# ml4ai/iqlpref

Measured on AMD Instinct MI355X. Metric: iql_grad_steps_per_sec, higher is better.
Workload: dtype bf16; 1 GPU; IQL antmaze-medium-diverse-v2 shapes (S=29 A=8 H=256), 1M-transition device replay, batch 256, one seed per GPU; batch=256, buffer_rows=1000000, graph_unroll=0, graph_launches_per_block=0, eager_steps_per_block=1390

## Files before the change

include/iqlhip.h:

```cpp
#ifndef IQLHIP_H
#define IQLHIP_H

#include <stddef.h>
#include <stdint.h>

#ifdef __cplusplus
extern "C" {
#endif

typedef enum {
  IQLHIP_OK = 0,
  IQLHIP_ERR_INVALID = -1,
  IQLHIP_ERR_HIP = -2,
  IQLHIP_ERR_UNSUPPORTED = -3,
  IQLHIP_ERR_NOMEM = -4
} iqlhip_status;

const char *iqlhip_last_error(void);
int iqlhip_abi_version(void);
const char *iqlhip_build_tag(void);


typedef struct {
  const float *rows;
  int64_t n_rows;
  int32_t row_stride;
  int32_t state_dim;
  int32_t action_dim;
  uint64_t generation;
} iqlhip_replay_view;

int32_t iqlhip_replay_next_offset(int32_t state_dim, int32_t action_dim);
int32_t iqlhip_replay_row_stride(int32_t state_dim, int32_t action_dim);

int iqlhip_replay_pack(float *rows, int32_t row_stride, int32_t state_dim,
                       int32_t action_dim, int64_t first_row, int64_t n,
                       const float *obs, const float *act, const float *rew,
                       const float *next_obs, const float *done, void *stream);

int iqlhip_replay_pack_normalized(float *rows, int32_t row_stride, int32_t state_dim,
                                  int32_t action_dim, int64_t first_row, int64_t n,
                                  const float *obs, const float *act, const float *rew,
                                  const float *next_obs, const float *done, const float *mean,
                                  const float *std, void *stream);

int iqlhip_prep_keep_mask(const uint8_t *terminals, const uint8_t *timeouts, int64_t n,
                          int32_t max_episode_steps, int32_t terminate_on_end, uint8_t *keep,
                          int64_t *ep_steps, void *stream);
int iqlhip_prep_reward_range(const float *rewards, const uint8_t *terminals, int64_t n,
                             int32_t max_episode_steps, double *trj_lens, double *min_ret,
                             double *max_ret, void *stream);
int iqlhip_prep_modify_reward(float *rewards, int64_t n, const double *trj_lens, int32_t sub_first,
                              int32_t scale, int32_t sub_one, double min_ret, double max_ret,
                              int32_t max_episode_steps, void *stream);
int iqlhip_prep_state_stats(const float *obs, int64_t n, int32_t state_dim, double eps, float *mean,
                            float *std, void *stream);

int iqlhip_replay_sample(const iqlhip_replay_view *view, int32_t batch,
                         const int64_t *idx, uint64_t seed, uint64_t step, float *s,
                         float *a, float *r, float *s2, float *d, int64_t *idx_out,
                         void *stream);

#define IQLHIP_PREC_FP32 0
#define IQLHIP_PREC_BF16 1

typedef struct {
  int32_t state_dim, action_dim;
  int32_t hidden_dim;
  int32_t batch_size;
  int32_t deterministic;
  int32_t precision;
  float dropout_p;
  float discount, tau, beta, iql_tau;
  double lr_q, lr_v, lr_actor;
  double adam_beta1, adam_beta2, adam_eps;
  int64_t cosine_t_max;
  uint64_t seed;
  int32_t n_critics;
  int32_t polyak_form;
  int32_t n_hidden;
} iqlhip_trainer_config;

#define IQLHIP_MAX_CRITICS 8
#define IQLHIP_MAX_HIDDEN 6
#define IQLHIP_N_TENSORS (2 * (IQLHIP_MAX_HIDDEN + 1) * (IQLHIP_MAX_CRITICS + 2) + 1)
int iqlhip_arena_layout(const iqlhip_trainer_config *cfg, int64_t offsets[IQLHIP_N_TENSORS],
                        int64_t *n_params, int64_t *n_target);

typedef struct {
  float *params;
  float *exp_avg;
  float *exp_avg_sq;
  float *target;
  float *grads;
} iqlhip_arenas;

typedef struct iqlhip_trainer iqlhip_trainer;

int iqlhip_trainer_create(iqlhip_trainer **out, const iqlhip_trainer_config *cfg,
                          const iqlhip_arenas *arenas);
int iqlhip_trainer_destroy(iqlhip_trainer *t);

int iqlhip_trainer_step_kind(iqlhip_trainer *t, int32_t *kind);

int iqlhip_trainer_sync_weights(iqlhip_trainer *t, void *stream);

int iqlhip_trainer_set_step(iqlhip_trainer *t, int64_t total_it);
int iqlhip_trainer_get_step(iqlhip_trainer *t, int64_t *total_it, double *actor_lr);
int iqlhip_trainer_set_lr(iqlhip_trainer *t, double lr_q, double lr_v, double lr_actor_base);

int iqlhip_train_steps(iqlhip_trainer *t, const iqlhip_replay_view *view, int64_t n_steps,
                       const int64_t *idx, const uint8_t *dropout_keep, float *losses_out,
                       int32_t graph_unroll, void *stream);

int iqlhip_train_steps_valid(iqlhip_trainer *t, const iqlhip_replay_view *view, int64_t n_steps,
                             const int64_t *idx, const int32_t *n_valid, const uint8_t *dropout_keep,
                             float *losses_out, int32_t graph_unroll, void *stream);

#define IQLHIP_MAX_GROUP 16
typedef struct iqlhip_group iqlhip_group;
int iqlhip_group_create(iqlhip_group **out, iqlhip_trainer *const *trainers, int32_t n);
int iqlhip_group_destroy(iqlhip_group *g);
int iqlhip_group_train_steps(iqlhip_group *g, const iqlhip_replay_view *views, int64_t n_steps,
                             const int64_t *const *idx, const uint8_t *const *dropout_keep,
                             float *const *losses_out, int32_t graph_unroll, void *stream);

int iqlhip_group_train_steps_valid(iqlhip_group *g, const iqlhip_replay_view *views, int64_t n_steps,
                                   const int64_t *const *idx, const int32_t *const *n_valid,
                                   const uint8_t *const *dropout_keep, float *const *losses_out,
                                   int32_t graph_unroll, void *stream);

int iqlhip_stream_create_cu_slice(void **stream, int32_t slice, int32_t n_slices);
int iqlhip_stream_destroy(void *stream);

int iqlhip_trainer_launch_counts(iqlhip_trainer *t, int64_t *eager_steps, int64_t *graph_launches);
int iqlhip_group_launch_counts(iqlhip_group *g, int64_t *eager_steps, int64_t *graph_launches);

int iqlhip_group_set_timing(iqlhip_group *g, int32_t enable);
int iqlhip_group_get_timing(iqlhip_group *g, double avg_ms[3], int64_t *n_launches);

int iqlhip_train_batch(iqlhip_trainer *t, const float *s, const float *a, const float *r,
                       const float *s2, const float *d, const uint8_t *dropout_keep,
                       float *losses_out, void *stream);

int iqlhip_forward(iqlhip_trainer *t, int32_t which, const float *s, const float *a,
                   int64_t n, float *out, void *stream);

#define IQLHIP_MLP_MAX_LAYERS 8
typedef struct {
  int32_t n_layers;
  int32_t dims[IQLHIP_MLP_MAX_LAYERS + 1];
  const float *weights[IQLHIP_MLP_MAX_LAYERS];
  const float *biases[IQLHIP_MLP_MAX_LAYERS];
  int32_t w_in_out;
  int32_t hidden_act;
  int32_t out_act;
  float dropout_p;
  uint32_t dropout_call;
  uint64_t dropout_seed;
} iqlhip_mlp_desc;

int iqlhip_mlp_forward(const iqlhip_mlp_desc *d, const float *x, int64_t n, int32_t x_stride,
                       float *out, int32_t out_stride, void *stream);

int iqlhip_cvar_tail_mean(const float *preds, int32_t S, int64_t N, int32_t n_tail, float *out,
                          void *stream);

typedef struct {
  int32_t state_dim, action_dim;
  int32_t embd_dim;
  int32_t num_heads;
  int32_t inter_dim;
  int32_t num_layers;
  int32_t n_temb;
  float eps;
  const float *state_wT, *state_b;
  const float *action_wT, *action_b;
  const float *temb;
  const float *sln_w, *sln_b;
  const float *ln0_w, *ln0_b;
  const float *qkv_w, *qkv_b;
  const float *attn_out_w, *attn_out_b;
  const float *ln1_w, *ln1_b;
  const float *mlp_in_w, *mlp_in_b;
  const float *mlp_out_w, *mlp_out_b;
  const float *lnf_w, *lnf_b;
  const float *pref_w_last;
  float pref_b_last;
} iqlhip_pt_weights;

int iqlhip_pt_relabel(const iqlhip_pt_weights *w, const float *obs, const float *act, int64_t n_rows,
                      const int64_t *win_start, const int32_t *win_len, const int32_t *win_t0,
                      int64_t n_win, int32_t query_length, float *out, void *stream);

typedef struct {
  const float *ln0_w, *ln0_b;
  const float *qkv_w, *qkv_b;
  const float *attn_out_w, *attn_out_b;
  const float *ln1_w, *ln1_b;
  const float *mlp_in_w, *mlp_in_b;
  const float *mlp_out_w, *mlp_out_b;
} iqlhip_pt_block;

typedef struct {
  int32_t state_dim, action_dim;
  int32_t embd_dim;
  int32_t num_heads;
  int32_t inter_dim;
  int32_t num_layers;
  int32_t n_temb;
  float eps;
  const float *state_wT, *state_b;
  const float *action_wT, *action_b;
  const float *temb;
  const float *sln_w, *sln_b;
  const float *lnf_w, *lnf_b;
  const float *pref_w_last;
  float pref_b_last;
  const iqlhip_pt_block *blocks;
} iqlhip_pt_model;

int iqlhip_pt_general_workspace_bytes(const iqlhip_pt_model *m, int32_t query_length, int64_t n_win,
                                      size_t *bytes);

int iqlhip_pt_relabel_general(const iqlhip_pt_model *m, const float *obs, const float *act, int64_t n_rows,
                              const int64_t *win_start, const int32_t *win_len, const int32_t *win_t0,
                              int64_t n_win, int32_t query_length, void *workspace, size_t workspace_bytes,
                              float *out, void *stream);

int iqlhip_np_randint(uint32_t *state, const int64_t *hi, int32_t K, int32_t batch,
                      int64_t n_batches, int64_t *const *out, void *stream);

int iqlhip_replay_append(float *rows, int32_t row_stride, int32_t state_dim, int32_t action_dim,
                         int64_t capacity, int64_t pointer, int64_t n, const float *obs, const float *act,
                         const float *rew, const float *next_obs, const float *done, void *stream);

int iqlhip_np_randint_growing(uint32_t *state, const int64_t *hi0, const int64_t *cap, int32_t growth,
                              int32_t K, int32_t batch, int64_t n_steps, int64_t *const *out, void *stream);

int iqlhip_explore_action(iqlhip_trainer *t, const float *s, int64_t rows, const float *eps,
                          float expl_noise, float noise_clip, float max_action, uint32_t call, float *out,
                          void *stream);

int iqlhip_block_epoch_indices(const int64_t *perm, int64_t n_rows, int32_t batch, int64_t t0,
                               int64_t n_steps, int64_t *idx, int32_t *n_valid, void *stream);

int iqlhip_block_epoch_indices_group(const int64_t *const *perm, int64_t n_rows, int32_t batch, int64_t t0,
                                     int64_t n_steps, int64_t *const *idx, int32_t *n_valid, int32_t K,
                                     void *stream);

typedef struct {
  int32_t n_obs;
  int32_t n_near;
  int32_t state_dim;
  int32_t action_dim;
  int32_t max_horizon;
// ... 41 lines not shown
```

iqlpref_amd/_lib.py:

```python
import ctypes as C
import os

HERE = os.path.dirname(os.path.abspath(__file__))
LIB_PATH = os.environ.get("IQLHIP_LIB") or os.path.join(HERE, "libiqlhip.so")

PREC_FP32 = 0
PREC_BF16 = 1
MAX_CRITICS = 8
MAX_HIDDEN = 6
N_TENSORS = 2 * (MAX_HIDDEN + 1) * (MAX_CRITICS + 2) + 1
MLP_MAX_LAYERS = 8
MAX_GROUP = 16
ACT_FLAX_BASE = 8
ABI_VERSION = 6
CHOICE_MEAN = 0
CHOICE_MEDIAN = 1

ERR_INVALID = -1
ERR_HIP = -2
ERR_UNSUPPORTED = -3
ERR_NOMEM = -4


class ReplayView(C.Structure):
    _fields_ = [("rows", C.c_void_p), ("n_rows", C.c_int64), ("row_stride", C.c_int32),
                ("state_dim", C.c_int32), ("action_dim", C.c_int32), ("generation", C.c_uint64)]


class TrainerConfig(C.Structure):
    _fields_ = [("state_dim", C.c_int32), ("action_dim", C.c_int32),
                ("hidden_dim", C.c_int32), ("batch_size", C.c_int32),
                ("deterministic", C.c_int32), ("precision", C.c_int32),
                ("dropout_p", C.c_float),
                ("discount", C.c_float), ("tau", C.c_float), ("beta", C.c_float),
                ("iql_tau", C.c_float),
                ("lr_q", C.c_double), ("lr_v", C.c_double), ("lr_actor", C.c_double),
                ("adam_beta1", C.c_double), ("adam_beta2", C.c_double),
                ("adam_eps", C.c_double),
                ("cosine_t_max", C.c_int64), ("seed", C.c_uint64),
                ("n_critics", C.c_int32), ("polyak_form", C.c_int32), ("n_hidden", C.c_int32)]


class Arenas(C.Structure):
    _fields_ = [("params", C.c_void_p), ("exp_avg", C.c_void_p), ("exp_avg_sq", C.c_void_p),
                ("target", C.c_void_p), ("grads", C.c_void_p)]


class MlpDesc(C.Structure):
    _fields_ = [("n_layers", C.c_int32), ("dims", C.c_int32 * (MLP_MAX_LAYERS + 1)),
                ("weights", C.c_void_p * MLP_MAX_LAYERS),
                ("biases", C.c_void_p * MLP_MAX_LAYERS),
                ("w_in_out", C.c_int32), ("hidden_act", C.c_int32), ("out_act", C.c_int32),
                ("dropout_p", C.c_float), ("dropout_call", C.c_uint32), ("dropout_seed", C.c_uint64)]


class PtWeights(C.Structure):
    _fields_ = ([("state_dim", C.c_int32), ("action_dim", C.c_int32), ("embd_dim", C.c_int32),
                 ("num_heads", C.c_int32), ("inter_dim", C.c_int32), ("num_layers", C.c_int32),
                 ("n_temb", C.c_int32), ("eps", C.c_float)] +
                [(n, C.c_void_p) for n in (
                    "state_wT", "state_b", "action_wT", "action_b", "temb", "sln_w", "sln_b",
                    "ln0_w", "ln0_b", "qkv_w", "qkv_b", "attn_out_w", "attn_out_b",
                    "ln1_w", "ln1_b", "mlp_in_w", "mlp_in_b", "mlp_out_w", "mlp_out_b",
                    "lnf_w", "lnf_b", "pref_w_last")] +
                [("pref_b_last", C.c_float)])


PT_MAX_LAYERS = 8


class PtBlock(C.Structure):
    _fields_ = [(n, C.c_void_p) for n in (
        "ln0_w", "ln0_b", "qkv_w", "qkv_b", "attn_out_w", "attn_out_b",
        "ln1_w", "ln1_b", "mlp_in_w", "mlp_in_b", "mlp_out_w", "mlp_out_b")]


class PtModel(C.Structure):
    _fields_ = ([("state_dim", C.c_int32), ("action_dim", C.c_int32), ("embd_dim", C.c_int32),
                 ("num_heads", C.c_int32), ("inter_dim", C.c_int32), ("num_layers", C.c_int32),
                 ("n_temb", C.c_int32), ("eps", C.c_float)] +
                [(n, C.c_void_p) for n in (
                    "state_wT", "state_b", "action_wT", "action_b", "temb", "sln_w", "sln_b",
                    "lnf_w", "lnf_b", "pref_w_last")] +
                [("pref_b_last", C.c_float), ("blocks", C.POINTER(PtBlock))])


class BbSim(C.Structure):
    _fields_ = ([(n, C.c_int32) for n in ("n_obs", "n_near", "state_dim", "action_dim", "max_horizon",
                                          "actor_out_stride")] +
                [(n, C.c_void_p) for n in ("state", "drift", "ctl", "obs_hist", "act_hist", "record", "actor_in",
                                           "actor_out", "state_mean", "state_std", "min_actions", "max_actions")])


P = C.c_void_p
SYMBOLS = {
    "iqlhip_last_error": (C.c_char_p, []),
    "iqlhip_abi_version": (C.c_int, []),
    "iqlhip_build_tag": (C.c_char_p, []),
    "iqlhip_replay_row_stride": (C.c_int32, [C.c_int32, C.c_int32]),
    "iqlhip_replay_next_offset": (C.c_int32, [C.c_int32, C.c_int32]),
    "iqlhip_replay_pack": (C.c_int, [P, C.c_int32, C.c_int32, C.c_int32, C.c_int64, C.c_int64,
                                     P, P, P, P, P, P]),
    "iqlhip_replay_pack_normalized": (C.c_int, [P, C.c_int32, C.c_int32, C.c_int32, C.c_int64, C.c_int64,
                                                P, P, P, P, P, P, P, P]),
    "iqlhip_prep_keep_mask": (C.c_int, [P, P, C.c_int64, C.c_int32, C.c_int32, P, P, P]),
    "iqlhip_prep_reward_range": (C.c_int, [P, P, C.c_int64, C.c_int32, P, C.POINTER(C.c_double),
                                           C.POINTER(C.c_double), P]),
    "iqlhip_prep_modify_reward": (C.c_int, [P, C.c_int64, P, C.c_int32, C.c_int32, C.c_int32, C.c_double,
                                            C.c_double, C.c_int32, P]),
    "iqlhip_prep_state_stats": (C.c_int, [P, C.c_int64, C.c_int32, C.c_double, P, P, P]),
    "iqlhip_replay_sample": (C.c_int, [C.POINTER(ReplayView), C.c_int32, P, C.c_uint64,
                                       C.c_uint64, P, P, P, P, P, P, P]),
    "iqlhip_arena_layout": (C.c_int, [C.POINTER(TrainerConfig), C.POINTER(C.c_int64 * N_TENSORS),
                                      C.POINTER(C.c_int64), C.POINTER(C.c_int64)]),
    "iqlhip_trainer_create": (C.c_int, [C.POINTER(P), C.POINTER(TrainerConfig), C.POINTER(Arenas)]),
    "iqlhip_trainer_destroy": (C.c_int, [P]),
    "iqlhip_trainer_step_kind": (C.c_int, [P, C.POINTER(C.c_int32)]),
    "iqlhip_trainer_sync_weights": (C.c_int, [P, P]),
    "iqlhip_trainer_set_step": (C.c_int, [P, C.c_int64]),
    "iqlhip_trainer_get_step": (C.c_int, [P, C.POINTER(C.c_int64), C.POINTER(C.c_double)]),
    "iqlhip_trainer_set_lr": (C.c_int, [P, C.c_double, C.c_double, C.c_double]),
    "iqlhip_train_steps": (C.c_int, [P, C.POINTER(ReplayView), C.c_int64, P, P, P, C.c_int32, P]),
    "iqlhip_train_steps_valid": (C.c_int, [P, C.POINTER(ReplayView), C.c_int64, P, P, P, P, C.c_int32, P]),
    "iqlhip_group_create": (C.c_int, [C.POINTER(P), C.POINTER(P), C.c_int32]),
    "iqlhip_group_destroy": (C.c_int, [P]),
    "iqlhip_group_train_steps": (C.c_int, [P, C.POINTER(ReplayView), C.c_int64, C.POINTER(P), C.POINTER(P),
                                           C.POINTER(P), C.c_int32, P]),
    "iqlhip_group_train_steps_valid": (C.c_int, [P, C.POINTER(ReplayView), C.c_int64, C.POINTER(P), C.POINTER(P),
                                                 C.POINTER(P), C.POINTER(P), C.c_int32, P]),
    "iqlhip_group_set_timing": (C.c_int, [P, C.c_int32]),
    "iqlhip_group_get_timing": (C.c_int, [P, C.POINTER(C.c_double * 3), C.POINTER(C.c_int64)]),
    "iqlhip_trainer_launch_counts": (C.c_int, [P, C.POINTER(C.c_int64), C.POINTER(C.c_int64)]),
    "iqlhip_group_launch_counts": (C.c_int, [P, C.POINTER(C.c_int64), C.POINTER(C.c_int64)]),
    "iqlhip_stream_create_cu_slice": (C.c_int, [C.POINTER(P), C.c_int32, C.c_int32]),
    "iqlhip_stream_destroy": (C.c_int, [P]),
    "iqlhip_train_batch": (C.c_int, [P, P, P, P, P, P, P, P, P]),
    "iqlhip_forward": (C.c_int, [P, C.c_int32, P, P, C.c_int64, P, P]),
    "iqlhip_mlp_forward": (C.c_int, [C.POINTER(MlpDesc), P, C.c_int64, C.c_int32, P, C.c_int32, P]),
    "iqlhip_cvar_tail_mean": (C.c_int, [P, C.c_int32, C.c_int64, C.c_int32, P, P]),
    "iqlhip_pt_relabel": (C.c_int, [C.POINTER(PtWeights), P, P, C.c_int64, P, P, P, C.c_int64, C.c_int32,
                                    P, P]),
    "iqlhip_pt_general_workspace_bytes": (C.c_int, [C.POINTER(PtModel), C.c_int32, C.c_int64,
                                                    C.POINTER(C.c_size_t)]),
    "iqlhip_pt_relabel_general": (C.c_int, [C.POINTER(PtModel), P, P, C.c_int64, P, P, P, C.c_int64, C.c_int32,
                                            P, C.c_size_t, P, P]),
    "iqlhip_np_randint": (C.c_int, [P, P, C.c_int32, C.c_int32, C.c_int64, P, P]),
    "iqlhip_replay_append": (C.c_int, [P, C.c_int32, C.c_int32, C.c_int32, C.c_int64, C.c_int64, C.c_int64,
                                       P, P, P, P, P, P]),
    "iqlhip_np_randint_growing": (C.c_int, [P, P, P, C.c_int32, C.c_int32, C.c_int32, C.c_int64, P, P]),
    "iqlhip_explore_action": (C.c_int, [P, P, C.c_int64, P, C.c_float, C.c_float, C.c_float, C.c_uint32, P, P]),
    "iqlhip_block_epoch_indices": (C.c_int, [P, C.c_int64, C.c_int32, C.c_int64, C.c_int64, P, P, P]),
    "iqlhip_block_epoch_indices_group": (C.c_int, [C.POINTER(P), C.c_int64, C.c_int32, C.c_int64, C.c_int64,
                                                   C.POINTER(P), P, C.c_int32, P]),
    "iqlhip_bb_sim_reset": (C.c_int, [C.POINTER(BbSim), P]),
    "iqlhip_bb_sim_step": (C.c_int, [C.POINTER(BbSim), P]),
    "iqlhip_bb_sim_rollout": (C.c_int, [C.POINTER(BbSim), C.POINTER(MlpDesc), C.c_int32, P]),
    "iqlhip_bb_sim_episodes_scratch_bytes": (C.c_int, [C.POINTER(C.POINTER(MlpDesc)), C.c_int32,
                                                       C.POINTER(C.c_size_t)]),
    "iqlhip_bb_sim_episodes": (C.c_int, [C.POINTER(BbSim), C.POINTER(C.POINTER(MlpDesc)), C.c_int32, P, C.c_size_t,
                                         P]),
    "iqlhip_posterior_choice_workspace_bytes": (C.c_int, [C.c_int32, C.c_int64, C.c_int32, C.POINTER(C.c_size_t)]),
    "iqlhip_posterior_choice": (C.c_int, [P, P, C.c_int32, C.c_int64, C.c_int32, C.c_int32, P, P, P, C.c_size_t, P]),
    "iqlhip_step_cost": (C.c_int, [C.POINTER(TrainerConfig), C.POINTER(C.c_double),
                                   C.POINTER(C.c_double)]),
    "iqlhip_trainer_set_timing": (C.c_int, [P, C.c_int32]),
    "iqlhip_trainer_get_timing": (C.c_int, [P, C.POINTER(C.c_double * 3), C.POINTER(C.c_int64)]),
}

_lib = None


def load():
    global _lib
    if _lib is not None:
        return _lib
    if not os.path.exists(LIB_PATH):
        raise ImportError(
            f"{LIB_PATH} is missing: build it with `python -m iqlpref_amd.build` "
            "(hipcc --offload-arch=gfx950). iqlpref_amd has no CPU fallback.")
    lib = C.CDLL(LIB_PATH)
    for name, (res, args) in SYMBOLS.items():
        fn = getattr(lib, name)
        fn.restype = res
        fn.argtypes = args
    if lib.iqlhip_abi_version() != ABI_VERSION:
        raise ImportError("libiqlhip.so ABI version mismatch; rebuild it")
    if not os.environ.get("IQLHIP_LIB"):
        from . import build as _build
        want, have = _build.source_tag(), lib.iqlhip_build_tag().decode()
        if want != have:
            raise ImportError(
                f"{LIB_PATH} was built from other sources (library tag {have}, sources {want}): "
                "rebuild it with `python -m iqlpref_amd.build`")
    _lib = lib
    return lib


def build_tag():
    return load().iqlhip_build_tag().decode()


def check(rc):
    if rc == 0:
        return
    msg = load().iqlhip_last_error().decode("utf-8", "replace")
    if rc == ERR_INVALID:
        raise ValueError(msg)
    if rc == ERR_UNSUPPORTED:
        raise NotImplementedError(msg)
    if rc == ERR_NOMEM:
        raise MemoryError(msg)
    raise RuntimeError(msg)


def require_gpu(device):
    import torch
    dev = torch.device(device)
    if dev.type != "cuda" or not torch.cuda.is_available():
        raise RuntimeError(
            f"iqlpref_amd runs on a ROCm GPU only (got device={device!r}, "
            f"torch.cuda.is_available()={torch.cuda.is_available()}); there is no CPU path")
    return dev


def stream_ptr():
    import torch
    raw = getattr(torch._C, "_cuda_getCurrentRawStream", None)
    if raw is not None:
        return C.c_void_p(raw(torch.cuda.current_device()))
    return C.c_void_p(torch.cuda.current_stream().cuda_stream)


def ptr(t):
    return C.c_void_p(t.data_ptr()) if t is not None else C.c_void_p(0)
```

iqlpref_amd/csrc/api.hip:

```cpp
#include <hip/hip_runtime.h>

#include <algorithm>
#include <cmath>
#include <cstdarg>
#include <cstdio>
#include <cstdlib>
#include <cstring>
#include <new>
#include <vector>

#include "../../include/iqlhip.h"
#include "common.h"
#include "iql_deep.h"
#include "iql_step.h"
#include "step_math.h"

namespace iqlhip {
struct DeepTrainer;
bool deep_shape_ok(const iqlhip_trainer_config &, int n_hidden, const char **why);
hipError_t deep_create(DeepTrainer **, const iqlhip_trainer_config &, int n_hidden, const iqlhip_arenas &,
                       const int64_t *offsets);
void deep_destroy(DeepTrainer *);
hipError_t deep_sync_weights(DeepTrainer *, hipStream_t);
const DeepDesc &deep_desc(const DeepTrainer *);
const DeepDesc *deep_desc_dev(const DeepTrainer *);
hipError_t deep_step(const DeepTrainer *, const DeepDesc *, const DeepArgs *, DeepCtr *, const AdamCoef *coefs, int K,
                     hipStream_t, hipEvent_t *ev);
hipError_t deep_infer(DeepTrainer *, int which, const float *s, const float *a, int64_t n, float *out, hipStream_t);
int layer2_parts(int H);
hipError_t launch_forward(bool, const TrainerDesc &, const TrainerDesc *, const DevArgs *, const DevCtr *,
                          int n_seeds, hipStream_t);
hipError_t launch_backward(bool, const TrainerDesc &, const TrainerDesc *, const DevArgs *, DevCtr *,
                           int n_seeds, hipStream_t, bool counts = false);
hipError_t launch_stage(bool, const TrainerDesc &, const TrainerDesc *, const DevArgs *, const DevCtr *,
                        int n_seeds, hipStream_t);
int strip_rows();
int update_lds_floats();
hipError_t launch_update(bool, const TrainerDesc *, const DevArgs *, DevCtr *, const UpdItem *, int,
                         int n_seeds, hipStream_t);
hipError_t launch_sync_weights(bool, const TrainerDesc *, hipStream_t);
hipError_t prepare_step_kernels();

hipError_t launch_infer(bool, const TrainerDesc &, const TrainerDesc *, const FwdNet &, const float *,
                        const float *, int64_t, float *, int, hipStream_t);

hipError_t launch_pack(float *rows, int stride, int S, int A, int64_t first, int64_t n, const float *obs,
                       const float *act, const float *rew, const float *nxt, const float *done,
                       hipStream_t st);
hipError_t launch_sample(const iqlhip_replay_view &v, int batch, const int64_t *idx, uint64_t seed,
                         uint64_t step, float *s, float *a, float *r, float *s2, float *d,
                         int64_t *idx_out, hipStream_t st);
hipError_t launch_mlp_f32(const iqlhip_mlp_desc &d, const float *x, int64_t n, int x_stride, float *out,
                          int out_stride, hipStream_t st);
hipError_t launch_cvar(const float *preds, int S, int64_t N, int n_tail, float *out, hipStream_t st);
hipError_t launch_keep_steps(const uint8_t *term, const uint8_t *tmo, int64_t n, int64_t M, int toe,
                             uint8_t *keep, int64_t *ep_steps, hipStream_t st);
hipError_t launch_reward_range(const float *rew, const uint8_t *term, int64_t n, int64_t M, double *trj_lens,
                               double *out3, hipStream_t st);
hipError_t launch_modify_reward(float *rew, int64_t n, const double *trj_lens, int sub_first, int scale,
                                int sub_one, double min_ret, double range, float steps, hipStream_t st);
hipError_t launch_state_stats(const float *x, int64_t n, int S, double eps, float *mean_f, float *std_f,
                              hipStream_t st);
hipError_t launch_pack_norm(float *rows, int stride, int S, int A, int64_t first, int64_t n, const float *obs,
                            const float *act, const float *rew, const float *nxt, const float *done,
                            const float *mean, const float *sd, hipStream_t st);
size_t pt_smem_bytes(const iqlhip_pt_weights &W, int ql);
hipError_t launch_pt(const iqlhip_pt_weights &W, const float *obs, const float *act, int64_t n_rows,
                     const int64_t *win_start, const int32_t *win_len, const int32_t *win_t0, int64_t n_win,
                     int ql, float *out, hipStream_t st);
size_t pt_general_bytes(const iqlhip_pt_model &m, int ql, int64_t nw);
int64_t pt_general_fit(const iqlhip_pt_model &m, int ql, size_t bytes);
int pt_general_tp(int ql);
hipError_t launch_pt_general(const iqlhip_pt_model &m, const float *obs, const float *act, int64_t n_rows,
                             const int64_t *win_start, const int32_t *win_len, const int32_t *win_t0,
                             int64_t n_win, int ql, float *ws, int64_t chunk, float *out, hipStream_t st);
hipError_t launch_block_epoch(const int64_t *perm, int64_t n_rows, int batch, int64_t t0, int64_t n_steps, int64_t *idx,
                              int32_t *n_valid, hipStream_t st);
hipError_t launch_block_epoch_group(const int64_t *const *perm, int64_t n_rows, int batch, int64_t t0, int64_t n_steps,
                                    int64_t *const *idx, int32_t *n_valid, int K, hipStream_t st);
hipError_t launch_replay_append(float *rows, int stride, int S, int A, int64_t pointer, int64_t capacity, int64_t n,
                                const float *obs, const float *act, const float *rew, const float *nxt,
                                const float *done, hipStream_t st);
hipError_t launch_np_randint_growing(uint32_t *state, const int64_t *hi0, const int64_t *cap, int growth, int K,
                                     int batch, int64_t n_steps, int64_t *const *out, hipStream_t st);
hipError_t launch_explore_epilogue(float *act, int64_t rows, int A, const float *log_std, const float *eps,
                                   float expl_noise, float noise_clip, float max_action, uint64_t seed, uint32_t call,
                                   hipStream_t st);
hipError_t launch_np_randint(uint32_t *state, const int64_t *hi, int K, int64_t total, int64_t *const *out,
                             hipStream_t st);
hipError_t launch_bb_step(const iqlhip_bb_sim &sim, int reset, hipStream_t st);
size_t bb_episodes_scratch_bytes(const iqlhip_mlp_desc *const *actors, int n);
hipError_t launch_bb_episodes(const iqlhip_bb_sim *sims, const iqlhip_mlp_desc *const *actors, int n, void *scratch,
                              hipStream_t st);
size_t choice_workspace_bytes(int64_t N, int n);
int64_t choice_fit_rows(int64_t N, int n, size_t bytes);
hipError_t launch_posterior_choice(uint32_t *state, const float *preds, int S, int64_t N, int n, int mode,
                                   float *out, uint16_t *idx_out, uint16_t *ws, int64_t slot_rows,
                                   hipStream_t st);
}

using namespace iqlhip;

static thread_local char g_err[512] = "";
static int fail(int code, const char *fmt, ...) {
  va_list ap;
  va_start(ap, fmt);
  vsnprintf(g_err, sizeof(g_err), fmt, ap);
  va_end(ap);
  return code;
}
#define HIP_TRY(expr)                                                                         \
  do {                                                                                        \
    hipError_t e_ = (expr);                                                                   \
    if (e_ != hipSuccess)                                                                     \
      return fail(IQLHIP_ERR_HIP, "%s failed: %s (%s:%d)", #expr, hipGetErrorString(e_), __FILE__, \
                  __LINE__);                                                                  \
  } while (0)

extern "C" const char *iqlhip_last_error(void) { return g_err; }
static hipError_t capture_stream(hipStream_t *out) {
  static thread_local hipStream_t pool[64] = {};
  int dev = 0;
  hipError_t e = hipGetDevice(&dev);
  if (e != hipSuccess) return e;
  if (dev < 0 || dev >= 64) return hipErrorInvalidDevice;
  if (!pool[dev]) {
    e = hipStreamCreateWithFlags(&pool[dev], hipStreamNonBlocking);
    if (e != hipSuccess) return e;
  }
  *out = pool[dev];
  return hipSuccess;
}

extern "C" int iqlhip_abi_version(void) { return 6; }
#ifndef IQLHIP_BUILD_TAG
#define IQLHIP_BUILD_TAG "untagged"
#endif
static const char g_build_tag[] = "IQLHIP_BUILD_TAG=" IQLHIP_BUILD_TAG;
extern "C" const char *iqlhip_build_tag(void) { return g_build_tag + sizeof("IQLHIP_BUILD_TAG=") - 1; }

extern "C" int32_t iqlhip_replay_next_offset(int32_t S, int32_t A) { return round_up(S + A + 2, 4); }
extern "C" int32_t iqlhip_replay_row_stride(int32_t S, int32_t A) {
  return round_up(iqlhip_replay_next_offset(S, A) + S, 4);
}

extern "C" int iqlhip_replay_pack(float *rows, int32_t row_stride, int32_t S, int32_t A, int64_t first_row,
                                  int64_t n, const float *obs, const float *act, const float *rew,
                                  const float *next_obs, const float *done, void *stream) {
  if (!rows || !obs || !act || !rew || !next_obs || !done) return fail(IQLHIP_ERR_INVALID, "null pointer");
  if (S <= 0 || A <= 0 || n < 0 || first_row < 0 || row_stride < iqlhip_replay_row_stride(S, A) || (row_stride & 3))
    return fail(IQLHIP_ERR_INVALID, "bad replay geometry S=%d A=%d stride=%d", S, A, row_stride);
  if (n == 0) return 0;
  HIP_TRY(launch_pack(rows, row_stride, S, A, first_row, n, obs, act, rew, next_obs, done,
                      (hipStream_t)stream));
  return 0;
}

extern "C" int iqlhip_replay_pack_normalized(float *rows, int32_t row_stride, int32_t S, int32_t A,
                                             int64_t first_row, int64_t n, const float *obs, const float *act,
                                             const float *rew, const float *next_obs, const float *done,
                                             const float *mean, const float *std, void *stream) {
  if (!rows || !obs || !act || !rew || !next_obs || !done || !mean || !std)
    return fail(IQLHIP_ERR_INVALID, "null pointer");
  if (S <= 0 || A <= 0 || n < 0 || first_row < 0 || row_stride < iqlhip_replay_row_stride(S, A) || (row_stride & 3))
    return fail(IQLHIP_ERR_INVALID, "bad replay geometry S=%d A=%d stride=%d", S, A, row_stride);
  if (n == 0) return 0;
  HIP_TRY(launch_pack_norm(rows, row_stride, S, A, first_row, n, obs, act, rew, next_obs, done, mean, std,
                           (hipStream_t)stream));
  return 0;
}

extern "C" int iqlhip_prep_keep_mask(const uint8_t *terminals, const uint8_t *timeouts, int64_t n,
                                     int32_t max_episode_steps, int32_t terminate_on_end, uint8_t *keep,
                                     int64_t *ep_steps, void *stream) {
  if (!terminals || !keep || !ep_steps) return fail(IQLHIP_ERR_INVALID, "null pointer");
  if (n < 1) return fail(IQLHIP_ERR_INVALID, "n must be >= 1");
  if (!timeouts && max_episode_steps < 1) return fail(IQLHIP_ERR_INVALID, "max_episode_steps must be >= 1");
  HIP_TRY(launch_keep_steps(terminals, timeouts, n, max_episode_steps, terminate_on_end != 0, keep, ep_steps,
                            (hipStream_t)stream));
  return 0;
}

extern "C" int iqlhip_prep_reward_range(const float *rewards, const uint8_t *terminals, int64_t n,
                                        int32_t max_episode_steps, double *trj_lens, double *min_ret,
                                        double *max_ret, void *stream) {
  if (!rewards || !terminals || !trj_lens || !min_ret || !max_ret) return fail(IQLHIP_ERR_INVALID, "null pointer");
  if (n < 1 || max_episode_steps < 1) return fail(IQLHIP_ERR_INVALID, "n and max_episode_steps must be >= 1");
  double out3[3];
  HIP_TRY(launch_reward_range(rewards, terminals, n, max_episode_steps, trj_lens, out3, (hipStream_t)stream));
  if (out3[2] == 0.0) return fail(IQLHIP_ERR_INVALID, "dataset holds no complete episode");
  *min_ret = out3[0], *max_ret = out3[1];
  return 0;
}

extern "C" int iqlhip_prep_modify_reward(float *rewards, int64_t n, const double *trj_lens, int32_t sub_first,
                                         int32_t scale, int32_t sub_one, double min_ret, double max_ret,
                                         int32_t max_episode_steps, void *stream) {
  if (!rewards) return fail(IQLHIP_ERR_INVALID, "null pointer");
  if (sub_first < 0 || sub_first > 2) return fail(IQLHIP_ERR_INVALID, "sub_first must be 0, 1 or 2");
  if (sub_first == 2 && !trj_lens) return fail(IQLHIP_ERR_INVALID, "sub_first = 2 needs trj_lens");
  if (n <= 0) return 0;
  HIP_TRY(launch_modify_reward(rewards, n, trj_lens, sub_first, scale != 0, sub_one != 0, min_ret,
                               max_ret - min_ret, (float)max_episode_steps, (hipStream_t)stream));
  return 0;
}

extern "C" int iqlhip_prep_state_stats(const float *obs, int64_t n, int32_t state_dim, double eps, float *mean,
                                       float *std, void *stream) {
  if (!obs || !mean || !std) return fail(IQLHIP_ERR_INVALID, "null pointer");
  if (n < 1 || state_dim < 1 || state_dim > 256) return fail(IQLHIP_ERR_UNSUPPORTED, "n >= 1, 1 <= state_dim <= 256");
  HIP_TRY(launch_state_stats(obs, n, state_dim, eps, mean, std, (hipStream_t)stream));
  return 0;
}

extern "C" int iqlhip_replay_sample(const iqlhip_replay_view *view, int32_t batch, const int64_t *idx,
                                    uint64_t seed, uint64_t step, float *s, float *a, float *r, float *s2,
                                    float *d, int64_t *idx_out, void *stream) {
  if (!view || !view->rows || !s || !a || !r || !s2 || !d) return fail(IQLHIP_ERR_INVALID, "null pointer");
  if (batch <= 0) return fail(IQLHIP_ERR_INVALID, "batch must be positive");
  if (view->n_rows <= 0) return fail(IQLHIP_ERR_INVALID, "cannot sample from an empty replay buffer");
  HIP_TRY(launch_sample(*view, batch, idx, seed, step, s, a, r, s2, d, idx_out, (hipStream_t)stream));
  return 0;
}

static void group_invalidate(struct iqlhip_group *g);

struct Throttle {
  static constexpr int NEV = 2;
  hipEvent_t ev[NEV] = {};
  bool used[NEV] = {};
  int head = 0;
  int64_t since = 0;
  static int64_t window() {
    static const int64_t w = [] {
      const char *e = getenv("IQLHIP_MAX_INFLIGHT");
      const int64_t total = e ? atoll(e) : 6144;
      return total <= 0 ? (int64_t)0 : (total / 3 > 0 ? total / 3 : (int64_t)1);
    }();
    return w;
  }
  hipError_t queued(int64_t n, hipStream_t st) {
    const int64_t w = window();
    if (w == 0) return hipSuccess;
    since += n;
    if (since < w) return hipSuccess;
    since = 0;
    hipError_t e;
    if (!ev[head] && (e = hipEventCreateWithFlags(&ev[head], hipEventDisableTiming)) != hipSuccess) return e;
    if (used[head] && (e = hipEventSynchronize(ev[head])) != hipSuccess) return e;
    if ((e = hipEventRecord(ev[head], st)) != hipSuccess) return e;
    used[head] = true;
    head = (head + 1) % NEV;
    return hipSuccess;
  }
  void destroy() {
    for (auto &e : ev)
      if (e) (void)hipEventDestroy(e), e = nullptr;
  }
};

struct StepQueue {
  static constexpr int ARG_RING = 8;
  DevArgs *harg[ARG_RING] = {};
  hipEvent_t harg_ev[ARG_RING] = {};
  bool harg_used[ARG_RING] = {};
  int harg_head = 0;
  DevArgs dev_args[IQLHIP_MAX_GROUP];
  bool dev_args_valid = false;
  hipGraphExec_t gexec = nullptr;
  int graph_unroll = 0;
  bool graph_counts = false;
  hipStream_t cap_stream = nullptr;
  Throttle throttle;
  bool timing = false;
  hipEvent_t ev[5] = {};
  double t_acc[3] = {0, 0, 0};
  double t_empty = 0;
  int64_t t_n = 0;
  int64_t n_eager = 0, n_graph = 0;

  int push(const DevArgs *want, int K, DevArgs *dst, hipStream_t st) {
    const int slot = harg_head;
    harg_head = (slot + 1) % ARG_RING;
    if (!harg[slot]) {
      HIP_TRY(hipHostMalloc((void **)&harg[slot], sizeof(DevArgs) * K, hipHostMallocDefault));
      HIP_TRY(hipEventCreateWithFlags(&harg_ev[slot], hipEventDisableTiming));
    }
    if (harg_used[slot]) HIP_TRY(hipEventSynchronize(harg_ev[slot]));
    for (int k = 0; k < K; ++k) harg[slot][k] = dev_args[k] = want[k];
    HIP_TRY(hipMemcpyAsync(dst, harg[slot], sizeof(DevArgs) * K, hipMemcpyHostToDevice, st));
    HIP_TRY(hipEventRecord(harg_ev[slot], st));
    harg_used[slot] = true;
    return 0;
  }
  void drop_graph() {
    if (gexec) (void)hipGraphExecDestroy(gexec);
    gexec = nullptr;
  }
  template <typename Step>
  int ensure_graph(int U, bool counts, Step step) {
    if (gexec && graph_unroll == U && graph_counts == counts) return 0;
    drop_graph();
    hipGraph_t g = nullptr;
    if (!cap_stream) HIP_TRY(capture_stream(&cap_stream));
    HIP_TRY(hipStreamBeginCapture(cap_stream, hipStreamCaptureModeThreadLocal));
    int rc = 0;
    for (int u = 0; u < U && !rc; ++u) rc = step(cap_stream);
    const hipError_t ce = hipStreamEndCapture(cap_stream, &g);
    if ((rc || ce != hipSuccess) && g) (void)hipGraphDestroy(g);
    if (rc) return rc;
    HIP_TRY(ce);
    const hipError_t ie = hipGraphInstantiate(&gexec, g, nullptr, nullptr, 0);
    (void)hipGraphDestroy(g);
    HIP_TRY(ie);
    graph_unroll = U, graph_counts = counts;
    return 0;
  }
  int replay(int64_t &done, int64_t n, hipStream_t st) {
    for (; done + graph_unroll <= n; done += graph_unroll) {
      HIP_TRY(hipGraphLaunch(gexec, st));
      ++n_graph;
      HIP_TRY(throttle.queued(3 * (int64_t)graph_unroll, st));
    }
    return 0;
  }
  int eager_issued(hipStream_t st) {
    ++n_eager;
    if (!timing) {
      HIP_TRY(throttle.queued(3, st));
      return 0;
    }
    HIP_TRY(hipEventRecord(ev[4], st));
    HIP_TRY(hipEventSynchronize(ev[4]));
    for (int k = 0; k < 3; ++k) {
      float ms = 0.f;
      HIP_TRY(hipEventElapsedTime(&ms, ev[k], ev[k + 1]));
      t_acc[k] += ms;
    }
    float ems = 0.f;
    HIP_TRY(hipEventElapsedTime(&ems, ev[3], ev[4]));
    t_empty += ems;
    ++t_n;
    return 0;
  }
  int set_timing(bool enable) {
    timing = enable;
    t_acc[0] = t_acc[1] = t_acc[2] = 0, t_empty = 0, t_n = 0;
    if (timing)
      for (auto &e : ev)
        if (!e) HIP_TRY(hipEventCreate(&e));
    return 0;
  }
  void get_timing(double avg_ms[3], int64_t *n) const {
    for (int k = 0; k < 3; ++k) {
      const double v = t_n ? (t_acc[k] - t_empty) / (double)t_n : 0.0;
      avg_ms[k] = v > 0 ? v : 0.0;
    }
    if (n) *n = t_n;
  }
  void launch_counts(int64_t *eager_steps, int64_t *graph_launches) const {
    if (eager_steps) *eager_steps = n_eager;
    if (graph_launches) *graph_launches = n_graph;
  }
  void destroy() {
    drop_graph();
    for (int k = 0; k < ARG_RING; ++k) {
      if (harg_ev[k]) (void)hipEventDestroy(harg_ev[k]);
      if (harg[k]) (void)hipHostFree(harg[k]);
    }
    for (auto &e : ev)
      if (e) (void)hipEventDestroy(e);
    throttle.destroy();
  }
};

struct DeepRing {
  static constexpr int RING = 4;
  static constexpr int64_t CAP = 1024;
  int K = 0;
  char *dev = nullptr;
  char *host[RING] = {};
  hipEvent_t ev[RING] = {};
  bool used[RING] = {};
  int head = 0;
  size_t head_bytes() const { return (size_t)K * (sizeof(DeepArgs) + sizeof(DeepCtr)); }
  size_t bytes(int64_t n) const { return head_bytes() + (size_t)n * K * sizeof(AdamCoef); }
  DeepArgs *dargs() const { return reinterpret_cast<DeepArgs *>(dev); }
  DeepCtr *dctr() const { return reinterpret_cast<DeepCtr *>(dev + (size_t)K * sizeof(DeepArgs)); }
  AdamCoef *dcoef() const { return reinterpret_cast<AdamCoef *>(dev + head_bytes()); }
  hipError_t init(int k) {
    K = k;
    hipError_t e = hipMalloc((void **)&dev, bytes(CAP));
    return e != hipSuccess ? e : hipMemset(dev, 0, bytes(CAP));
  }
  void destroy() {
    for (int k = 0; k < RING; ++k) {
      if (ev[k]) (void)hipEventDestroy(ev[k]);
      if (host[k]) (void)hipHostFree(host[k]);
      ev[k] = nullptr, host[k] = nullptr;
    }
    if (dev) (void)hipFree(dev);
    dev = nullptr;
  }
};

struct iqlhip_trainer {
  iqlhip_trainer_config cfg;
  iqlhip_arenas arenas;
  DeepTrainer *deep = nullptr;
  DeepRing deep_ring;
  TrainerDesc D;
  bool bf16;
  void *ws = nullptr;
  size_t ws_bytes = 0;
  TrainerDesc *ddesc = nullptr;
  DevArgs *dargs = nullptr;
  DevCtr *dctr = nullptr;
  UpdItem *ditems = nullptr;
  int n_items = 0;
  int own_n_items = 0;
  std::vector<UpdItem> net_items[MAX_TRAIN];
  int n_half0[MAX_TRAIN] = {};
  TrainerDesc *own_ddesc = nullptr;
  DevArgs *own_dargs = nullptr;
  DevCtr *own_dctr = nullptr;
  UpdItem *own_ditems = nullptr;
  struct iqlhip_group *group = nullptr;

  float *batch_rows = nullptr;
  int64_t total_it = 0;
  double lr_q, lr_v, lr_a_base;
  StepQueue queue;
};

static_assert(MAX_CRITICS == IQLHIP_MAX_CRITICS, "iql_step.h and iqlhip.h disagree");
static_assert(IQLHIP_N_TENSORS == 2 * DEEP_MAX_LIN * MAX_TRAIN + 1, "offset table size");
static_assert(IQLHIP_MAX_HIDDEN + 1 == DEEP_MAX_LIN, "iql_deep.h and iqlhip.h disagree");
static int n_critics(const iqlhip_trainer_config &c) { return c.n_critics > 0 ? c.n_critics : 2; }
static int n_hidden(const iqlhip_trainer_config &c) { return c.n_hidden > 0 ? c.n_hidden : 2; }
static bool is_deep(const iqlhip_trainer_config &c) {
  static const bool force_general = getenv("IQLHIP_FORCE_GENERAL") != nullptr;
  return n_hidden(c) != 2 || (c.hidden_dim != 64 && c.hidden_dim != 128 && c.hidden_dim != 256) || force_general;
}

static int check_cfg(const iqlhip_trainer_config *c) {
  if (!c) return fail(IQLHIP_ERR_INVALID, "null config");
  if (c->n_critics < 0 || c->n_critics == 1 || c->n_critics > MAX_CRITICS)
    return fail(IQLHIP_ERR_UNSUPPORTED, "n_critics %d: 0 (= 2) or 2..%d", c->n_critics, MAX_CRITICS);
  if (c->state_dim <= 0 || c->action_dim <= 0) return fail(IQLHIP_ERR_INVALID, "bad dims");
  if (c->n_hidden < 0) return fail(IQLHIP_ERR_INVALID, "n_hidden must be >= 0");
  if (const char *why = nullptr; !deep_shape_ok(*c, n_hidden(*c), &why))
    return fail(IQLHIP_ERR_UNSUPPORTED, "n_hidden %d, hidden_dim %d: %s", n_hidden(*c), c->hidden_dim, why);
  if (c->batch_size < 16 || c->batch_size % 16)
    return fail(IQLHIP_ERR_UNSUPPORTED, "batch_size %d: must be a positive multiple of 16", c->batch_size);
  if (c->action_dim > 32) return fail(IQLHIP_ERR_UNSUPPORTED, "action_dim %d > 32", c->action_dim);
  if (c->state_dim + c->action_dim > 128) return fail(IQLHIP_ERR_UNSUPPORTED, "state_dim+action_dim > 128");
  if (!is_deep(*c) && (c->batch_size / 16) * (n_critics(*c) + 2 + (c->deterministic ? 0 : c->action_dim)) + n_critics(*c) + 2 >
      update_lds_floats())
    return fail(IQLHIP_ERR_UNSUPPORTED, "batch_size %d too large for action_dim %d", c->batch_size,
                c->action_dim);
  if (c->precision != IQLHIP_PREC_FP32 && c->precision != IQLHIP_PREC_BF16)
    return fail(IQLHIP_ERR_INVALID, "precision must be IQLHIP_PREC_FP32 or IQLHIP_PREC_BF16");
  if (c->dropout_p >= 1.0f) return fail(IQLHIP_ERR_INVALID, "dropout_p must be < 1");
  if (c->cosine_t_max <= 0) return fail(IQLHIP_ERR_INVALID, "cosine_t_max must be positive");
  if (c->polyak_form != 0 && c->polyak_form != 1) return fail(IQLHIP_ERR_INVALID, "polyak_form must be 0 or 1");
  return 0;
}

struct Layout {
  int64_t off[IQLHIP_N_TENSORS];
  int64_t n_params, n_target;
  int64_t true_params, true_target;
};
static void net_dims(const iqlhip_trainer_config &c, int net, int *in, int *out) {
  const int E = n_critics(c);
  *in = net < E ? c.state_dim + c.action_dim : c.state_dim;
  *out = (net == E + 1) ? c.action_dim : 1;
}
static Layout make_layout(const iqlhip_trainer_config &c) {
  constexpr int64_t ALIGN = 32;
  Layout L;
  int64_t o = 0, cnt = 0;
  const int H = c.hidden_dim, NL = n_hidden(c) + 1;
  const int E = n_critics(c), ntrain = E + 2;
  for (int k = 0; k < IQLHIP_N_TENSORS; ++k) L.off[k] = -1;
  for (int n = 0; n < ntrain; ++n) {
    int in, out;
    net_dims(c, n, &in, &out);
    for (int l = 0; l < NL; ++l) {
      const int64_t rows = l == NL - 1 ? out : H, cols = l == 0 ? in : H;
      const int64_t sz[2] = {rows * cols, rows};
      for (int k = 0; k < 2; ++k) {
        o = (o + ALIGN - 1) / ALIGN * ALIGN;
        L.off[(n * NL + l) * 2 + k] = o;
        o += sz[k];
        cnt += sz[k];
      }
    }
    if (n == E - 1) L.n_target = o, L.true_target = cnt;
  }
  if (c.deterministic) {
    L.off[ntrain * NL * 2] = -1;
  } else {
    o = (o + ALIGN - 1) / ALIGN * ALIGN;
    L.off[ntrain * NL * 2] = o;
    o += c.action_dim;
    cnt += c.action_dim;
  }
  L.n_params = o;
  L.true_params = cnt;
  return L;
}

extern "C" int iqlhip_arena_layout(const iqlhip_trainer_config *cfg, int64_t offsets[IQLHIP_N_TENSORS],
                                   int64_t *n_params, int64_t *n_target) {
  if (int e = check_cfg(cfg)) return e;
  const Layout L = make_layout(*cfg);
  if (offsets) memcpy(offsets, L.off, sizeof(L.off));
  if (n_params) *n_params = L.n_params;
  if (n_target) *n_target = L.n_target;
  return 0;
}

extern "C" int iqlhip_step_cost(const iqlhip_trainer_config *cfg, double *bytes, double *flops) {
  if (int e = check_cfg(cfg)) return e;
  const Layout L = make_layout(*cfg);
  const double B = cfg->batch_size, S = cfg->state_dim, A = cfg->action_dim, H = cfg->hidden_dim;
  if (bytes) *bytes = 4.0 * B * (2 * S + A + 2) + 32.0 * (double)L.true_params + 8.0 * (double)L.true_target;
  if (flops) {
    const double E = n_critics(*cfg), HH = (n_hidden(*cfg) - 1) * H * H;
    const double wv = S * H + HH + H, wq = (S + A) * H + HH + H, wa = S * H + HH + H * A;
    const double fwd = 2 * wv + 2 * E * wq + wa;
    const double dw = wv + E * wq + wa;
    const double dx = (HH + H) * (E + 1) + (HH + H * A);
    *flops = 2.0 * B * (fwd + dw + dx);
  }
  return 0;
}

template <typename T>
static T *carve(char *&p, size_t n) {
  T *r = reinterpret_cast<T *>(p);
  p += (n * sizeof(T) + 255) / 256 * 256;
  return r;
}

static std::vector<UpdItem> flatten_table(const std::vector<UpdItem> (&per_xcd)[8], size_t min_depth, size_t *depth_out,
                                          size_t min_idle) {
  size_t depth = 0, n_real = 0;
  for (auto &v : per_xcd) depth = v.size() > depth ? v.size() : depth, n_real += v.size();
  while (8 * depth - n_real < min_idle) ++depth;
  if (depth < min_depth) depth = min_depth;
  std::vector<UpdItem> items;
  for (size_t d = 0; d < depth; ++d)
    for (int x = 0; x < 8; ++x) {
      UpdItem pad;
      memset(&pad, 0, sizeof(pad));
      pad.net = -1;
      items.push_back(d < per_xcd[x].size() ? per_xcd[x][d] : pad);
    }
  int n_pad = 0;
  for (auto &it : items)
    if (it.net < 0) it.o0 = n_pad++;
  for (auto &it : items)
    if (it.net < 0) it.i0 = n_pad;
  if (depth_out) *depth_out = depth;
  return items;
}

static void deal_items(const iqlhip_trainer *t, int member, int group_size, std::vector<UpdItem> (&per_xcd)[8]) {
  const int NT = t->D.ntrain;
  const bool group = group_size > 1;
  const bool whole = group && group_size % 8 == 0;
  if (whole && NT == 4) {
    for (int n = 0; n < NT; ++n)
      for (auto &it : t->net_items[n]) per_xcd[(2 * n + member) & 7].push_back(it);
    return;
  }
  if (NT == 4) {
    for (int n = 0; n < NT; ++n)
      for (size_t i = 0; i < t->net_items[n].size(); ++i)
        per_xcd[(2 * n + ((int)i < t->n_half0[n] ? 0 : 1)) & 7].push_back(t->net_items[n][i]);
    return;
  }
  size_t total = 0, g = 0;
  for (int n = 0; n < NT; ++n) total += t->net_items[n].size();
  for (int n = 0; n < NT; ++n)
    for (auto &it : t->net_items[n]) {
      const int x = (int)(g * 8 / total);
      per_xcd[(x + (group ? member : 0)) & 7].push_back(it);
      ++g;
    }
  if (!group) {
    constexpr size_t CUS_PER_XCD = 32;
    auto weight = [](const UpdItem &it) { return it.layer == 1 ? 3 : (it.layer == 0 ? 2 : 1); };
    for (auto &col : per_xcd) {
      if (col.size() <= CUS_PER_XCD || col.size() >= 2 * CUS_PER_XCD) continue;
      const size_t d = col.size() - CUS_PER_XCD;
      std::vector<UpdItem> sorted(col);
      std::stable_sort(sorted.begin(), sorted.end(), [&](const UpdItem &a, const UpdItem &b) { return weight(a) < weight(b); });
      std::vector<UpdItem> out(sorted.begin(), sorted.begin() + d);
      out.insert(out.end(), sorted.begin() + 2 * d, sorted.end());
      out.insert(out.end(), sorted.begin() + d, sorted.begin() + 2 * d);
      col.swap(out);
    }
  }
}

extern "C" int iqlhip_trainer_create(iqlhip_trainer **out, const iqlhip_trainer_config *cfg,
                                     const iqlhip_arenas *ar) {
  if (!out) return fail(IQLHIP_ERR_INVALID, "null out");
  if (int e = check_cfg(cfg)) return e;
  if (!ar || !ar->params || !ar->exp_avg || !ar->exp_avg_sq || !ar->target)
    return fail(IQLHIP_ERR_INVALID, "null arena pointer");
  HIP_TRY(prepare_step_kernels());
  iqlhip_trainer *t = new (std::nothrow) iqlhip_trainer();
  if (!t) return fail(IQLHIP_ERR_NOMEM, "host allocation failed");
  t->cfg = *cfg;
  t->arenas = *ar;
  t->bf16 = cfg->precision == IQLHIP_PREC_BF16;
  t->lr_q = cfg->lr_q, t->lr_v = cfg->lr_v, t->lr_a_base = cfg->lr_actor;
  const Layout L = make_layout(*cfg);
  if (is_deep(*cfg)) {
    memset(&t->D, 0, sizeof(t->D));
    t->D.E = n_critics(*cfg);
    const size_t rows_bytes = (size_t)cfg->batch_size * iqlhip_replay_row_stride(cfg->state_dim, cfg->action_dim) * 4;
    hipError_t e = deep_create(&t->deep, *cfg, n_hidden(*cfg), *ar, L.off);
    if (e == hipSuccess && (e = hipMalloc((void **)&t->batch_rows, rows_bytes)) != hipSuccess) deep_destroy(t->deep);
    if (e == hipSuccess && (e = t->deep_ring.init(1)) != hipSuccess) {
      deep_destroy(t->deep);
      (void)hipFree(t->batch_rows);
      t->deep_ring.destroy();
    }
    if (e != hipSuccess) {
      delete t;
      return fail(e == hipErrorOutOfMemory ? IQLHIP_ERR_NOMEM : IQLHIP_ERR_HIP, "general step: %s", hipGetErrorString(e));
    }
    *out = t;
    return 0;
  }
  const int S = cfg->state_dim, A = cfg->action_dim, H = cfg->hidden_dim, B = cfg->batch_size;
  const int es = t->bf16 ? 2 : 4, KM = t->bf16 ? 32 : 16;
  TrainerDesc &D = t->D;
  memset(&D, 0, sizeof(D));
  D.S = S, D.A = A, D.H = H, D.B = B, D.BP = round_up(B, 32);
  const int E = n_critics(*cfg), NT = E + 2, NF = 2 * E + 3;
  D.E = E, D.ntrain = NT, D.nfwd = NF, D.net_v = E, D.net_a = E + 1;
  D.out_v = E, D.out_qt = E + 1, D.out_nv = 2 * E + 1, D.out_mean = 2 * E + 2;
  D.two_over_B = 2.0f / (float)B, D.inv_E = 1.0f / (float)E;
  D.OUTW = round_up(D.out_mean + A, 4);
  D.deterministic = cfg->deterministic;
  D.has_dropout = cfg->dropout_p > 0.f;
  D.discount = cfg->discount, D.tau = cfg->tau, D.beta = cfg->beta, D.iql_tau = cfg->iql_tau;
  D.one_m_tau = (float)(1.0 - (double)cfg->tau);
  D.polyak_convex = cfg->polyak_form == 1;
  if (D.has_dropout) {
    const float scale = 1.0f / (float)(1.0 - (double)cfg->dropout_p);
    if (t->bf16) {
      uint32_t u;
      memcpy(&u, &scale, 4);
      u = (u + 0x7fffu + ((u >> 16) & 1u)) & 0xffff0000u;
      memcpy(&D.drop_scale, &u, 4);
    } else {
      D.drop_scale = scale;
    }
    const double thr = (double)cfg->dropout_p * 4294967296.0;
    D.drop_thr = thr >= 4294967295.0 ? 0xffffffffu : (uint32_t)thr;
  }
  D.beta1 = cfg->adam_beta1, D.beta2 = cfg->adam_beta2, D.eps = cfg->adam_eps;
  D.t_max = cfg->cosine_t_max;
  D.seed = cfg->seed;
  D.params = ar->params, D.exp_avg = ar->exp_avg, D.exp_avg_sq = ar->exp_avg_sq;
  D.target = ar->target, D.grads = ar->grads;
  D.off_log_std = L.off[NT * 6];
  D.opmax = round_up(A, 16);
  D.xrows = round_up(S + A, 64);
  D.k1max = round_up(S + A, KM);
  size_t total = 0;
  auto add = [&](size_t bytes) { total += (bytes + 255) / 256 * 256; };
  int k1pad[MAX_TRAIN], outpad[MAX_TRAIN], indim[MAX_TRAIN], outdim[MAX_TRAIN];
  for (int n = 0; n < NT; ++n) {
    net_dims(*cfg, n, &indim[n], &outdim[n]);
    k1pad[n] = round_up(indim[n], KM);
    outpad[n] = round_up(outdim[n], 16);
    const int copies = (n < E) ? 2 : 1;
    for (int c = 0; c < copies; ++c) {
      add((size_t)H * k1pad[n] * es);
      add((size_t)H * H * es);
      add((size_t)outpad[n] * H * es);
    }
    add((size_t)H * H * es);
    add((size_t)H * outpad[n] * es);
  }
  add((size_t)2 * D.xrows * D.BP * es);
  add((size_t)B * 2 * 4);
  add((size_t)B * A * 4);
  add((size_t)NT * 2 * H * D.BP * es);
  add((size_t)NT * H * D.BP * es);
  add((size_t)NT * H * D.BP * es);
  add((size_t)NT * D.opmax * D.BP * es);
  add((size_t)layer2_parts(H) * B * D.OUTW * 4);
  add((size_t)NT * (B / 16) * 4);
  add((size_t)(B / 16) * A * 4);
  add((size_t)A * 4);
  const int stride = iqlhip_replay_row_stride(S, A);
  add((size_t)B * stride * 4);
  add((size_t)B * stride * 4);
  add(sizeof(DevArgs));
  add(sizeof(DevCtr));
  add(sizeof(TrainerDesc));
  for (int n = 0; n < NT; ++n) {
    std::vector<UpdItem> half[2];
    auto put = [&](int layer, int o0, int i0) {
      UpdItem it;
      memset(&it, 0, sizeof(it));
      it.net = n, it.layer = layer, it.o0 = o0, it.i0 = i0;
      const int rows = layer == 2 ? outpad[n] : H;
      half[(layer == 2 && rows <= 64) ? ((i0 / 32) & 1) : (o0 >= rows / 2 ? 1 : 0)].push_back(it);
    };
    for (int o0 = 0; o0 < H; o0 += 64)
      for (int i0 = 0; i0 < H; i0 += 32) put(1, o0, i0);
    for (int o0 = 0; o0 < H; o0 += strip_rows()) put(0, o0, 0);
    for (int o0 = 0; o0 < outpad[n]; o0 += 64)
      for (int i0 = 0; i0 < H; i0 += 32) put(2, o0, i0);
    t->n_half0[n] = (int)half[0].size();
    t->net_items[n] = half[0];
    t->net_items[n].insert(t->net_items[n].end(), half[1].begin(), half[1].end());
  }
  size_t n_slots;
  {
    std::vector<UpdItem> per_xcd[8];
    deal_items(t, 0, 1, per_xcd);
    size_t depth = 0;
    n_slots = flatten_table(per_xcd, 0, &depth, (size_t)(B + 15) / 16).size();
  }
  t->n_items = t->own_n_items = (int)n_slots;
  add(n_slots * sizeof(UpdItem));

  if (hipMalloc(&t->ws, total) != hipSuccess) {
    delete t;
    return fail(IQLHIP_ERR_NOMEM, "hipMalloc of %zu workspace bytes failed", total);
  }
  t->ws_bytes = total;
  if (hipMemset(t->ws, 0, total) != hipSuccess) {
    (void)hipFree(t->ws);
    delete t;
    return fail(IQLHIP_ERR_HIP, "hipMemset failed");
  }
  char *p = reinterpret_cast<char *>(t->ws);
  for (int n = 0; n < NT; ++n) {
    TrainNet &N = D.net[n];
    N.in_dim = indim[n], N.k1pad = k1pad[n], N.out_dim = outdim[n], N.out_pad = outpad[n];
    N.has_target = n < E;
    for (int k = 0; k < 3; ++k) {
      N.off_w[k] = L.off[n * 6 + 2 * k];
      N.off_b[k] = L.off[n * 6 + 2 * k + 1];
      N.toff_w[k] = N.has_target ? N.off_w[k] : -1;
      N.toff_b[k] = N.has_target ? N.off_b[k] : -1;
    }
    N.wc[0] = carve<char>(p, (size_t)H * k1pad[n] * es);
    N.wc[1] = carve<char>(p, (size_t)H * H * es);
    N.wc[2] = carve<char>(p, (size_t)outpad[n] * H * es);
    if (N.has_target) {
      N.tc[0] = carve<char>(p, (size_t)H * k1pad[n] * es);
      N.tc[1] = carve<char>(p, (size_t)H * H * es);
      N.tc[2] = carve<char>(p, (size_t)outpad[n] * H * es);
    }
    N.w2ct = carve<char>(p, (size_t)H * H * es);
    N.w3t = carve<char>(p, (size_t)H * outpad[n] * es);
  }
  D.xT = carve<char>(p, (size_t)2 * D.xrows * D.BP * es);
  D.rd = carve<float>(p, (size_t)B * 2);
  D.actf = carve<float>(p, (size_t)B * A);
  D.hT = carve<char>(p, (size_t)NT * 2 * H * D.BP * es);
  D.dz1T = carve<char>(p, (size_t)NT * H * D.BP * es);
  D.dz2T = carve<char>(p, (size_t)NT * H * D.BP * es);
  D.dz3T = carve<char>(p, (size_t)NT * D.opmax * D.BP * es);
  D.outs = carve<float>(p, (size_t)layer2_parts(H) * B * D.OUTW);
  D.lossp = carve<float>(p, (size_t)NT * (B / 16));
  D.lsp = carve<float>(p, (size_t)(B / 16) * A);
  D.ls_snap = carve<float>(p, (size_t)A);
  t->batch_rows = carve<float>(p, (size_t)B * stride);
  D.stage_rows = carve<float>(p, (size_t)B * stride);
  D.stage_stride = stride;
  D.next_off = iqlhip_replay_next_offset(S, A);
  D.prefetch = !getenv("IQLHIP_NO_PREFETCH") ? 1 : 0;
  t->own_dargs = t->dargs = carve<DevArgs>(p, 1);
  t->own_dctr = t->dctr = carve<DevCtr>(p, 1);
  t->own_ddesc = t->ddesc = carve<TrainerDesc>(p, 1);
  t->own_ditems = t->ditems = carve<UpdItem>(p, n_slots);

  for (int n_ = 0; n_ < NT; ++n_)
  for (auto &it : t->net_items[n_]) {
    const TrainNet &N = D.net[it.net];
    const int L = it.layer;
    it.Odim = (L == 2) ? N.out_dim : H;
    it.Idim = (L == 0) ? N.in_dim : H;
    it.Opad = (L == 2) ? N.out_pad : H;
    it.Kw = (L == 0) ? N.k1pad : H;
    it.has_target = N.has_target;
    it.group = it.net == D.net_v ? 1 : (it.net == D.net_a ? 2 : 0);
    it.off_w = N.off_w[L], it.off_b = N.off_b[L], it.toff_w = N.toff_w[L], it.toff_b = N.toff_b[L];

    it.wc = N.wc[L], it.tc = N.has_target ? N.tc[L] : nullptr, it.w2ct = (L == 1) ? N.w2ct : nullptr;
    it.w3t = (L == 2) ? N.w3t : nullptr;
    const size_t plane = (size_t)H * D.BP * es;
    it.Xsrc = (L == 0) ? D.xT : reinterpret_cast<char *>(D.hT) + (size_t)(it.net * 2 + (L - 1)) * plane;
    it.Zsrc = (L == 0)   ? reinterpret_cast<char *>(D.dz1T) + (size_t)it.net * plane
              : (L == 1) ? reinterpret_cast<char *>(D.dz2T) + (size_t)it.net * plane
                         : reinterpret_cast<char *>(D.dz3T) + (size_t)it.net * D.opmax * D.BP * es;
  }
  std::vector<UpdItem> items;
  {
    std::vector<UpdItem> per_xcd[8];
    deal_items(t, 0, 1, per_xcd);
    items = flatten_table(per_xcd, 0, nullptr, (size_t)(B + 15) / 16);
  }
  if (items.size() != n_slots || hipMemcpy(t->ditems, items.data(), items.size() * sizeof(UpdItem), hipMemcpyHostToDevice) !=
      hipSuccess) {
    (void)hipFree(t->ws);
    delete t;
    return fail(IQLHIP_ERR_HIP, "hipMemcpy of the work items failed");
  }

  auto mk = [&](int f, int net, bool target, int in_off, int out_col, int slot) {
    FwdNet &F = D.fwd[f];
    const TrainNet &N = D.net[net];
    F.w1c = target ? N.tc[0] : N.wc[0];
    F.w2c = target ? N.tc[1] : N.wc[1];
    F.w3c = target ? N.tc[2] : N.wc[2];
    const float *base = target ? ar->target : ar->params;
    F.b1 = base + N.off_b[0], F.b2 = base + N.off_b[1], F.b3 = base + N.off_b[2];
    F.in_off = in_off, F.in_dim = N.in_dim, F.k1pad = N.k1pad;
    F.out_dim = N.out_dim, F.out_pad = N.out_pad, F.out_col = out_col;
    F.train_slot = slot;
    F.tanh_out = net == D.net_a;
    F.dropout = (net == D.net_a) && D.has_dropout;
    F.stage = f == 0;
  };
  for (int e = 0; e < E; ++e) mk(e, e, false, 0, e, e);
  mk(E, D.net_v, false, 0, D.out_v, D.net_v);
  mk(E + 1, D.net_a, false, 0, D.out_mean, D.net_a);
  for (int e = 0; e < E; ++e) mk(E + 2 + e, e, true, 0, D.out_qt + e, -1);
  mk(2 * E + 2, D.net_v, false, D.next_off, D.out_nv, -1);

  if (hipMemcpy(t->ddesc, &t->D, sizeof(TrainerDesc), hipMemcpyHostToDevice) != hipSuccess) {
    (void)hipFree(t->ws);
    delete t;
    return fail(IQLHIP_ERR_HIP, "hipMemcpy of the descriptor failed");
  }
  *out = t;
  return 0;
}

extern "C" int iqlhip_trainer_destroy(iqlhip_trainer *t) {
  if (!t) return 0;
  if (t->group) return fail(IQLHIP_ERR_INVALID, "trainer is a member of a group: destroy the group first");
  t->queue.destroy();
  if (t->deep) {
    deep_destroy(t->deep);
    (void)hipFree(t->batch_rows);
    t->deep_ring.destroy();
  }
  if (t->ws) (void)hipFree(t->ws);
  delete t;
  return 0;
}

extern "C" int iqlhip_trainer_step_kind(iqlhip_trainer *t, int32_t *kind) {
  if (!t || !kind) return fail(IQLHIP_ERR_INVALID, "null argument");
  *kind = t->deep ? 1 : 0;
  return 0;
}

extern "C" int iqlhip_trainer_sync_weights(iqlhip_trainer *t, void *stream) {
  if (!t) return fail(IQLHIP_ERR_INVALID, "null trainer");
  if (t->deep) {
    HIP_TRY(deep_sync_weights(t->deep, (hipStream_t)stream));
    return 0;
  }
  HIP_TRY(launch_sync_weights(t->bf16, t->ddesc, (hipStream_t)stream));
  return 0;
}

extern "C" int iqlhip_trainer_set_step(iqlhip_trainer *t, int64_t total_it) {
  if (!t || total_it < 0) return fail(IQLHIP_ERR_INVALID, "bad argument");
  HIP_TRY(hipDeviceSynchronize());
  t->total_it = total_it;
  if (t->deep) return 0;
  DevCtr c;
  memset(&c, 0, sizeof(c));
  c.ctr[0] = total_it, c.ctr[1] = total_it;
  HIP_TRY(hipMemcpy(t->dctr, &c, sizeof(c), hipMemcpyHostToDevice));
  t->queue.dev_args_valid = false;
  if (t->group) group_invalidate(t->group);
  return 0;
}

static double cosine_lr(double base, int64_t t, int64_t t_max) {
  return base * (1.0 + cos(M_PI * (double)t / (double)t_max)) * 0.5;
}

extern "C" int iqlhip_trainer_get_step(iqlhip_trainer *t, int64_t *total_it, double *actor_lr) {
  if (!t) return fail(IQLHIP_ERR_INVALID, "null trainer");
  if (total_it) *total_it = t->total_it;
  if (actor_lr) *actor_lr = cosine_lr(t->lr_a_base, t->total_it, t->cfg.cosine_t_max);
  return 0;
}

extern "C" int iqlhip_trainer_set_lr(iqlhip_trainer *t, double lr_q, double lr_v, double lr_a_base) {
  if (!t) return fail(IQLHIP_ERR_INVALID, "null trainer");
  t->lr_q = lr_q, t->lr_v = lr_v, t->lr_a_base = lr_a_base;
  return 0;
}

extern "C" int iqlhip_trainer_set_timing(iqlhip_trainer *t, int32_t enable) {
  return t ? t->queue.set_timing(enable != 0) : fail(IQLHIP_ERR_INVALID, "null trainer");
}

extern "C" int iqlhip_trainer_get_timing(iqlhip_trainer *t, double avg_ms[3], int64_t *n) {
  if (!t) return fail(IQLHIP_ERR_INVALID, "null trainer");
  t->queue.get_timing(avg_ms, n);
  return 0;
}

extern "C" int iqlhip_trainer_launch_counts(iqlhip_trainer *t, int64_t *eager_steps, int64_t *graph_launches) {
  if (!t) return fail(IQLHIP_ERR_INVALID, "null trainer");
  t->queue.launch_counts(eager_steps, graph_launches);
  return 0;
}

static bool continues(const DevArgs &a, const DevArgs &b) {
  return a.rows == b.rows && a.n_rows == b.n_rows && a.row_stride == b.row_stride &&
         a.generation == b.generation && a.idx_mode == 0 && b.idx_mode == 0 && !a.drop_keep && !b.drop_keep &&
         !a.losses_out && !b.losses_out && !a.n_valid && !b.n_valid && a.lr_q == b.lr_q && a.lr_v == b.lr_v && a.lr_a_base == b.lr_a_base;
}

struct StepTarget {
  bool bf16;
  const TrainerDesc &D;
  const TrainerDesc *desc;
  DevArgs *args;
  DevCtr *ctr;
  const UpdItem *items;
  int n_items, K;
};

static int enqueue_step(const StepTarget &x, bool counts, hipStream_t st, hipEvent_t *ev) {
  if (!x.D.prefetch) HIP_TRY(launch_stage(x.bf16, x.D, x.desc, x.args, x.ctr, x.K, st));
  if (ev) HIP_TRY(hipEventRecord(ev[0], st));
  HIP_TRY(launch_forward(x.bf16, x.D, x.desc, x.args, x.ctr, x.K, st));
  if (ev) HIP_TRY(hipEventRecord(ev[1], st));
  HIP_TRY(launch_backward(x.bf16, x.D, x.desc, x.args, x.ctr, x.K, st, counts));
  if (ev) HIP_TRY(hipEventRecord(ev[2], st));
  HIP_TRY(launch_update(x.bf16, x.desc, x.args, x.ctr, x.items, x.n_items, x.K, st));
  if (ev) HIP_TRY(hipEventRecord(ev[3], st));
  return 0;
}

static int run_tuned(StepQueue &q, const StepTarget &x, const DevArgs *want, int64_t n_steps, int graph_unroll,
                     bool counts, hipStream_t st) {
  bool same = x.D.prefetch && q.dev_args_valid && !q.timing, all_philox = true;
  for (int k = 0; k < x.K; ++k) {
    same = same && continues(q.dev_args[k], want[k]);
    all_philox = all_philox && want[k].idx_mode == 0;
  }
  if (!same) {
    if (int rc = q.push(want, x.K, x.args, st)) return rc;
    if (x.D.prefetch) HIP_TRY(launch_stage(x.bf16, x.D, x.desc, x.args, x.ctr, x.K, st));
  }
  q.dev_args_valid = all_philox;
  int64_t done = 0;
  if (!q.timing && graph_unroll > 0 && n_steps >= graph_unroll) {
    if (int rc = q.ensure_graph(graph_unroll, counts, [&](hipStream_t cs) { return enqueue_step(x, counts, cs, nullptr); }))
      return rc;
    if (int rc = q.replay(done, n_steps, st)) return rc;
  }
  for (; done < n_steps; ++done) {
    if (int rc = enqueue_step(x, counts, st, q.timing ? q.ev : nullptr)) return rc;
    if (int rc = q.eager_issued(st)) return rc;
  }
  return 0;
}

struct DeepRun {
  iqlhip_trainer *const *tr;
  int K;
  DeepRing *ring;
  const DeepDesc *ddesc;
  StepQueue &q;
};

static int deep_push(const DeepRun &r, const DevArgs *a, int64_t done, int64_t n, hipStream_t st) {
  DeepRing &R = *r.ring;
  const int K = r.K, slot = R.head;
  R.head = (slot + 1) % DeepRing::RING;
  if (!R.host[slot]) {
    HIP_TRY(hipHostMalloc((void **)&R.host[slot], R.bytes(DeepRing::CAP), hipHostMallocDefault));
    HIP_TRY(hipEventCreateWithFlags(&R.ev[slot], hipEventDisableTiming));
  }
  if (R.used[slot]) HIP_TRY(hipEventSynchronize(R.ev[slot]));
  DeepArgs *ha = reinterpret_cast<DeepArgs *>(R.host[slot]);
  DeepCtr *hc = reinterpret_cast<DeepCtr *>(R.host[slot] + (size_t)K * sizeof(DeepArgs));
  AdamCoef *hk = reinterpret_cast<AdamCoef *>(R.host[slot] + R.head_bytes());
  for (int k = 0; k < K; ++k) {
    const iqlhip_trainer_config &c = r.tr[k]->cfg;
    const int64_t B = c.batch_size, H = c.hidden_dim, NH = n_hidden(c);
    DeepArgs &x = ha[k];
    memset(&x, 0, sizeof(x));
    x.rows = a[k].rows, x.n_rows = a[k].n_rows, x.row_stride = a[k].row_stride, x.idx_mode = a[k].idx_mode;
    x.idx = a[k].idx ? a[k].idx + done * B : nullptr;
    x.drop_keep = a[k].drop_keep ? a[k].drop_keep + done * NH * B * H : nullptr;
    x.losses_out = a[k].losses_out ? a[k].losses_out + done * 3 : nullptr;
    x.base_step = a[k].base_step + done, x.n_steps = n;
    hc[k].ctr[0] = hc[k].ctr[1] = x.base_step;
    for (int64_t i = 0; i < n; ++i)
      hk[i * K + k] = make_adam_coef(c.adam_beta1, c.adam_beta2, c.adam_eps, a[k].lr_q, a[k].lr_v, a[k].lr_a_base,
                                     c.cosine_t_max, x.base_step + i + 1);
  }
  HIP_TRY(hipMemcpyAsync(R.dev, R.host[slot], R.bytes(n), hipMemcpyHostToDevice, st));
  HIP_TRY(hipEventRecord(R.ev[slot], st));
  R.used[slot] = true;
  return 0;
}

static int deep_run(const DeepRun &r, const DevArgs *a, int64_t n_steps, int graph_unroll, hipStream_t st) {
  StepQueue &q = r.q;
  auto step = [&](hipStream_t s, hipEvent_t *ev) {
    HIP_TRY(deep_step(r.tr[0]->deep, r.ddesc, r.ring->dargs(), r.ring->dctr(), r.ring->dcoef(), r.K, s, ev));
    return 0;
  };
  const int U = q.timing ? 0 : (int)std::min<int64_t>(std::max(graph_unroll, 0), DeepRing::CAP);
  const int64_t cap = U > 0 ? DeepRing::CAP / U * U : DeepRing::CAP;
  for (int64_t done = 0; done < n_steps;) {
    const int64_t n = std::min(cap, n_steps - done);
    if (int rc = deep_push(r, a, done, n, st)) return rc;
    int64_t i = 0;
    if (U > 0 && n >= U) {
      if (int rc = q.ensure_graph(U, false, [&](hipStream_t cs) { return step(cs, nullptr); })) return rc;
      if (int rc = q.replay(i, n, st)) return rc;
    }
    for (; i < n; ++i) {
      if (int rc = step(st, q.timing ? q.ev : nullptr)) return rc;
      if (int rc = q.eager_issued(st)) return rc;
    }
    done += n;
  }
  return 0;
}

static int check_counts(const iqlhip_trainer *t0, bool counts, const char *who) {
  if (counts && t0->deep)
    return fail(IQLHIP_ERR_UNSUPPORTED,
                "per-step valid-row counts (a short batch) run on the tuned step only (n_hidden 2, hidden_dim 64 / "
                "128 / 256); this %s (n_hidden %d, hidden_dim %d) runs the general layer-wise step",
                who, n_hidden(t0->cfg), t0->cfg.hidden_dim);
  if (counts && t0->bf16)
    return fail(IQLHIP_ERR_UNSUPPORTED, "per-step valid-row counts (a short batch) are built for precision fp32 only");
  return 0;
}

static int check_view(const iqlhip_replay_view &v, const iqlhip_trainer_config &c) {
  if (v.state_dim != c.state_dim || v.action_dim != c.action_dim)
    return fail(IQLHIP_ERR_INVALID, "replay dims (%d,%d) do not match the trainer (%d,%d)", v.state_dim,
                v.action_dim, c.state_dim, c.action_dim);
  if (v.n_rows <= 0) return fail(IQLHIP_ERR_INVALID, "cannot sample from an empty replay buffer");
  if (v.row_stride != iqlhip_replay_row_stride(v.state_dim, v.action_dim))
    return fail(IQLHIP_ERR_INVALID, "row_stride %d is not the packed layout's (%d)", v.row_stride,
                iqlhip_replay_row_stride(v.state_dim, v.action_dim));
  return 0;
}

static DevArgs make_args(const iqlhip_trainer *t, const iqlhip_replay_view &v, int64_t n_steps, const int64_t *idx,
                         const int32_t *n_valid, const uint8_t *dropout_keep, float *losses_out) {
  DevArgs a;
  memset(&a, 0, sizeof(a));
  a.rows = v.rows, a.n_rows = v.n_rows, a.row_stride = v.row_stride;
  a.generation = v.generation;
  a.idx_mode = idx ? 1 : 0, a.idx = idx;
  a.drop_keep = dropout_keep, a.losses_out = losses_out;
  a.n_valid = n_valid;
  a.base_step = t->total_it, a.n_steps = n_steps;
  a.lr_q = t->lr_q, a.lr_v = t->lr_v, a.lr_a_base = t->lr_a_base;
  return a;
}

static int run_solo(iqlhip_trainer *t, const DevArgs &a, int graph_unroll, hipStream_t st) {
  const bool counts = a.n_valid != nullptr;
  if (int rc = check_counts(t, counts, "trainer")) return rc;
  if (t->deep) {
    iqlhip_trainer *tr[1] = {t};
    return deep_run({tr, 1, &t->deep_ring, deep_desc_dev(t->deep), t->queue}, &a, a.n_steps, graph_unroll, st);
  }
  if (t->group) group_invalidate(t->group);
  const StepTarget x = {t->bf16, t->D, t->ddesc, t->dargs, t->dctr, t->ditems, t->n_items, 1};
  return run_tuned(t->queue, x, &a, a.n_steps, graph_unroll, counts, st);
}

extern "C" int iqlhip_train_steps(iqlhip_trainer *t, const iqlhip_replay_view *view, int64_t n_steps,
                                  const int64_t *idx, const uint8_t *dropout_keep, float *losses_out,
                                  int32_t graph_unroll, void *stream) {
  return iqlhip_train_steps_valid(t, view, n_steps, idx, nullptr, dropout_keep, losses_out, graph_unroll, stream);
}

extern "C" int iqlhip_train_steps_valid(iqlhip_trainer *t, const iqlhip_replay_view *view, int64_t n_steps,
                                        const int64_t *idx, const int32_t *n_valid, const uint8_t *dropout_keep,
                                        float *losses_out, int32_t graph_unroll, void *stream) {
  if (!t || !view || !view->rows) return fail(IQLHIP_ERR_INVALID, "null argument");
  if (n_steps < 0) return fail(IQLHIP_ERR_INVALID, "n_steps must be >= 0");
  if (int rc = check_view(*view, t->cfg)) return rc;
  if (n_steps == 0) return 0;
  const DevArgs a = make_args(t, *view, n_steps, idx, n_valid, dropout_keep, losses_out);
  if (int rc = run_solo(t, a, graph_unroll, (hipStream_t)stream)) return rc;
  t->total_it += n_steps;
  return 0;
}

extern "C" int iqlhip_train_batch(iqlhip_trainer *t, const float *s, const float *a, const float *r,
                                  const float *s2, const float *d, const uint8_t *dropout_keep,
                                  float *losses_out, void *stream) {
  if (!t || !s || !a || !r || !s2 || !d) return fail(IQLHIP_ERR_INVALID, "null argument");
  const int S = t->cfg.state_dim, A = t->cfg.action_dim, B = t->cfg.batch_size;
  const int stride = iqlhip_replay_row_stride(S, A);
  HIP_TRY(launch_pack(t->batch_rows, stride, S, A, 0, B, s, a, r, s2, d, (hipStream_t)stream));
  const iqlhip_replay_view rows = {t->batch_rows, B, stride, S, A, 0};
  DevArgs args = make_args(t, rows, 1, nullptr, nullptr, dropout_keep, losses_out);
  args.idx_mode = 2;
  if (int rc = run_solo(t, args, 0, (hipStream_t)stream)) return rc;
  t->total_it += 1;
  return 0;
}

struct iqlhip_group {
  int K = 0;
  int n_items = 0;
  iqlhip_trainer *tr[IQLHIP_MAX_GROUP] = {};
  void *mem = nullptr;
  TrainerDesc *gdesc = nullptr;
  DevArgs *gargs = nullptr;
  DevCtr *gctr = nullptr;
  UpdItem *gitems = nullptr;
  StepQueue queue;
  bool deep = false;
  DeepRing deep_ring;
  DeepDesc *gdeep = nullptr;
};

static void group_invalidate(iqlhip_group *g) { g->queue.dev_args_valid = false; }

static bool same_shape(const iqlhip_trainer_config &a, const iqlhip_trainer_config &b) {
  return a.state_dim == b.state_dim && a.action_dim == b.action_dim && a.hidden_dim == b.hidden_dim &&
         a.batch_size == b.batch_size && a.deterministic == b.deterministic && a.precision == b.precision &&
         n_critics(a) == n_critics(b) && (a.dropout_p > 0.f) == (b.dropout_p > 0.f) &&
         n_hidden(a) == n_hidden(b);
}

static int deep_group_create(iqlhip_group **out, iqlhip_trainer *const *trainers, int32_t n) {
  iqlhip_group *g = new (std::nothrow) iqlhip_group();
  if (!g) return fail(IQLHIP_ERR_NOMEM, "host allocation failed");
  g->K = n, g->deep = true;
  hipError_t e = hipDeviceSynchronize();
  if (e == hipSuccess) e = hipMalloc(&g->mem, sizeof(DeepDesc) * n);
  if (e == hipSuccess) {
    g->gdeep = reinterpret_cast<DeepDesc *>(g->mem);
    e = g->deep_ring.init(n);
  }
  for (int k = 0; k < n && e == hipSuccess; ++k)
    e = hipMemcpy(g->gdeep + k, &deep_desc(trainers[k]->deep), sizeof(DeepDesc), hipMemcpyHostToDevice);
  if (e != hipSuccess) {
    g->deep_ring.destroy();
    if (g->mem) (void)hipFree(g->mem);
    delete g;
    return fail(e == hipErrorOutOfMemory ? IQLHIP_ERR_NOMEM : IQLHIP_ERR_HIP, "general-step group: %s",
                hipGetErrorString(e));
  }
  for (int k = 0; k < n; ++k) g->tr[k] = trainers[k], trainers[k]->group = g;
  *out = g;
  return 0;
}

extern "C" int iqlhip_group_create(iqlhip_group **out, iqlhip_trainer *const *trainers, int32_t n) {
  if (!out || !trainers) return fail(IQLHIP_ERR_INVALID, "null argument");
  if (n < 1 || n > IQLHIP_MAX_GROUP) return fail(IQLHIP_ERR_INVALID, "group size %d: 1..%d", n, IQLHIP_MAX_GROUP);
  for (int k = 0; k < n; ++k) {
    if (!trainers[k]) return fail(IQLHIP_ERR_INVALID, "null trainer");
    if ((trainers[k]->deep != nullptr) != (trainers[0]->deep != nullptr))
      return fail(IQLHIP_ERR_INVALID, "trainer %d: a group holds trainers of the tuned step (n_hidden = 2, hidden_dim "
                  "64 / 128 / 256) or of the general step, not both", k);
    if (trainers[k]->group) return fail(IQLHIP_ERR_INVALID, "trainer %d already belongs to a group", k);
    for (int j = 0; j < k; ++j)
      if (trainers[j] == trainers[k]) return fail(IQLHIP_ERR_INVALID, "trainer %d listed twice", k);
    if (!same_shape(trainers[0]->cfg, trainers[k]->cfg) || trainers[k]->n_items != trainers[0]->n_items)
      return fail(IQLHIP_ERR_INVALID, "trainer %d differs in shape from trainer 0 (dims, batch, precision, "
                  "critics, hidden layers, policy kind and dropout on/off must match)", k);
  }
  if (trainers[0]->deep) return deep_group_create(out, trainers, n);
  iqlhip_group *g = new (std::nothrow) iqlhip_group();
  if (!g) return fail(IQLHIP_ERR_NOMEM, "host allocation failed");
  g->K = n;
  std::vector<std::vector<UpdItem>> tables(n);
  {
    size_t depth = 0;
    for (int pass = 0; pass < 2; ++pass)
      for (int k = 0; k < n; ++k) {
        std::vector<UpdItem> per_xcd[8];
        deal_items(trainers[k], k, n, per_xcd);
        size_t d = 0;
        tables[k] = flatten_table(per_xcd, depth, &d, (size_t)(trainers[k]->D.B + 15) / 16);
        depth = d > depth ? d : depth;
      }
  }
  const int ni = (int)tables[0].size();
  for (int k = 0; k < n; ++k)
    if ((int)tables[k].size() != ni) {
      delete g;
      return fail(IQLHIP_ERR_INVALID, "item tables of the members differ in size");
    }
  g->n_items = ni;
  auto up = [](size_t b) { return (b + 255) / 256 * 256; };
  const size_t b_desc = up(sizeof(TrainerDesc) * n), b_args = up(sizeof(DevArgs) * n),
               b_ctr = up(sizeof(DevCtr) * n), b_items = up(sizeof(UpdItem) * (size_t)ni * n);
  HIP_TRY(hipDeviceSynchronize());
  if (hipMalloc(&g->mem, b_desc + b_args + b_ctr + b_items) != hipSuccess) {
    delete g;
    return fail(IQLHIP_ERR_NOMEM, "hipMalloc of the group descriptors failed");
  }
  char *p = reinterpret_cast<char *>(g->mem);
  g->gdesc = reinterpret_cast<TrainerDesc *>(p), p += b_desc;
  g->gargs = reinterpret_cast<DevArgs *>(p), p += b_args;
  g->gctr = reinterpret_cast<DevCtr *>(p), p += b_ctr;
  g->gitems = reinterpret_cast<UpdItem *>(p);
  hipError_t e = hipSuccess;
  for (int k = 0; k < n && e == hipSuccess; ++k) {
    iqlhip_trainer *t = trainers[k];
    e = hipMemcpy(g->gdesc + k, t->ddesc, sizeof(TrainerDesc), hipMemcpyDeviceToDevice);
    if (e == hipSuccess) e = hipMemcpy(g->gargs + k, t->dargs, sizeof(DevArgs), hipMemcpyDeviceToDevice);
    if (e == hipSuccess) e = hipMemcpy(g->gctr + k, t->dctr, sizeof(DevCtr), hipMemcpyDeviceToDevice);
    if (e == hipSuccess)
      e = hipMemcpy(g->gitems + (size_t)k * ni, tables[k].data(), sizeof(UpdItem) * ni, hipMemcpyHostToDevice);
  }
  if (e != hipSuccess) {
    (void)hipFree(g->mem);
    delete g;
    return fail(IQLHIP_ERR_HIP, "copying the member descriptors failed: %s", hipGetErrorString(e));
  }
  for (int k = 0; k < n; ++k) {
    iqlhip_trainer *t = trainers[k];
    g->tr[k] = t;
    t->group = g;
// ... 552 lines not shown
```

iqlpref_amd/csrc/iql_step.h:

```cpp
#pragma once
#include <stdint.h>

namespace iqlhip {

constexpr int MAX_CRITICS = 8;
constexpr int MAX_TRAIN = MAX_CRITICS + 2;
constexpr int MAX_FWD = 2 * MAX_CRITICS + 3;

struct FwdNet {
  const void *w1c, *w2c, *w3c;
  const float *b1, *b2, *b3;
  int32_t in_off;
  int32_t in_dim, k1pad;
  int32_t out_dim, out_pad;
  int32_t out_col;
  int32_t train_slot;
  int32_t tanh_out;
  int32_t dropout;
  int32_t stage;
};

struct TrainNet {
  int64_t off_w[3], off_b[3];
  int64_t toff_w[3], toff_b[3];
  void *wc[3];
  void *w2ct;
  void *w3t;
  void *tc[3];
  int32_t in_dim, k1pad, out_dim, out_pad;
  int32_t has_target;
};

struct TrainerDesc {
  int32_t S, A, H, B, BP, OUTW, k1max;
  int32_t E, ntrain, nfwd, net_v, net_a;
  int32_t out_v, out_qt, out_nv, out_mean;
  int32_t stage_stride, next_off;
  int32_t opmax, xrows;
  int32_t deterministic, has_dropout;
  int32_t prefetch;
  int32_t polyak_convex;
  float two_over_B, inv_E;
  float discount, tau, beta, iql_tau;
  float one_m_tau;
  float drop_scale;
  uint32_t drop_thr;
  int32_t pad0_;
  uint64_t seed;
  float *stage_rows;
  void *xT;
  float *rd;
  float *actf;
  void *hT;
  void *dz1T;
  void *dz2T;
  void *dz3T;
  float *outs;
  float *lossp;
  float *lsp;
  float *ls_snap;
  float *params, *exp_avg, *exp_avg_sq, *target, *grads;
  int64_t off_log_std;
  unsigned long long *dbg;
  double beta1, beta2, eps;
  int64_t t_max;
  FwdNet fwd[MAX_FWD];
  TrainNet net[MAX_TRAIN];
};

struct DevArgs {
  const float *rows;
  int64_t n_rows;
  int32_t row_stride;
  int32_t idx_mode;
  const int64_t *idx;
  const uint8_t *drop_keep;
  float *losses_out;
  int64_t base_step;
  double lr_q, lr_v, lr_a_base;
  int64_t n_steps;
  uint64_t generation;
  const int32_t *n_valid;
};

struct AdamCoef {
  float one_m_b1, b2, one_m_b2, neg_step[3], bc2_sqrt, eps;
  float inv_bc2_sqrt, pad_;
};

struct DevCtr {
  int64_t ctr[2];
  int64_t coef_step;
  AdamCoef coef;
  float last_losses[4];
  double loss_sum[4];
};

struct UpdItem {
  int32_t net, layer;
  int32_t o0, i0;
  int32_t Odim, Idim;
  int32_t Opad, Kw;
  int32_t has_target, group;
  int64_t off_w, off_b, toff_w, toff_b;
  void *wc, *tc, *w2ct;
  void *w3t;
  const void *Xsrc, *Zsrc;
};

}
```

iqlpref_amd/csrc/iql_step.hip:

```cpp
#include "common.h"
#include "iql_step.h"
#include "step_math.h"

namespace iqlhip {

constexpr int SLAB = 16;

#ifdef IQL_STAMPS
#define STAMP(kern, slot)                                                                   \
  do {                                                                                      \
    if (D.dbg && threadIdx.x == 0 && blockIdx.x < 512) {                                                      \
      unsigned long long *d_ = D.dbg + (((size_t)(kern) * 512 + blockIdx.x) * 8 + (slot)) * 2; \
      d_[0] = wall_clock64();                                                               \
      d_[1] = clock64();                                                                    \
    }                                                                                       \
  } while (0)
#else
#define STAMP(kern, slot) \
  do {                    \
  } while (0)
#endif

template <class T>
__device__ __forceinline__ void pin_s(T v) {
// ... 129 lines not shown
template <bool BF16, int H, class Issue, class Fill>
__device__ __forceinline__ void mlp_slab(const FwdNet &N, const TrainerDesc &D, const DevArgs *Ap,
                                         int64_t step, int slab, char *smem, float *out, int out_stride,
                                         int64_t row0, int64_t n_valid, Issue issue, Fill fill) {
  using K = KCfg<BF16, H>;
  using P = Prec<BF16>;
  using T = typename P::T;
  const int tid = threadIdx.x, lane = tid & 63;
  const int wave = __builtin_amdgcn_readfirstlane(tid >> 6);
  const int r = lane & 15, q = lane >> 4;
  constexpr int HP = K::HP, TPW = K::TPW;
  const int K1P = D.k1max + P::EPV;
  T *xs = reinterpret_cast<T *>(smem);
  T *h1 = xs + SLAB * K1P;
  T *h2 = h1 + SLAB * HP;
  float *red = reinterpret_cast<float *>(h2 + SLAB * HP);

  STAMP(0, 0);
  pin_s(D.hT), pin_s(D.BP), pin_s(N.train_slot), pin_s(N.dropout), pin_s(N.b3), pin_s(N.out_dim);
  pin_s(N.out_col), pin_s(N.tanh_out), pin_s(N.out_pad), pin_s(out), pin_s(out_stride), pin_s(n_valid);
  issue();
  const int nk1 = N.k1pad / P::KM;
  const int nt3 = N.out_pad / 16;
  float bias1[TPW], bias2[TPW];
#pragma unroll
  for (int jj = 0; jj < TPW; ++jj) {
    bias1[jj] = ldg(N.b1 + 16 * (wave * TPW + jj) + r);
    bias2[jj] = ldg(N.b2 + 16 * (wave * TPW + jj) + r);
  }
  float bias3[2];
#pragma unroll
  for (int jt = 0; jt < 2; ++jt) bias3[jt] = ldg(N.b3 + (16 * jt + r < N.out_dim ? 16 * jt + r : N.out_dim - 1));
  uint4 w1[K::NK1][TPW], w2[K::NKC][TPW], w3[K::NK3][2];
  const T *W1 = reinterpret_cast<const T *>(N.w1c);
  const T *W2 = reinterpret_cast<const T *>(N.w2c);
  const T *W3 = reinterpret_cast<const T *>(N.w3c);
  load_w<P, K::NK1, TPW>(w1, W1, nk1, 0, nk1, wave * TPW, lane);
  load_w<P, K::NKC, TPW>(w2, W2, K::NK2, 0, K::NKC, wave * TPW, lane);
#pragma unroll
  for (int i = 0; i < K::NK3; ++i) {
    const int ks = wave + 4 * i;
#pragma unroll
    for (int jt = 0; jt < 2; ++jt)
      w3[i][jt] = ldg16(W3 + frag_off<P>(jt < nt3 ? jt : 0, ks < K::NK2 ? ks : 0, K::NK2, lane));
  }

  STAMP(0, 1);
  fill(xs, K1P);
  __syncthreads();
  STAMP(0, 2);

  {
    f32x4 acc[TPW];
#pragma unroll
    for (int jj = 0; jj < TPW; ++jj) acc[jj] = f32x4{0.f, 0.f, 0.f, 0.f};
    mma_w<P, K::NK1, TPW>(xs, K1P, 0, nk1, w1, acc, lane);
#pragma unroll
    for (int jj = 0; jj < TPW; ++jj) {
      const int col = 16 * (wave * TPW + jj) + r;
      const float bias = P::round(bias1[jj]);
      float v[4];
#pragma unroll
      for (int i = 0; i < 4; ++i) v[i] = fmaxf(P::round(acc[jj][i] + bias), 0.f);
      if (N.dropout) {
        bool keep[4];
        dropout_keep4(D, *Ap, step, 0, slab * 4 + q, col, keep);
#pragma unroll
        for (int i = 0; i < 4; ++i) v[i] = keep[i] ? P::round(v[i] * D.drop_scale) : 0.f;
      }
#pragma unroll
      for (int i = 0; i < 4; ++i) h1[(4 * q + i) * HP + col] = P::from_f32(v[i]);
      if (N.train_slot >= 0)
        store4T<BF16>(reinterpret_cast<T *>(D.hT) + (size_t)(N.train_slot * 2 + 0) * H * D.BP +
                          fidx<P>(col, slab * SLAB + 4 * q, D.BP / P::KM), v);
    }
  }
  __syncthreads();
  STAMP(0, 3);

  {
    f32x4 acc[TPW];
#pragma unroll
    for (int jj = 0; jj < TPW; ++jj) acc[jj] = f32x4{0.f, 0.f, 0.f, 0.f};
    mma_w<P, K::NKC, TPW>(h1, HP, 0, K::NKC, w2, acc, lane);
#pragma unroll 1
    for (int ch = 1; ch < K::NCH; ++ch) {
      load_w<P, K::NKC, TPW>(w2, W2, K::NK2, ch * K::NKC, K::NKC, wave * TPW, lane);
      mma_w<P, K::NKC, TPW>(h1, HP, ch * K::NKC * P::KM, K::NKC, w2, acc, lane);
    }
#pragma unroll
    for (int jj = 0; jj < TPW; ++jj) {
      const int col = 16 * (wave * TPW + jj) + r;
      const float bias = P::round(bias2[jj]);
      float v[4];
#pragma unroll
      for (int i = 0; i < 4; ++i) v[i] = fmaxf(P::round(acc[jj][i] + bias), 0.f);
      if (N.dropout) {
        bool keep[4];
        dropout_keep4(D, *Ap, step, 1, slab * 4 + q, col, keep);
#pragma unroll
        for (int i = 0; i < 4; ++i) v[i] = keep[i] ? P::round(v[i] * D.drop_scale) : 0.f;
      }
#pragma unroll
      for (int i = 0; i < 4; ++i) h2[(4 * q + i) * HP + col] = P::from_f32(v[i]);
      if (N.train_slot >= 0)
        store4T<BF16>(reinterpret_cast<T *>(D.hT) + (size_t)(N.train_slot * 2 + 1) * H * D.BP +
                          fidx<P>(col, slab * SLAB + 4 * q, D.BP / P::KM), v);
    }
  }
  __syncthreads();
  STAMP(0, 4);

  {
    f32x4 acc3[2] = {f32x4{0.f, 0.f, 0.f, 0.f}, f32x4{0.f, 0.f, 0.f, 0.f}};
#pragma unroll
    for (int i = 0; i < K::NK3; ++i) {
      const int ks = wave + 4 * i;
      if (ks < K::NK2) {
        const uint4 a = *reinterpret_cast<const uint4 *>(h2 + r * HP + ks * P::KM + P::EPV * q);
#pragma unroll
        for (int jt = 0; jt < 2; ++jt)
          if (jt < nt3) P::mma(a, w3[i][jt], acc3[jt]);
      }
    }
#pragma unroll
    for (int jt = 0; jt < 2; ++jt)
      *reinterpret_cast<f32x4 *>(red + ((wave * 2 + jt) * 64 + lane) * 4) = acc3[jt];
  }
  __syncthreads();
  if (wave == 0) {
#pragma unroll
    for (int jt = 0; jt < 2; ++jt) {
      if (jt < nt3) {
        f32x4 s = *reinterpret_cast<f32x4 *>(red + ((0 * 2 + jt) * 64 + lane) * 4);
#pragma unroll
        for (int w = 1; w < 4; ++w) s += *reinterpret_cast<f32x4 *>(red + ((w * 2 + jt) * 64 + lane) * 4);
        const int col = 16 * jt + r;
        if (col < N.out_dim) {
          const float bias = P::round(bias3[jt]);
#pragma unroll
          for (int i = 0; i < 4; ++i) {
            float v = P::round(s[i] + bias);
            if (N.tanh_out) v = P::round(tanhf(v));
            if (row0 + 4 * q + i < n_valid)
              stg(out + (size_t)(row0 + 4 * q + i) * out_stride + N.out_col + col, v);
          }
        }
      }
    }
  }
  STAMP(0, 5);
}

template <bool BF16>
__device__ __forceinline__ void stage_rows16(const TrainerDesc &D, const DevArgs &A, int64_t step, int row0,
                                             int row_step, int tid) {
  using P = Prec<BF16>;
  using T = typename P::T;
  const int rr = tid >> 4, l16 = tid & 15;
  const int B = D.B, nq = D.stage_stride >> 2, S = D.S, SA = D.S + D.A, nkb = D.BP / P::KM;
  T *const xT = reinterpret_cast<T *>(D.xT) + (size_t)(step & 1) * D.xrows * D.BP;
  for (int row = row0 + rr; row < B; row += row_step) {
    int64_t ix;
    if (A.idx_mode == 1)
      ix = ldg(A.idx + (size_t)(step - A.base_step) * B + row);
    else if (A.idx_mode == 2)
      ix = row;
    else
      ix = philox_index(D.seed, (uint64_t)step, (uint32_t)row, (uint64_t)A.n_rows);
    ix = ix < 0 ? 0 : (ix >= A.n_rows ? A.n_rows - 1 : ix);
    const float *src = A.rows + (size_t)ix * A.row_stride;
    float *dst = D.stage_rows + (size_t)row * D.stage_stride;
    for (int c = l16; c < nq; c += 16) {
      const float4 v4 = __builtin_bit_cast(float4, ldg16(src + 4 * c));
      stg16(dst + 4 * c, v4);
      const float v[4] = {v4.x, v4.y, v4.z, v4.w};
#pragma unroll
      for (int e = 0; e < 4; ++e) {
        const int col = 4 * c + e;
        if (col < SA) stg(xT + fidx<P>(col, row, nkb), P::from_f32(v[e]));
        if (col >= S && col < SA) stg(D.actf + (size_t)row * D.A + (col - S), v[e]);
        if (col >= SA && col < SA + 2) stg(D.rd + (size_t)row * 2 + (col - SA), v[e]);
      }
    }
  }
}

template <bool BF16>
__global__ __launch_bounds__(256) void k_stage(const TrainerDesc *__restrict__ Dp,
                                               const DevArgs *__restrict__ Ap,
                                               const DevCtr *__restrict__ Cp) {
  Dp += blockIdx.y, Ap += blockIdx.y, Cp += blockIdx.y;
  stage_rows16<BF16>(*Dp, *Ap, Cp->ctr[0], blockIdx.x * 16, gridDim.x * 16, threadIdx.x);
}

__device__ __forceinline__ void write_adam_coef(const TrainerDesc &D, const DevArgs &A, int64_t t1,
                                                AdamCoef *out);

template <bool BF16, int H>
struct FCfg {
  using P = Prec<BF16>;
  static constexpr int TPW = H / 64;
  static constexpr int SPL = TPW >= 4 ? 4 : TPW;
  static constexpr int HQ = H / SPL;
  static constexpr int NK2 = H / P::KM;
  static constexpr int NK3 = HQ / P::KM;
  static constexpr int NK1 = BF16 ? 4 : 8;
  static constexpr int HP = H + P::EPV;
  static constexpr int HQP = HQ + P::EPV;
  static_assert(HQ == 64, "one 16-column tile per wave and part");
};

template <bool BF16, int H, int MT, int PW>
__global__ __launch_bounds__(256, 3) void k_forward(const TrainerDesc *__restrict__ Dp,
                                                 const DevArgs *__restrict__ Ap,
                                                 const DevCtr *__restrict__ Cp, const int nsl_,
                                                 const int nfwd_) {
  using C = FCfg<BF16, H>;
  using P = Prec<BF16>;
  using T = typename P::T;
  constexpr int ROWS = 16 * MT, TPW = C::TPW, SPL = C::SPL, HP = C::HP, HQP = C::HQP;
  constexpr int NPG = SPL / PW;
  static_assert(SPL % PW == 0 && PW <= 2, "parts per work-group: 1 or 2, dividing the parts");
  Dp += blockIdx.y, Ap += blockIdx.y, Cp += blockIdx.y;
  const TrainerDesc &D = *Dp;
  const int idx_ = blockIdx.x >> 3;
  const int per_job = nsl_ * NPG;
  const int fnet = (idx_ / per_job) * 8 + (blockIdx.x & 7);
  const int rest = idx_ % per_job;
  const int slab = rest / NPG;
  const int part0 = __builtin_amdgcn_readfirstlane((rest % NPG) * PW);
  if (fnet > nfwd_) return;
  if (fnet == nfwd_) {
    if (rest == 0 && threadIdx.x == 0) {
      STAMP(0, 0);
      write_adam_coef(D, *Ap, Cp->ctr[0] + 1, const_cast<AdamCoef *>(&Cp->coef));
      const_cast<DevCtr *>(Cp)->coef_step = Cp->ctr[0] + 1;
      STAMP(0, 5);
    }
    if (rest == 0 && !D.deterministic && (int)threadIdx.x < D.A)
      stg(D.ls_snap + threadIdx.x, ldg(D.params + D.off_log_std + threadIdx.x));
    return;
  }
  const FwdNet N = D.fwd[fnet];
  const int B = D.B, BP = D.BP, OUTW = D.OUTW, k1max = D.k1max;
  const float *const stage = D.stage_rows;
  const unsigned sstride = (unsigned)D.stage_stride;
  float *const g_outs = D.outs;
  void *const g_hT = D.hT;
  const int64_t step = Cp->ctr[0];
  extern __shared__ __attribute__((aligned(16))) char smem[];
  const int tid = threadIdx.x, lane = tid & 63;
  const int wave = __builtin_amdgcn_readfirstlane(tid >> 6);
  const int r = lane & 15, q = lane >> 4;
  const int K1P = k1max + P::EPV;
  T *xs = reinterpret_cast<T *>(smem);
  T *h1 = xs + ROWS * K1P;
  T *h2 = h1 + ROWS * HP;
  STAMP(0, 0);

  const int rr = tid >> 4, l16 = tid & 15;
  const int lim4 = round_up(N.in_dim, 4) - 4;
  float4 xq[MT][2];
#pragma unroll
  for (int m = 0; m < MT; ++m) {
    const int row_ = slab * ROWS + 16 * m + rr;
    const unsigned row = (unsigned)(row_ < B ? row_ : B - 1);
    const float *src = stage + N.in_off;
#pragma unroll
    for (int j = 0; j < 2; ++j) {
      const int c = 4 * l16 + 64 * j;
      xq[m][j] = __builtin_bit_cast(float4, ldg16(src + (row * sstride + (unsigned)(c < lim4 ? c : lim4))));
    }
  }
  const int nk1 = N.k1pad / P::KM;
  const int nt3 = N.out_pad / 16;
  const int tile2 = part0 * 4 + wave;
  float bias1[TPW], bias3[2];
  {
    const float *b1w = N.b1 + 16 * (wave * TPW);
#pragma unroll
    for (int jj = 0; jj < TPW; ++jj) bias1[jj] = ldg(b1w + 16 * jj + r);
  }
  float bias2[PW];
#pragma unroll
  for (int j = 0; j < PW; ++j) bias2[j] = ldg(N.b2 + 16 * (tile2 + 4 * j) + r);
#pragma unroll
  for (int jt = 0; jt < 2; ++jt)
    bias3[jt] = ldg(N.b3 + (16 * jt + r < N.out_dim ? 16 * jt + r : N.out_dim - 1));
  uint4 w1[C::NK1][TPW], w2[PW][C::NK2], w3[PW][C::NK3][2];
  auto load_w2 = [&]() {
#pragma unroll
    for (int j = 0; j < PW; ++j) {
      const T *W2w = reinterpret_cast<const T *>(N.w2c) + (size_t)(tile2 + 4 * j) * C::NK2 * 64 * P::EPV;
#pragma unroll
      for (int ks = 0; ks < C::NK2; ++ks) w2[j][ks] = ldg16(W2w + ks * 64 * P::EPV + lane * P::EPV);
    }
  };
  auto load_w3 = [&]() {
#pragma unroll
    for (int j = 0; j < PW; ++j) {
      const T *W3w = reinterpret_cast<const T *>(N.w3c) + (size_t)((part0 + j) * C::NK3) * 64 * P::EPV;
#pragma unroll
      for (int ks = 0; ks < C::NK3; ++ks)
#pragma unroll
        for (int jt = 0; jt < 2; ++jt)
          if (jt < nt3) w3[j][ks][jt] = ldg16(W3w + (size_t)(jt * C::NK2 + ks) * 64 * P::EPV + lane * P::EPV);
    }
  };
  {
    const T *W1w = reinterpret_cast<const T *>(N.w1c) + (size_t)(wave * TPW) * nk1 * 64 * P::EPV;
#pragma unroll
    for (int ks = 0; ks < C::NK1; ++ks) {
      if (ks < nk1) {
#pragma unroll
        for (int jj = 0; jj < TPW; ++jj)
          w1[ks][jj] = ldg16(W1w + (size_t)(jj * nk1 + ks) * 64 * P::EPV + lane * P::EPV);
      }
    }
  }
  STAMP(0, 1);

#pragma unroll
  for (int m = 0; m < MT; ++m) {
#pragma unroll
    for (int j = 0; j < 2; ++j) {
      const int c = 4 * l16 + 64 * j;
      const float v[4] = {xq[m][j].x, xq[m][j].y, xq[m][j].z, xq[m][j].w};
      if (c < N.k1pad) {
        T tv[4];
#pragma unroll
        for (int e = 0; e < 4; ++e) tv[e] = P::from_f32(c + e < N.in_dim ? v[e] : 0.f);
        if constexpr (BF16) {
          uint2 u;
          u.x = (uint32_t)tv[0] | ((uint32_t)tv[1] << 16), u.y = (uint32_t)tv[2] | ((uint32_t)tv[3] << 16);
          *reinterpret_cast<uint2 *>(xs + (16 * m + rr) * K1P + c) = u;
        } else {
          *reinterpret_cast<float4 *>(xs + (16 * m + rr) * K1P + c) = make_float4(tv[0], tv[1], tv[2], tv[3]);
        }
      }
    }
  }
  __syncthreads();
  STAMP(0, 2);

  {
    f32x4 acc[MT][TPW];
#pragma unroll
    for (int m = 0; m < MT; ++m)
#pragma unroll
      for (int jj = 0; jj < TPW; ++jj) acc[m][jj] = f32x4{0.f, 0.f, 0.f, 0.f};
#pragma unroll
    for (int ks = 0; ks < C::NK1; ++ks) {
      if (ks < nk1) {
#pragma unroll
        for (int m = 0; m < MT; ++m) {
          const uint4 a = *reinterpret_cast<const uint4 *>(xs + (16 * m + r) * K1P + ks * P::KM + P::EPV * q);
#pragma unroll
          for (int jj = 0; jj < TPW; ++jj) P::mma(a, w1[ks][jj], acc[m][jj]);
        }
      }
    }
    __builtin_amdgcn_sched_barrier(0);
    load_w2();
    __builtin_amdgcn_sched_barrier(0);
    bool lean = false;
    if constexpr (BF16) lean = !N.dropout;
#pragma unroll
    for (int jj = 0; jj < TPW; ++jj) {
      const int tile = wave * TPW + jj;
      const int col = 16 * tile + r;
      const float bias = P::round(bias1[jj]);
      const bool mine = N.train_slot >= 0 && ((tile * SPL) / (4 * TPW)) / PW * PW == part0;
      if (lean) {
        if constexpr (BF16) {
          uint2 u[MT];
#pragma unroll
          for (int m = 0; m < MT; ++m) {
            u[m] = relu_bias_bf16x4(acc[m][jj], bias);
            T *hrow = h1 + (16 * m + 4 * q) * HP + col;
            hrow[0] = (T)(u[m].x & 0xffff), hrow[HP] = (T)(u[m].x >> 16);
            hrow[2 * HP] = (T)(u[m].y & 0xffff), hrow[3 * HP] = (T)(u[m].y >> 16);
          }
          T *plane = reinterpret_cast<T *>(g_hT) + (size_t)(N.train_slot * 2 + 0) * H * BP;
          if constexpr (MT == 2) {
            if (mine && slab * ROWS + ROWS <= B) {
#pragma unroll
              for (int m = 0; m < MT; m += 2) act_store16_pair(plane, col, slab * ROWS + 16 * m, q, BP / P::KM, u[m], u[m + 1]);
            }
          } else {
#pragma unroll
            for (int m = 0; m < MT; ++m)
              if (mine && slab * ROWS + 16 * m < B) act_store8_fwd(plane, fidx<P>(col, slab * ROWS + 16 * m + 4 * q, BP / P::KM), u[m]);
          }
        }
        continue;
      }
#pragma unroll
      for (int m = 0; m < MT; ++m) {
        const int row0 = slab * ROWS + 16 * m;
        float v[4];
#pragma unroll
        for (int i = 0; i < 4; ++i) v[i] = fmaxf(P::round(acc[m][jj][i] + bias), 0.f);
        if (N.dropout) {
          bool keep[4];
          dropout_keep4(D, *Ap, step, 0, (row0 >> 2) + q, col, keep);
#pragma unroll
          for (int i = 0; i < 4; ++i) v[i] = keep[i] ? P::round(v[i] * D.drop_scale) : 0.f;
        }
#pragma unroll
        for (int i = 0; i < 4; ++i) h1[(16 * m + 4 * q + i) * HP + col] = P::from_f32(v[i]);
        if (mine && row0 < B)
          store4T<BF16>(reinterpret_cast<T *>(g_hT) + (size_t)(N.train_slot * 2 + 0) * H * BP +
                            fidx<P>(col, row0 + 4 * q, BP / P::KM), v);
      }
    }
  }
  __syncthreads();
  STAMP(0, 3);

  {
    f32x4 acc[PW][MT];
#pragma unroll
    for (int j = 0; j < PW; ++j)
#pragma unroll
      for (int m = 0; m < MT; ++m) acc[j][m] = f32x4{0.f, 0.f, 0.f, 0.f};
#pragma unroll
    for (int ks = 0; ks < C::NK2; ++ks) {
#pragma unroll
      for (int m = 0; m < MT; ++m) {
        const uint4 a = *reinterpret_cast<const uint4 *>(h1 + (16 * m + r) * HP + ks * P::KM + P::EPV * q);
#pragma unroll
        for (int j = 0; j < PW; ++j) P::mma(a, w2[j][ks], acc[j][m]);
      }
    }
    __builtin_amdgcn_sched_barrier(0);
    load_w3();
    __builtin_amdgcn_sched_barrier(0);
    bool lean = false;
    if constexpr (BF16) lean = !N.dropout;
#pragma unroll
    for (int j = 0; j < PW; ++j) {
      const int col = 16 * (tile2 + 4 * j) + r;
      const float bias = P::round(bias2[j]);
      T *h2j = h2 + j * ROWS * HQP;
      if (lean) {
        if constexpr (BF16) {
          uint2 u[MT];
#pragma unroll
          for (int m = 0; m < MT; ++m) {
            u[m] = relu_bias_bf16x4(acc[j][m], bias);
            T *hrow = h2j + (16 * m + 4 * q) * HQP + 16 * wave + r;
            hrow[0] = (T)(u[m].x & 0xffff), hrow[HQP] = (T)(u[m].x >> 16);
            hrow[2 * HQP] = (T)(u[m].y & 0xffff), hrow[3 * HQP] = (T)(u[m].y >> 16);
          }
          T *plane = reinterpret_cast<T *>(g_hT) + (size_t)(N.train_slot * 2 + 1) * H * BP;
          if constexpr (MT == 2) {
            if (N.train_slot >= 0 && slab * ROWS + ROWS <= B) {
#pragma unroll
              for (int m = 0; m < MT; m += 2) act_store16_pair(plane, col, slab * ROWS + 16 * m, q, BP / P::KM, u[m], u[m + 1]);
            }
          } else {
#pragma unroll
            for (int m = 0; m < MT; ++m)
              if (N.train_slot >= 0 && slab * ROWS + 16 * m < B)
                act_store8_fwd(plane, fidx<P>(col, slab * ROWS + 16 * m + 4 * q, BP / P::KM), u[m]);
          }
        }
        continue;
      }
#pragma unroll
      for (int m = 0; m < MT; ++m) {
        const int row0 = slab * ROWS + 16 * m;
        float v[4];
#pragma unroll
        for (int i = 0; i < 4; ++i) v[i] = fmaxf(P::round(acc[j][m][i] + bias), 0.f);
        if (N.dropout) {
          bool keep[4];
          dropout_keep4(D, *Ap, step, 1, (row0 >> 2) + q, col, keep);
#pragma unroll
          for (int i = 0; i < 4; ++i) v[i] = keep[i] ? P::round(v[i] * D.drop_scale) : 0.f;
        }
#pragma unroll
        for (int i = 0; i < 4; ++i) h2j[(16 * m + 4 * q + i) * HQP + 16 * wave + r] = P::from_f32(v[i]);
        if (N.train_slot >= 0 && row0 < B)
          store4T<BF16>(reinterpret_cast<T *>(g_hT) + (size_t)(N.train_slot * 2 + 1) * H * BP +
                            fidx<P>(col, row0 + 4 * q, BP / P::KM), v);
      }
    }
  }
  __syncthreads();
  STAMP(0, 4);

  for (int pr = wave; pr < MT * PW; pr += 4) {
    const int m = pr % MT, j = pr / MT;
    const T *h2j = h2 + j * ROWS * HQP;
    f32x4 acc3[2] = {f32x4{0.f, 0.f, 0.f, 0.f}, f32x4{0.f, 0.f, 0.f, 0.f}};
#pragma unroll
    for (int ks = 0; ks < C::NK3; ++ks) {
      const uint4 a = *reinterpret_cast<const uint4 *>(h2j + (16 * m + r) * HQP + ks * P::KM + P::EPV * q);
#pragma unroll
      for (int jt = 0; jt < 2; ++jt) {
        if (jt < nt3) {
          if constexpr (PW == 1) {
            P::mma(a, w3[0][ks][jt], acc3[jt]);
          } else {
            if (j == 0) P::mma(a, w3[0][ks][jt], acc3[jt]);
            else P::mma(a, w3[PW - 1][ks][jt], acc3[jt]);
          }
        }
      }
    }
    float *outp = g_outs + (size_t)(part0 + j) * B * OUTW;
    const int row0 = slab * ROWS + 16 * m + 4 * q;
#pragma unroll
    for (int jt = 0; jt < 2; ++jt) {
      const int col = 16 * jt + r;
      if (jt < nt3 && col < N.out_dim && row0 < B) {
        const float bias = part0 + j == 0 ? P::round(bias3[jt]) : 0.f;
        outs_store4<false>(outp, (size_t)(N.out_col + col) * B + row0,
                           make_float4(acc3[jt][0] + bias, acc3[jt][1] + bias, acc3[jt][2] + bias, acc3[jt][3] + bias));
      }
    }
  }
  STAMP(0, 5);
}

template <int H, bool DROP>
__global__ __launch_bounds__(512, 1) void k_forward_tp(const TrainerDesc *__restrict__ Dp,
                                                        const DevArgs *__restrict__ Ap,
                                                        const DevCtr *__restrict__ Cp, const int nsl_,
                                                        const int nfwd_) {
  using C = FCfg<true, H>;
  using P = Prec<true>;
  using T = typename P::T;
  constexpr int ROWS = 64, MT = ROWS / 16, NW = 8;
  constexpr int TPW = H / (16 * NW);
  constexpr int SPL = C::SPL, HP = C::HP, NK2 = C::NK2, NK3 = C::NK3;
  static_assert(H == 256 && TPW == 2 && SPL == 4, "k_forward_tp is built for H = 256");
  Dp += blockIdx.y, Ap += blockIdx.y, Cp += blockIdx.y;
  const TrainerDesc &D = *Dp;
  const int idx_ = blockIdx.x >> 3;
  const int fnet = (idx_ / nsl_) * 8 + (blockIdx.x & 7);
  const int slab = idx_ % nsl_;
  if (fnet > nfwd_) return;
  if (fnet == nfwd_) {
    if (slab == 0 && threadIdx.x == 0) {
      STAMP(0, 0);
      write_adam_coef(D, *Ap, Cp->ctr[0] + 1, const_cast<AdamCoef *>(&Cp->coef));
      const_cast<DevCtr *>(Cp)->coef_step = Cp->ctr[0] + 1;
      STAMP(0, 5);
    }
    if (slab == 0 && !D.deterministic && (int)threadIdx.x < D.A)
      stg(D.ls_snap + threadIdx.x, ldg(D.params + D.off_log_std + threadIdx.x));
    return;
  }
  const FwdNet N = D.fwd[fnet];
  const int B = D.B, BP = D.BP, OUTW = D.OUTW, k1max = D.k1max;
  const float *const stage = D.stage_rows;
  const unsigned sstride = (unsigned)D.stage_stride;
  float *const g_outs = D.outs;
  void *const g_hT = D.hT;
  const int64_t step = Cp->ctr[0];
  extern __shared__ __attribute__((aligned(16))) char smem[];
  const int tid = threadIdx.x, lane = tid & 63;
  const int wave = __builtin_amdgcn_readfirstlane(tid >> 6);
  const int r = lane & 15, q = lane >> 4;
  const int K1P = k1max + P::EPV;
  T *xs = reinterpret_cast<T *>(smem);
  T *h1 = xs + ROWS * K1P;
  T *h2 = h1 + ROWS * HP;
  STAMP(0, 0);

  const int rr = tid >> 3, l8 = tid & 7;
  const int lim4 = round_up(N.in_dim, 4) - 4;
  float4 xq[4];
  {
    const int row_ = slab * ROWS + rr;
    const unsigned row = (unsigned)(row_ < B ? row_ : B - 1);
    const float *src = stage + N.in_off;
#pragma unroll
    for (int j = 0; j < 4; ++j) {
      const int c = 4 * l8 + 32 * j;
      xq[j] = __builtin_bit_cast(float4, ldg16(src + (row * sstride + (unsigned)(c < lim4 ? c : lim4))));
    }
  }
  const int nk1 = N.k1pad / P::KM;
  const int nt3 = N.out_pad / 16;
  const int tile0 = wave * TPW;
  const int part = tile0 / 4;
  float bias1[TPW], bias2[TPW], bias3[2];
#pragma unroll
  for (int jj = 0; jj < TPW; ++jj) {
    bias1[jj] = ldg(N.b1 + 16 * (tile0 + jj) + r);
    bias2[jj] = ldg(N.b2 + 16 * (tile0 + jj) + r);
  }
#pragma unroll
  for (int jt = 0; jt < 2; ++jt)
    bias3[jt] = ldg(N.b3 + (16 * jt + r < N.out_dim ? 16 * jt + r : N.out_dim - 1));
  uint4 w1[C::NK1][TPW], w2[TPW][NK2], w3[NK3][2];
  {
    const T *W1w = reinterpret_cast<const T *>(N.w1c) + (size_t)tile0 * nk1 * 64 * P::EPV;
#pragma unroll
    for (int ks = 0; ks < C::NK1; ++ks) {
      if (ks < nk1) {
#pragma unroll
        for (int jj = 0; jj < TPW; ++jj)
          w1[ks][jj] = ldg16(W1w + (size_t)(jj * nk1 + ks) * 64 * P::EPV + lane * P::EPV);
      }
    }
  }
  auto load_w23 = [&]() {
#pragma unroll
    for (int jj = 0; jj < TPW; ++jj) {
      const T *W2w = reinterpret_cast<const T *>(N.w2c) + (size_t)(tile0 + jj) * NK2 * 64 * P::EPV;
#pragma unroll
      for (int ks = 0; ks < NK2; ++ks) w2[jj][ks] = ldg16(W2w + ks * 64 * P::EPV + lane * P::EPV);
    }
    const T *W3w = reinterpret_cast<const T *>(N.w3c) + (size_t)(part * NK3) * 64 * P::EPV;
// ... 1240 lines not shown
      }
      uint4 xf[UKC][GNI], zf[UKC][GNB];
      auto issue = [&](const int k0, const int ks) {
        const int kk = k0 + ks < kend ? k0 + ks : kend - 1;
#pragma unroll
        for (int c = 0; c < GNI; ++c) xf[ks][c] = ldg16(xb[c] + (size_t)kk * 1024 + lane16);
#pragma unroll
        for (int b = 0; b < GNB; ++b) zf[ks][b] = ldg16(zb[b] + (size_t)kk * 1024 + lane16);
      };
      auto chunk = [&](const int k0, const bool first) {
#pragma unroll
        for (int ks = 0; ks < GIF; ++ks) issue(k0, ks);
        if (first) STAMP(2, 1);
#pragma unroll
        for (int ks = 0; ks < UKC; ++ks) {
          __builtin_amdgcn_sched_barrier(0);
          if (k0 + ks < kend) {
#pragma unroll
            for (int b = 0; b < GNB; ++b) {
              if (wave_bias) frag_acc<BF16>(bsum[b], zf[ks][b]);
#pragma unroll
              for (int c = 0; c < GNI; ++c) P::mma(xf[ks][c], zf[ks][b], acc[b][c]);
            }
          }
          __builtin_amdgcn_sched_barrier(0);
          if (ks + GIF < UKC) issue(k0, ks + GIF);
        }
      };
      chunk(kbeg, true);
#pragma unroll 1
      for (int k0 = kbeg + UKC; k0 < kend; k0 += UKC) chunk(k0, false);
      __builtin_amdgcn_sched_barrier(0);
      load_state();
      float *const tdst = half ? tile2 : tile;
#pragma unroll
      for (int b = 0; b < GNB; ++b)
#pragma unroll
        for (int c = 0; c < GNI; ++c)
          *reinterpret_cast<f32x4 *>(&tdst[(16 * GNB * gw + 16 * b + r) * ULD + 16 * c + 4 * q]) = acc[b][c];
      if (wave_bias) {
#pragma unroll
        for (int b = 0; b < GNB; ++b) {
          float bs = bsum[b];
          bs = xor32_sum(xor16_sum(bs));
          if (q == 0) (half ? bgrad2 : bgrad)[16 * GNB * gw + 16 * b + r] = bs;
        }
      }
    }
  }
  __syncthreads();
  STAMP(2, 3);

  T *wc = reinterpret_cast<T *>(it.wc);
  T *tc = reinterpret_cast<T *>(it.tc);
  const int nkw = Kw / P::KM;
#pragma unroll
  for (int ps = 0; ps < UNP; ++ps) {
    const int ol = tr + URPP * ps, o = o0 + ol, i = i0 + tc4;
    const float4 g4 = *reinterpret_cast<const float4 *>(&tile[ol * ULD + tc4]);
    float g[4] = {g4.x, g4.y, g4.z, g4.w};
    if constexpr (!LAT) {
      if (ksplit) {
        const float4 h4 = *reinterpret_cast<const float4 *>(&tile2[ol * ULD + tc4]);
        g[0] += h4.x, g[1] += h4.y, g[2] += h4.z, g[3] += h4.w;
      }
    }
    float p[4] = {pw[ps][0], pw[ps][1], pw[ps][2], pw[ps][3]};
    float m[4] = {mw[ps][0], mw[ps][1], mw[ps][2], mw[ps][3]};
    float v[4] = {vw[ps][0], vw[ps][1], vw[ps][2], vw[ps][3]};
    float tv[4] = {tw[ps][0], tw[ps][1], tw[ps][2], tw[ps][3]};
#pragma unroll
    for (int k = 0; k < 4; ++k) {
      g[k] = P::round(g[k]);
      adam_apply<BF16>(p[k], m[k], v[k], g[k], coef, neg_step);
      if (has_target) tv[k] = polyak(D, tv[k], p[k]);
    }
    if (L == 1) *reinterpret_cast<float4 *>(&tile[ol * ULD + tc4]) = make_float4(p[0], p[1], p[2], p[3]);
    const bool copies_from_lds = !LAT && L == 1;
    if (copies_from_lds && has_target)
      *reinterpret_cast<float4 *>(&tile2[ol * ULD + tc4]) = make_float4(tv[0], tv[1], tv[2], tv[3]);
    if (o < Odim && i < Idim) {
      const int64_t e = it.off_w + (int64_t)o * Idim + i;
      const int64_t te = it.toff_w + (int64_t)o * Idim + i;
      state_store(g_params, e, make_float4(p[0], p[1], p[2], p[3]));
      state_store(g_m, e, make_float4(m[0], m[1], m[2], m[3]));
      state_store(g_v, e, make_float4(v[0], v[1], v[2], v[3]));
      if (g_grads) stg16(g_grads + e, make_float4(g[0], g[1], g[2], g[3]));
      if (has_target) state_store(g_target, te, make_float4(tv[0], tv[1], tv[2], tv[3]));
      if (!copies_from_lds) {
        store4T<BF16>(wc + fidx<P>(o, i, nkw), p);
        if (has_target) store4T<BF16>(tc + fidx<P>(o, i, nkw), tv);
      }
      if (L == 2) {
        T *w3t = reinterpret_cast<T *>(it.w3t);
#pragma unroll
        for (int k = 0; k < 4; ++k) stg(w3t + (size_t)(i + k) * Opad + o, P::from_f32(p[k]));
      }
    }
  }
  STAMP(2, 5);
  if (do_bias && tid < UTO && o0 + tid < Odim) {
    const int64_t e = it.off_b + o0 + tid;
    float gb = bgrad[tid];
    if constexpr (!LAT) {
      if (ksplit) gb += bgrad2[tid];
    }
    const float g = P::round(gb);
    adam_apply<BF16>(pb, mb, vb, g, coef, neg_step);
    stg(g_params + e, pb), stg(g_m + e, mb), stg(g_v + e, vb);
    if (g_grads) stg(g_grads + e, g);
    if (has_target) stg(g_target + it.toff_b + o0 + tid, polyak(D, tb, pb));
  }
  STAMP(2, 6);
  if (L == 1) {
    __syncthreads();
    if constexpr (!LAT) {
      static_assert(LAT || (UT == 256 && UTO == 64 && UTI == 32), "one pass of 8-element stores covers the tile");
      {
        const int ol = tid >> 2, c8 = (tid & 3) * 8;
        const float4 a0 = *reinterpret_cast<const float4 *>(&tile[ol * ULD + c8]);
        const float4 a1 = *reinterpret_cast<const float4 *>(&tile[ol * ULD + c8 + 4]);
        const float pv8[8] = {a0.x, a0.y, a0.z, a0.w, a1.x, a1.y, a1.z, a1.w};
        copy_store8<BF16>(wc, fidx<P>(o0 + ol, i0 + c8, nkw), fidx<P>(o0 + ol, i0 + c8 + 4, nkw), pv8);
        if (has_target) {
          const float4 t0 = *reinterpret_cast<const float4 *>(&tile2[ol * ULD + c8]);
          const float4 t1 = *reinterpret_cast<const float4 *>(&tile2[ol * ULD + c8 + 4]);
          const float tv8[8] = {t0.x, t0.y, t0.z, t0.w, t1.x, t1.y, t1.z, t1.w};
          copy_store8<BF16>(tc, fidx<P>(o0 + ol, i0 + c8, nkw), fidx<P>(o0 + ol, i0 + c8 + 4, nkw), tv8);
        }
      }
      {
        const int il = tid & (UTI - 1), o8 = (tid >> 5) * 8;
        float pv8[8];
#pragma unroll
        for (int k = 0; k < 8; ++k) pv8[k] = tile[(o8 + k) * ULD + il];
        copy_store8<BF16>(reinterpret_cast<T *>(it.w2ct), fidx<P>(i0 + il, o0 + o8, H / P::KM),
                          fidx<P>(i0 + il, o0 + o8 + 4, H / P::KM), pv8);
      }
      STAMP(2, 4);
      return;
    }
#pragma unroll
    for (int ps = 0; ps < (UTO / 4) / (UT / UTI); ++ps) {
      const int il = tid & (UTI - 1), o4 = ((tid >> 5) + (UT / UTI) * ps) * 4;
      float pv4[4];
#pragma unroll
      for (int k = 0; k < 4; ++k) pv4[k] = tile[(o4 + k) * ULD + il];
      store4T<BF16>(reinterpret_cast<T *>(it.w2ct) + fidx<P>(i0 + il, o0 + o4, H / P::KM), pv4);
    }
  }
  STAMP(2, 4);
}

template <bool BF16, int H, bool PRE, int PW, bool NV = false>
__global__ __launch_bounds__(256, PRE ? 1 : (PW > 1 ? (BF16 ? 4 : 2) : (BF16 ? 6 : 3)))
void k_backward(const TrainerDesc *__restrict__ Dp, const DevArgs *__restrict__ Ap, DevCtr *__restrict__ Cp,
                const int nslab, const int ntrain) {
  extern __shared__ __attribute__((aligned(16))) char smem[];
  backward_body<BF16, H, PRE, PW, NV>(Dp + blockIdx.y, Ap + blockIdx.y, Cp + blockIdx.y, (int)blockIdx.x, smem, nslab,
                                      ntrain);
}

template <bool BF16, bool LAT>
__global__ __launch_bounds__(LAT ? 512 : 256, LAT ? 2 : (BF16 ? 4 : 3)) void k_update(const TrainerDesc *__restrict__ Dp,
                                                             const DevArgs *__restrict__ Ap,
                                                             DevCtr *__restrict__ Cp,
                                                             const UpdItem *__restrict__ items, int n_items) {
  if ((int)blockIdx.x > n_items) return;
  update_body<BF16, LAT, (LAT ? 512 : 256)>(Dp + blockIdx.y, Ap + blockIdx.y, Cp + blockIdx.y,
                         items + (size_t)blockIdx.y * n_items, n_items, (int)blockIdx.x);
}

template <bool BF16>
__global__ void k_sync_weights(const TrainerDesc *__restrict__ Dp) {
  const TrainerDesc &D = *Dp;
  using P = Prec<BF16>;
  using T = typename P::T;
  const int net = blockIdx.y;
  if (net >= D.ntrain) return;
  const TrainNet &N = D.net[net];
  const int H = D.H;
  for (int L = 0; L < 3; ++L) {
    const int Odim = (L == 2) ? N.out_dim : H;
    const int Idim = (L == 0) ? N.in_dim : H;
    const int Kw = (L == 0) ? N.k1pad : H;
    const int total = Odim * Idim;
    for (int e = blockIdx.x * blockDim.x + threadIdx.x; e < total; e += gridDim.x * blockDim.x) {
      const int o = e / Idim, i = e - o * Idim;
      const float p = ldg(D.params + N.off_w[L] + e);
      stg(reinterpret_cast<T *>(N.wc[L]) + fidx<P>(o, i, Kw / P::KM), P::from_f32(p));
      if (L == 1) stg(reinterpret_cast<T *>(N.w2ct) + fidx<P>(i, o, H / P::KM), P::from_f32(p));
      if (L == 2) stg(reinterpret_cast<T *>(N.w3t) + (size_t)i * N.out_pad + o, P::from_f32(p));
      if (N.has_target)
        stg(reinterpret_cast<T *>(N.tc[L]) + fidx<P>(o, i, Kw / P::KM),
            P::from_f32(ldg(D.target + N.toff_w[L] + e)));
    }
  }
}

size_t infer_smem_bytes(bool bf16, int H, int k1max) {
  const int es = bf16 ? 2 : 4, epv = bf16 ? 8 : 4;
  return (size_t)SLAB * (k1max + epv) * es + 2 * (size_t)SLAB * (H + epv) * es + 4 * 2 * 64 * 4 * 4;
}
size_t fwd_smem_bytes(bool bf16, int H, int k1max, int mt, int pw) {
  const int es = bf16 ? 2 : 4, epv = bf16 ? 8 : 4;
  return (size_t)16 * mt * ((k1max + epv) + (H + epv) + pw * (64 + epv)) * es;
}
size_t bwd_smem_bytes(bool bf16, int H) {
  const int es = bf16 ? 2 : 4, epv = bf16 ? 8 : 4;
  return (size_t)SLAB * (H + epv) * es + 3 * SLAB * 32 * 4 + SLAB * 4 + SLAB * FIN_LD * 4;
}
int fwd_row_tiles(int B, int n_seeds) {
  const int64_t rows = (int64_t)B * n_seeds;
  if (rows >= 512 && B % 32 == 0) return 2;
  return 1;
}
int layer2_parts(int H) { return H >= 256 ? 4 : H / 64; }
int fwd_parts_per_wg(int B, int H, int n_seeds) {
  return ((int64_t)B * n_seeds >= 1024 && layer2_parts(H) % 2 == 0) ? 2 : 1;
}

#define DISPATCH_H(BF, HH, CALL)                 \
  do {                                           \
    if (BF) {                                    \
      if (HH == 256) { CALL(true, 256); }        \
      else if (HH == 128) { CALL(true, 128); }   \
      else { CALL(true, 64); }                   \
    } else {                                     \
      if (HH == 256) { CALL(false, 256); }       \
      else if (HH == 128) { CALL(false, 128); }  \
      else { CALL(false, 64); }                  \
    }                                            \
  } while (0)

bool use_tp(bool bf16, const TrainerDesc &D, int n_seeds, bool backward) {
  if (!bf16 || D.H != 256 || D.B % 64 != 0) return false;
  const int64_t fwd_wgs = (int64_t)D.nfwd * (D.B / 64) * n_seeds, bwd_wgs = (int64_t)D.ntrain * (D.B / 32) * n_seeds;
  const bool fwd_tp = fwd_wgs >= 72 && fwd_wgs <= 256;
  return backward ? (fwd_tp && bwd_wgs >= 144 && bwd_wgs <= 256) : fwd_tp;
}
hipError_t prepare_step_kernels() {
  hipError_t e = hipFuncSetAttribute(reinterpret_cast<const void *>(k_forward_tp<256, false>),
                                     hipFuncAttributeMaxDynamicSharedMemorySize, 160 * 1024);
  if (e != hipSuccess) return e;
  return hipFuncSetAttribute(reinterpret_cast<const void *>(k_forward_tp<256, true>),
                             hipFuncAttributeMaxDynamicSharedMemorySize, 160 * 1024);
}
size_t fwd_tp_smem_bytes(int H, int k1max) { return (size_t)64 * ((k1max + 8) + 2 * (H + 8)) * 2; }
size_t bwd_smem_bytes(bool bf16, int H);

hipError_t launch_forward(bool bf16, const TrainerDesc &D, const TrainerDesc *dD, const DevArgs *a,
                          const DevCtr *c, int n_seeds, hipStream_t st) {
  if (use_tp(bf16, D, n_seeds, false)) {
    const int nsl64 = D.B / 64;
    const int grid = 8 * ((D.nfwd + 1 + 7) / 8) * nsl64;
    if (D.has_dropout)
      hipLaunchKernelGGL((k_forward_tp<256, true>), dim3(grid, n_seeds), dim3(512), fwd_tp_smem_bytes(256, D.k1max), st,
                         dD, a, c, nsl64, D.nfwd);
    else
      hipLaunchKernelGGL((k_forward_tp<256, false>), dim3(grid, n_seeds), dim3(512), fwd_tp_smem_bytes(256, D.k1max), st,
                         dD, a, c, nsl64, D.nfwd);
    return hipGetLastError();
  }
  const int mt = fwd_row_tiles(D.B, n_seeds), nsl = (D.B + 16 * mt - 1) / (16 * mt);
  const int pw = fwd_parts_per_wg(D.B, D.H, n_seeds);
  const int grid = 8 * ((D.nfwd + 1 + 7) / 8) * nsl * (layer2_parts(D.H) / pw);
  const size_t sm = fwd_smem_bytes(bf16, D.H, D.k1max, mt, pw);
#define LAUNCH_F(BF, HH, MTV, PWV)                                                                            \
  hipLaunchKernelGGL((k_forward<BF, HH, MTV, PWV>), dim3(grid, n_seeds), dim3(256), sm, st, dD, a, c, nsl, D.nfwd)
#define CALL(BF, HH)                                                   \
  do {                                                                 \
    if constexpr (HH >= 128) {                                         \
      if (pw == 2) {                                                   \
        if (mt == 2) LAUNCH_F(BF, HH, 2, 2);                           \
        else LAUNCH_F(BF, HH, 1, 2);                                   \
        break;                                                         \
      }                                                                \
    }                                                                  \
    if (mt == 2) LAUNCH_F(BF, HH, 2, 1);                               \
    else LAUNCH_F(BF, HH, 1, 1);                                       \
  } while (0)
  DISPATCH_H(bf16, D.H, CALL);
#undef CALL
#undef LAUNCH_F
  return hipGetLastError();
}
int bwd_parts_per_wg(int B, int H, int n_seeds) {
  return ((int64_t)B * n_seeds >= 512 && layer2_parts(H) % 2 == 0) ? 2 : 1;
}
hipError_t launch_backward(bool bf16, const TrainerDesc &D, const TrainerDesc *dD, const DevArgs *a,
                           DevCtr *c, int n_seeds, hipStream_t st, bool counts) {
  if (use_tp(bf16, D, n_seeds, true)) {
    const int nslab32 = D.B / 32;
    const int nxn = (D.ntrain <= 4 && nslab32 % 2 == 0) ? 2 : 1;
    const int grid = 8 * ((D.ntrain * nxn + 7) / 8) * (nslab32 / nxn);
    hipLaunchKernelGGL((k_backward_tp<256>), dim3(grid, n_seeds), dim3(512), 2 * bwd_smem_bytes(true, 256), st, dD, a, c,
                       nslab32, D.ntrain, nxn);
    return hipGetLastError();
  }
  const int pw = bwd_parts_per_wg(D.B, D.H, n_seeds);
  const int grid = 8 * ((layer2_parts(D.H) / pw * D.ntrain + 7) / 8) * (D.B / SLAB);
  const size_t sm = bwd_smem_bytes(bf16, D.H);
  const bool pre = (int64_t)D.B * n_seeds < 1024;
#define LAUNCH_B(BF, HH, PRE_, PW_)                                                                          \
  hipLaunchKernelGGL((k_backward<BF, HH, PRE_, PW_>), dim3(grid, n_seeds), dim3(256), sm, st, dD, a, c, D.B / SLAB, \
                     D.ntrain)
#define CALL(BF, HH)                                                  \
  do {                                                                \
    if constexpr (HH >= 128) {                                        \
      if (pw == 2) { LAUNCH_B(BF, HH, false, 2); break; }             \
    }                                                                 \
    if (pre) LAUNCH_B(BF, HH, true, 1);                               \
    else LAUNCH_B(BF, HH, false, 1);                                  \
  } while (0)
  if (counts && !bf16) {
#define LAUNCH_V(HH, PRE_, PW_)                                                                                      \
  hipLaunchKernelGGL((k_backward<false, HH, PRE_, PW_, true>), dim3(grid, n_seeds), dim3(256), sm, st, dD, a, c, D.B / SLAB, \
                     D.ntrain)
#define CALL_V(HH)                                                    \
  do {                                                                \
    if constexpr (HH >= 128) {                                        \
      if (pw == 2) { LAUNCH_V(HH, false, 2); break; }                 \
    }                                                                 \
    if (pre) LAUNCH_V(HH, true, 1);                                   \
    else LAUNCH_V(HH, false, 1);                                      \
  } while (0)
    if (D.H == 256) CALL_V(256);
    else if (D.H == 128) CALL_V(128);
    else CALL_V(64);
#undef CALL_V
#undef LAUNCH_V
    return hipGetLastError();
  }
  DISPATCH_H(bf16, D.H, CALL);
#undef CALL
#undef LAUNCH_B
  return hipGetLastError();
}
hipError_t launch_stage(bool bf16, const TrainerDesc &D, const TrainerDesc *dD, const DevArgs *a,
                        const DevCtr *c, int n_seeds, hipStream_t st) {
  if (bf16)
    hipLaunchKernelGGL(k_stage<true>, dim3((D.B + 15) / 16, n_seeds), dim3(256), 0, st, dD, a, c);
  else
    hipLaunchKernelGGL(k_stage<false>, dim3((D.B + 15) / 16, n_seeds), dim3(256), 0, st, dD, a, c);
  return hipGetLastError();
}
int strip_rows() { return USR; }
int update_lds_floats() { return UPD_LDS; }
hipError_t launch_update(bool bf16, const TrainerDesc *dD, const DevArgs *a, DevCtr *c,
                         const UpdItem *items, int n_items, int n_seeds, hipStream_t st) {
  const dim3 grid(n_seeds > 1 ? round_up(n_items + 1, 8) : n_items + 1, n_seeds);
  static const int cus = [] {
    int dev = 0, n = 256;
    if (hipGetDevice(&dev) != hipSuccess || hipDeviceGetAttribute(&n, hipDeviceAttributeMultiprocessorCount, dev) != hipSuccess)
      n = 256;
    return n;
  }();
  const bool lat = n_seeds == 1 && n_items + 1 <= cus + 1;
  if (bf16 && !lat)
    hipLaunchKernelGGL((k_update<true, false>), grid, dim3(256), 0, st, dD, a, c, items, n_items);
  else if (bf16)
    hipLaunchKernelGGL((k_update<true, true>), grid, dim3(512), 0, st, dD, a, c, items, n_items);
  else if (!lat)
    hipLaunchKernelGGL((k_update<false, false>), grid, dim3(256), 0, st, dD, a, c, items, n_items);
  else
    hipLaunchKernelGGL((k_update<false, true>), grid, dim3(512), 0, st, dD, a, c, items, n_items);
  return hipGetLastError();
}
hipError_t launch_infer(bool bf16, const TrainerDesc &D, const TrainerDesc *dD, const FwdNet &N,
                        const float *s, const float *a, int64_t n, float *out, int out_stride,
                        hipStream_t st) {
  const int grid = (int)((n + SLAB - 1) / SLAB);
  const size_t sm = infer_smem_bytes(bf16, D.H, D.k1max);
#define CALL(BF, HH) \
  hipLaunchKernelGGL((k_infer<BF, HH>), dim3(grid), dim3(256), sm, st, dD, N, s, a, n, out, out_stride)
  DISPATCH_H(bf16, D.H, CALL);
#undef CALL
  return hipGetLastError();
}
hipError_t launch_sync_weights(bool bf16, const TrainerDesc *dD, hipStream_t st) {
  if (bf16)
    hipLaunchKernelGGL(k_sync_weights<true>, dim3(32, MAX_TRAIN), dim3(256), 0, st, dD);
  else
    hipLaunchKernelGGL(k_sync_weights<false>, dim3(32, MAX_TRAIN), dim3(256), 0, st, dD);
  return hipGetLastError();
}

}
```

iqlpref_amd/iql.py:

```python
import copy
import ctypes as C
import math
import os
import random
import uuid
from dataclasses import asdict, dataclass, fields
from typing import Any, Callable, Dict, List, Optional, Tuple, Union

import numpy as np
import torch
import torch.nn as nn
from torch.distributions import Normal
from torch.optim.lr_scheduler import CosineAnnealingLR

from . import _lib
from ._lib import PREC_BF16, PREC_FP32, check, ptr, stream_ptr

TensorBatch = List[torch.Tensor]

EXP_ADV_MAX = 100.0
LOG_STD_MIN = -20.0
LOG_STD_MAX = 2.0


# ... 438 lines not shown
        crit = q_network.critics()
        self._n_critics = E = len(crit)
        self._nets = [(f"q{e + 1}", _linears(c, f"TwinQ.q{e + 1}")) for e, c in enumerate(crit)]
        self._nets += [("v", _linears(v_network.v, "ValueFunction")),
                       ("actor", _linears(actor.net, "actor"))]
        self._state_dim = self._nets[E][1][0].in_features
        self._action_dim = self._nets[E + 1][1][-1].out_features
        self._hidden = self._nets[E][1][0].out_features
        self._n_hidden = len(self._nets[E][1]) - 1
        for _, lin in self._nets:
            if len(lin) != self._n_hidden + 1:
                raise NotImplementedError("all networks must have the same number of hidden layers")
            if any(l.out_features != self._hidden for l in lin[:-1]) or \
                    any(l.in_features != self._hidden for l in lin[1:]):
                raise NotImplementedError("all hidden layers must share one width")
        if self._nets[0][1][0].in_features != self._state_dim + self._action_dim:
            raise ValueError("TwinQ input width must be state_dim + action_dim")
        self._dropout = actor.net._dropout
        for p in list(q_network.parameters()) + list(v_network.parameters()) + list(actor.parameters()):
            if p.device.type != "cuda":
                raise ValueError("networks must live on the trainer's device before construction")
        self._build_arenas()
        self.q_target = copy.deepcopy(self.qf).requires_grad_(False).to(device)
        self._bind_target()

    def _cfg(self, batch_size: int) -> _lib.TrainerConfig:
        g = lambda opt, k: opt.param_groups[0][k]
        for opt in (self.q_optimizer, self.v_optimizer, self.actor_optimizer):
            if not isinstance(opt, torch.optim.Adam) or g(opt, "weight_decay") != 0 or g(opt, "amsgrad") \
                    or g(opt, "maximize"):
                raise NotImplementedError("optimisers must be plain torch.optim.Adam "
                                          "(no weight decay / amsgrad / maximize)")
        b1, b2 = g(self.q_optimizer, "betas")
        for opt in (self.v_optimizer, self.actor_optimizer):
            if tuple(g(opt, "betas")) != (b1, b2) or g(opt, "eps") != g(self.q_optimizer, "eps"):
                raise NotImplementedError("the three Adam optimisers must share betas and eps")
        c = _lib.TrainerConfig()
        c.state_dim, c.action_dim, c.hidden_dim = self._state_dim, self._action_dim, self._hidden
        c.batch_size = batch_size
        c.deterministic = int(self._deterministic)
        c.precision = self._precision
        c.dropout_p = -1.0 if not self._dropout else float(self._dropout)
        c.discount, c.tau, c.beta, c.iql_tau = self.discount, self.tau, self.beta, self.iql_tau
        c.lr_q = float(g(self.q_optimizer, "lr"))
        c.lr_v = float(g(self.v_optimizer, "lr"))
        c.lr_actor = float(self.actor_lr_schedule.base_lrs[0])
        c.adam_beta1, c.adam_beta2, c.adam_eps = b1, b2, float(g(self.q_optimizer, "eps"))
        c.cosine_t_max = int(self.actor_lr_schedule.T_max)
        c.seed = self._seed
        c.n_critics = self._n_critics
        c.polyak_form = self._polyak_form
        c.n_hidden = self._n_hidden
        return c

    def _tensor_list(self) -> List[nn.Parameter]:
        out = []
        for _, lin in self._nets:
            for l in lin:
                out += [l.weight, l.bias]
        if not self._deterministic:
            out.append(self.actor.log_std)
        return out

    def _build_arenas(self):
        cfg = self._cfg(32)
        offs = (C.c_int64 * _lib.N_TENSORS)()
        n_params, n_target = C.c_int64(), C.c_int64()
        check(self._lib.iqlhip_arena_layout(C.byref(cfg), C.byref(offs), C.byref(n_params),
                                            C.byref(n_target)))
        self._offsets = [int(o) for o in offs]
        self._n_params, self._n_target = n_params.value, n_target.value
        dev = self._dev
        z = lambda n: torch.zeros(n, dtype=torch.float32, device=dev)
        self._params, self._exp_avg, self._exp_avg_sq = z(self._n_params), z(self._n_params), z(self._n_params)
        self._target = z(self._n_target)
        self._grads = z(self._n_params) if self._keep_grads else None
        tensors = self._tensor_list()
        offsets = [o for o in self._offsets if o >= 0]
        assert len(tensors) == len(offsets)
        self._views = []
        with torch.no_grad():
            for p, o in zip(tensors, offsets):
                view = self._params[o:o + p.numel()].view(p.shape)
                view.copy_(p.data)
                p.data = view
                self._views.append((p, o))
                if self._grads is not None:
                    p.grad = self._grads[o:o + p.numel()].view(p.shape)

    def _bind_target(self):
        tl = []
        for mlp in self.q_target.critics():
            for l in mlp.linears():
                tl += [l.weight, l.bias]
        with torch.no_grad():
            for p, o in zip(tl, self._offsets[:2 * (self._n_hidden + 1) * self._n_critics]):
                view = self._target[o:o + p.numel()].view(p.shape)
                view.copy_(p.data)
                p.data = view

    def _bind_optimizer_state(self, rebuild: bool = False):
        steps = getattr(self, "_step_tensors", None)
        if steps is None or rebuild:
            steps = []
            for p, o in self._views:
                for opt in (self.q_optimizer, self.v_optimizer, self.actor_optimizer):
                    if any(p is q for q in opt.param_groups[0]["params"]):
                        st = opt.state[p]
                        st["step"] = torch.tensor(float(self.total_it))
                        st["exp_avg"] = self._exp_avg[o:o + p.numel()].view(p.shape)
                        st["exp_avg_sq"] = self._exp_avg_sq[o:o + p.numel()].view(p.shape)
                        steps.append(st["step"])
            self._step_tensors = steps
            return
        t = float(self.total_it)
        for st in steps:
            st.fill_(t)

    def _ensure_handle(self, batch_size: int):
        if self._handle is not None and self._handle_batch == batch_size:
            return
        self._destroy_handle()
        cfg = self._cfg(batch_size)
        ar = _lib.Arenas(ptr(self._params), ptr(self._exp_avg), ptr(self._exp_avg_sq),
                         ptr(self._target), ptr(self._grads))
        h = C.c_void_p()
        with torch.cuda.device(self._dev):
            check(self._lib.iqlhip_trainer_create(C.byref(h), C.byref(cfg), C.byref(ar)))
            self._handle, self._handle_batch = h, batch_size
            check(self._lib.iqlhip_trainer_set_step(h, self.total_it))
            check(self._lib.iqlhip_trainer_sync_weights(h, stream_ptr()))

    def _destroy_handle(self):
        if getattr(self, "_handle", None) is not None:
            owner = getattr(self, "_group_owner", None)
            if owner is not None:
                owner._drop_group()
            torch.cuda.synchronize(self._dev)
            self._lib.iqlhip_trainer_destroy(self._handle)
            self._handle = None

    def __del__(self):
        try:
            self._destroy_handle()
        except Exception:
            pass

    def step_kind(self, batch_size: int) -> str:
        self._ensure_handle(batch_size)
        kind = C.c_int32()
        check(self._lib.iqlhip_trainer_step_kind(self._handle, C.byref(kind)))
        return "general" if kind.value else "tuned"

    def sync_weights(self):
        if self._handle is not None:
            with torch.cuda.device(self._dev):
                check(self._lib.iqlhip_trainer_sync_weights(self._handle, stream_ptr()))

    def _after_steps(self, n: int):
        self.total_it += n
        sch = self.actor_lr_schedule
        lr = sch.eta_min + (sch.base_lrs[0] - sch.eta_min) * (1 + math.cos(math.pi * self.total_it / sch.T_max)) / 2
        sch.last_epoch = self.total_it
        sch._step_count = self.total_it + 1
        sch._last_lr = [lr]
        self.actor_optimizer.param_groups[0]["lr"] = lr
        self._bind_optimizer_state()

    def launch_counts(self):
        if self._handle is None:
            return (0, 0)
        eager, graphs = C.c_int64(), C.c_int64()
        check(self._lib.iqlhip_trainer_launch_counts(self._handle, C.byref(eager), C.byref(graphs)))
        return (int(eager.value), int(graphs.value))

    def _check_keep(self, keep: torch.Tensor, n_steps: int, batch_size: int) -> torch.Tensor:
        want = (n_steps, self._n_hidden, batch_size, self._hidden)
        if tuple(keep.shape) != want:
            raise ValueError(f"dropout_keep must have shape {want} (n_steps, n_hidden, batch_size, hidden_dim), "
                             f"got {tuple(keep.shape)}")
        if keep.device.type != "cuda":
            raise ValueError("dropout_keep must be a device tensor")
        return keep.to(torch.uint8).contiguous()

    def _refresh_lrs(self):
        lrs = (self._handle.value, float(self.q_optimizer.param_groups[0]["lr"]),
               float(self.v_optimizer.param_groups[0]["lr"]), float(self.actor_lr_schedule.base_lrs[0]))
        if lrs != getattr(self, "_lrs_sent", None):
            check(self._lib.iqlhip_trainer_set_lr(self._handle, *lrs[1:]))
            self._lrs_sent = lrs

    def train(self, batch: TensorBatch, dropout_keep: Optional[torch.Tensor] = None) -> Dict[str, float]:
        s, a, r, s2, d = [t.detach().to(torch.float32).contiguous() for t in batch]
        if a.shape != (s.shape[0], self._action_dim):
            raise RuntimeError("Actions shape missmatch")
        self._ensure_handle(s.shape[0])
        self._refresh_lrs()
        if dropout_keep is not None:
            if dropout_keep.dim() == 3:
                dropout_keep = dropout_keep[None]
            dropout_keep = self._check_keep(dropout_keep, 1, s.shape[0])
        losses = torch.empty(3, dtype=torch.float32, device=self._dev)
        with torch.cuda.device(self._dev):
            check(self._lib.iqlhip_train_batch(self._handle, ptr(s), ptr(a), ptr(r), ptr(s2), ptr(d),
                                               ptr(dropout_keep), ptr(losses), stream_ptr()))
        self._after_steps(1)
        v, q, p = losses.tolist()
        return {"value_loss": v, "q_loss": q, "actor_loss": p}

    def train_steps(self, replay_buffer: ReplayBuffer, n_steps: int, batch_size: int, *,
                    indices: Optional[torch.Tensor] = None,
                    dropout_keep: Optional[torch.Tensor] = None,
                    return_losses: bool = True, graph_unroll: Optional[int] = None,
                    n_valid: Optional[torch.Tensor] = None):
        self._ensure_handle(batch_size)
        self._refresh_lrs()
        losses = (torch.empty((n_steps, 3), dtype=torch.float32, device=self._dev)
                  if return_losses else None)
        if indices is not None:
            if indices.dtype != torch.int64 or tuple(indices.shape) != (n_steps, batch_size):
                raise ValueError("indices must be int64 [n_steps, batch_size]")
            indices = indices.contiguous()
        if dropout_keep is not None:
            dropout_keep = self._check_keep(dropout_keep, n_steps, batch_size)
        v = replay_buffer.view()
        unroll = self._graph_unroll if graph_unroll is None else graph_unroll
        if n_valid is not None:
            if n_valid.dtype != torch.int32 or tuple(n_valid.shape) != (n_steps,) or n_valid.device.type != "cuda":
                raise ValueError("n_valid must be an int32 device tensor [n_steps]")
            n_valid = n_valid.contiguous()
            with torch.cuda.device(self._dev):
                check(self._lib.iqlhip_train_steps_valid(self._handle, C.byref(v), n_steps, ptr(indices), ptr(n_valid),
                                                         ptr(dropout_keep), ptr(losses), unroll, stream_ptr()))
        elif torch.cuda.current_device() == (self._dev.index or 0):
            check(self._lib.iqlhip_train_steps(self._handle, C.byref(v), n_steps, ptr(indices),
                                               ptr(dropout_keep), ptr(losses), unroll, stream_ptr()))
        else:
            with torch.cuda.device(self._dev):
                check(self._lib.iqlhip_train_steps(self._handle, C.byref(v), n_steps, ptr(indices),
                                                   ptr(dropout_keep), ptr(losses), unroll, stream_ptr()))
        self._after_steps(n_steps)
        return losses

    def state_dict(self) -> Dict[str, Any]:
        torch.cuda.synchronize(self._dev)
        if self.total_it > 0:
            self._bind_optimizer_state(rebuild=True)
        return {
            "qf": self.qf.state_dict(),
            "q_optimizer": self.q_optimizer.state_dict(),
            "vf": self.vf.state_dict(),
            "v_optimizer": self.v_optimizer.state_dict(),
            "actor": self.actor.state_dict(),
            "actor_optimizer": self.actor_optimizer.state_dict(),
            "actor_lr_schedule": self.actor_lr_schedule.state_dict(),
            "total_it": self.total_it,
        }

    def load_state_dict(self, state_dict: Dict[str, Any]):
        torch.cuda.synchronize(self._dev)
        strip = lambda sd: {k.removeprefix("_orig_mod."): v for k, v in sd.items()}
        self.qf.load_state_dict(strip(state_dict["qf"]))
        self.q_optimizer.load_state_dict(state_dict["q_optimizer"])
        self.vf.load_state_dict(strip(state_dict["vf"]))
        self.v_optimizer.load_state_dict(state_dict["v_optimizer"])
        self.actor.load_state_dict(strip(state_dict["actor"]))
        self.actor_optimizer.load_state_dict(state_dict["actor_optimizer"])
        self.actor_lr_schedule.load_state_dict(state_dict["actor_lr_schedule"])
        self.total_it = state_dict["total_it"]
        with torch.no_grad():
            self._exp_avg.zero_()
            self._exp_avg_sq.zero_()
            for p, o in self._views:
                for opt in (self.q_optimizer, self.v_optimizer, self.actor_optimizer):
                    st = opt.state.get(p)
                    if st and "exp_avg" in st:
                        self._exp_avg[o:o + p.numel()].copy_(st["exp_avg"].reshape(-1))
                        self._exp_avg_sq[o:o + p.numel()].copy_(st["exp_avg_sq"].reshape(-1))
            self._target.copy_(self._params[:self._n_target])
        self._bind_optimizer_state(rebuild=True)
        if self._handle is not None:
            with torch.cuda.device(self._dev):
                check(self._lib.iqlhip_trainer_set_step(self._handle, self.total_it))
        self.sync_weights()

    def forward(self, which: str, states: torch.Tensor, actions: Optional[torch.Tensor] = None):
        idx = {"q": 0, "v": 1, "actor": 2, "q_target": 3}[which]
        self._ensure_handle(self._handle_batch or 32)
        s = states.detach().to(torch.float32).contiguous()
        a = None if actions is None else actions.detach().to(torch.float32).contiguous()
        width = {0: self._n_critics, 1: 1, 2: self._action_dim, 3: self._n_critics}[idx]
        out = torch.empty((s.shape[0], width), dtype=torch.float32, device=self._dev)
        with torch.cuda.device(self._dev):
            check(self._lib.iqlhip_forward(self._handle, idx, ptr(s), ptr(a), s.shape[0], ptr(out),
                                           stream_ptr()))
        return out
```

Before: 67030 steps/s.

## Fuse backward pass into update kernel for two-launch bf16 H=256 B=256 steps

Adds a fused path for the common bf16, hidden 256, batch 256 configuration. Each step becomes forward plus a single fused update kernel that recomputes layer gradients from ReLU bitmasks written by forward and from double-buffered copies of the transposed weights. This removes the separate backward launch and its global round trip of activation gradients. In exchange it adds extra weight copies written by the update kernel, ping-pong staging buffers, a large-LDS kernel, and weight-copy memcpys whenever the step counter does not line up.

```diff
diff --git a/include/iqlhip.h b/include/iqlhip.h
--- a/include/iqlhip.h
+++ b/include/iqlhip.h
@@ -102,6 +102,10 @@
 int iqlhip_trainer_destroy(iqlhip_trainer *t);
 
 int iqlhip_trainer_step_kind(iqlhip_trainer *t, int32_t *kind);
+
+int iqlhip_trainer_step_launches(iqlhip_trainer *t, int32_t batch);
+int iqlhip_two_launch_rule(int32_t bf16, int32_t hidden_dim, int32_t batch, int32_t actor_dropout,
+                           int32_t n_items, int32_t n_cus);
 
 int iqlhip_trainer_sync_weights(iqlhip_trainer *t, void *stream);
 
diff --git a/iqlpref_amd/_lib.py b/iqlpref_amd/_lib.py
--- a/iqlpref_amd/_lib.py
+++ b/iqlpref_amd/_lib.py
@@ -116,6 +116,8 @@
     "iqlhip_trainer_create": (C.c_int, [C.POINTER(P), C.POINTER(TrainerConfig), C.POINTER(Arenas)]),
     "iqlhip_trainer_destroy": (C.c_int, [P]),
     "iqlhip_trainer_step_kind": (C.c_int, [P, C.POINTER(C.c_int32)]),
+    "iqlhip_trainer_step_launches": (C.c_int, [P, C.c_int32]),
+    "iqlhip_two_launch_rule": (C.c_int, [C.c_int32] * 6),
     "iqlhip_trainer_sync_weights": (C.c_int, [P, P]),
     "iqlhip_trainer_set_step": (C.c_int, [P, C.c_int64]),
     "iqlhip_trainer_get_step": (C.c_int, [P, C.POINTER(C.c_int64), C.POINTER(C.c_double)]),
diff --git a/iqlpref_amd/csrc/api.hip b/iqlpref_amd/csrc/api.hip
--- a/iqlpref_amd/csrc/api.hip
+++ b/iqlpref_amd/csrc/api.hip
@@ -29,11 +29,12 @@
 hipError_t deep_infer(DeepTrainer *, int which, const float *s, const float *a, int64_t n, float *out, hipStream_t);
 int layer2_parts(int H);
 hipError_t launch_forward(bool, const TrainerDesc &, const TrainerDesc *, const DevArgs *, const DevCtr *,
-                          int n_seeds, hipStream_t);
+                          int n_seeds, hipStream_t, bool fused = false);
 hipError_t launch_backward(bool, const TrainerDesc &, const TrainerDesc *, const DevArgs *, DevCtr *,
                            int n_seeds, hipStream_t, bool counts = false);
 hipError_t launch_stage(bool, const TrainerDesc &, const TrainerDesc *, const DevArgs *, const DevCtr *,
-                        int n_seeds, hipStream_t);
+                        int n_seeds, hipStream_t, bool fused = false);
+hipError_t launch_update_fused(const TrainerDesc *, const DevArgs *, DevCtr *, const UpdItem *, int, hipStream_t);
 int strip_rows();
 int update_lds_floats();
 hipError_t launch_update(bool, const TrainerDesc *, const DevArgs *, DevCtr *, const UpdItem *, int,
@@ -269,7 +270,7 @@
   bool dev_args_valid = false;
   hipGraphExec_t gexec = nullptr;
   int graph_unroll = 0;
-  bool graph_counts = false;
+  int graph_counts = 0;
   hipStream_t cap_stream = nullptr;
   Throttle throttle;
   bool timing = false;
@@ -298,7 +299,7 @@
     gexec = nullptr;
   }
   template <typename Step>
-  int ensure_graph(int U, bool counts, Step step) {
+  int ensure_graph(int U, int counts, Step step) {
     if (gexec && graph_unroll == U && graph_counts == counts) return 0;
     drop_graph();
     hipGraph_t g = nullptr;
@@ -431,6 +432,9 @@
   int64_t total_it = 0;
   double lr_q, lr_v, lr_a_base;
   StepQueue queue;
+  bool fused_ok = false;
+  int64_t alt_step = -1;
+  void *w2x[MAX_TRAIN][2] = {}, *w3x[MAX_TRAIN][2] = {};
 };
 
 static_assert(MAX_CRITICS == IQLHIP_MAX_CRITICS, "iql_step.h and iqlhip.h disagree");
@@ -605,6 +609,18 @@
       col.swap(out);
     }
   }
+}
+
+extern "C" int iqlhip_two_launch_rule(int32_t bf16, int32_t hidden_dim, int32_t batch, int32_t actor_dropout,
+                                      int32_t n_items, int32_t n_cus) {
+  return (bf16 && hidden_dim == 256 && batch == 256 && !actor_dropout && n_items + 1 <= n_cus) ? 2 : 3;
+}
+
+static int device_cus() {
+  int dev = 0, n = 256;
+  if (hipGetDevice(&dev) != hipSuccess || hipDeviceGetAttribute(&n, hipDeviceAttributeMultiprocessorCount, dev) != hipSuccess)
+    n = 256;
+  return n;
 }
 
 extern "C" int iqlhip_trainer_create(iqlhip_trainer **out, const iqlhip_trainer_config *cfg,
@@ -691,7 +707,11 @@
     }
     add((size_t)H * H * es);
     add((size_t)H * outpad[n] * es);
-  }
+    for (int c = 0; c < 2; ++c) add((size_t)H * H * es), add((size_t)H * outpad[n] * es);
+  }
+  add((size_t)NT * B * (H / 32 + 1) * 4);
+  add((size_t)2 * B * 2 * 4);
+  add((size_t)2 * B * A * 4);
   add((size_t)2 * D.xrows * D.BP * es);
   add((size_t)B * 2 * 4);
   add((size_t)B * A * 4);
@@ -768,7 +788,14 @@
     }
     N.w2ct = carve<char>(p, (size_t)H * H * es);
     N.w3t = carve<char>(p, (size_t)H * outpad[n] * es);
-  }
+    for (int c = 0; c < 2; ++c) {
+      t->w2x[n][c] = carve<char>(p, (size_t)H * H * es);
+      t->w3x[n][c] = carve<char>(p, (size_t)H * outpad[n] * es);
+    }
+  }
+  D.m2 = carve<uint32_t>(p, (size_t)NT * B * (H / 32 + 1));
+  D.rd2 = carve<float>(p, (size_t)2 * B * 2);
+  D.actf2 = carve<float>(p, (size_t)2 * B * A);
   D.xT = carve<char>(p, (size_t)2 * D.xrows * D.BP * es);
   D.rd = carve<float>(p, (size_t)B * 2);
   D.actf = carve<float>(p, (size_t)B * A);
@@ -785,6 +812,8 @@
   D.stage_stride = stride;
   D.next_off = iqlhip_replay_next_offset(S, A);
   D.prefetch = !getenv("IQLHIP_NO_PREFETCH") ? 1 : 0;
+  t->fused_ok = !getenv("IQLHIP_STEP3") &&
+                iqlhip_two_launch_rule(t->bf16, H, B, D.has_dropout, (int)n_slots, device_cus()) == 2;
   t->own_dargs = t->dargs = carve<DevArgs>(p, 1);
   t->own_dctr = t->dctr = carve<DevCtr>(p, 1);
   t->own_ddesc = t->ddesc = carve<TrainerDesc>(p, 1);
@@ -804,6 +833,8 @@
 
     it.wc = N.wc[L], it.tc = N.has_target ? N.tc[L] : nullptr, it.w2ct = (L == 1) ? N.w2ct : nullptr;
     it.w3t = (L == 2) ? N.w3t : nullptr;
+    it.nout = N.out_dim, it.nopad = N.out_pad;
+    for (int c = 0; c < 2; ++c) it.w2x[c] = t->w2x[it.net][c], it.w3x[c] = t->w3x[it.net][c];
     const size_t plane = (size_t)H * D.BP * es;
     it.Xsrc = (L == 0) ? D.xT : reinterpret_cast<char *>(D.hT) + (size_t)(it.net * 2 + (L - 1)) * plane;
     it.Zsrc = (L == 0)   ? reinterpret_cast<char *>(D.dz1T) + (size_t)it.net * plane
@@ -867,6 +898,11 @@
   return 0;
 }
 
+extern "C" int iqlhip_trainer_step_launches(iqlhip_trainer *t, int32_t batch) {
+  if (!t) return fail(IQLHIP_ERR_INVALID, "null trainer");
+  return (!t->deep && t->fused_ok && !t->group && batch == t->cfg.batch_size) ? 2 : 3;
+}
+
 extern "C" int iqlhip_trainer_step_kind(iqlhip_trainer *t, int32_t *kind) {
   if (!t || !kind) return fail(IQLHIP_ERR_INVALID, "null argument");
   *kind = t->deep ? 1 : 0;
@@ -880,6 +916,7 @@
     return 0;
   }
   HIP_TRY(launch_sync_weights(t->bf16, t->ddesc, (hipStream_t)stream));
+  t->alt_step = -1;
   return 0;
 }
 
@@ -887,6 +924,7 @@
   if (!t || total_it < 0) return fail(IQLHIP_ERR_INVALID, "bad argument");
   HIP_TRY(hipDeviceSynchronize());
   t->total_it = total_it;
+  t->alt_step = -1;
   if (t->deep) return 0;
   DevCtr c;
   memset(&c, 0, sizeof(c));
@@ -944,11 +982,20 @@
   DevCtr *ctr;
   const UpdItem *items;
   int n_items, K;
+  bool fused = false;
 };
 
 static int enqueue_step(const StepTarget &x, bool counts, hipStream_t st, hipEvent_t *ev) {
-  if (!x.D.prefetch) HIP_TRY(launch_stage(x.bf16, x.D, x.desc, x.args, x.ctr, x.K, st));
+  if (!x.D.prefetch) HIP_TRY(launch_stage(x.bf16, x.D, x.desc, x.args, x.ctr, x.K, st, x.fused));
   if (ev) HIP_TRY(hipEventRecord(ev[0], st));
+  if (x.fused) {
+    HIP_TRY(launch_forward(x.bf16, x.D, x.desc, x.args, x.ctr, 1, st, true));
+    if (ev) HIP_TRY(hipEventRecord(ev[1], st));
+    if (ev) HIP_TRY(hipEventRecord(ev[2], st));
+    HIP_TRY(launch_update_fused(x.desc, x.args, x.ctr, x.items, x.n_items, st));
+    if (ev) HIP_TRY(hipEventRecord(ev[3], st));
+    return 0;
+  }
   HIP_TRY(launch_forward(x.bf16, x.D, x.desc, x.args, x.ctr, x.K, st));
   if (ev) HIP_TRY(hipEventRecord(ev[1], st));
   HIP_TRY(launch_backward(x.bf16, x.D, x.desc, x.args, x.ctr, x.K, st, counts));
@@ -967,12 +1014,12 @@
   }
   if (!same) {
     if (int rc = q.push(want, x.K, x.args, st)) return rc;
-    if (x.D.prefetch) HIP_TRY(launch_stage(x.bf16, x.D, x.desc, x.args, x.ctr, x.K, st));
+    if (x.D.prefetch) HIP_TRY(launch_stage(x.bf16, x.D, x.desc, x.args, x.ctr, x.K, st, x.fused));
   }
   q.dev_args_valid = all_philox;
   int64_t done = 0;
   if (!q.timing && graph_unroll > 0 && n_steps >= graph_unroll) {
-    if (int rc = q.ensure_graph(graph_unroll, counts, [&](hipStream_t cs) { return enqueue_step(x, counts, cs, nullptr); }))
+    if (int rc = q.ensure_graph(graph_unroll, (counts ? 1 : 0) | (x.fused ? 2 : 0), [&](hipStream_t cs) { return enqueue_step(x, counts, cs, nullptr); }))
       return rc;
     if (int rc = q.replay(done, n_steps, st)) return rc;
   }
@@ -1093,8 +1140,22 @@
     return deep_run({tr, 1, &t->deep_ring, deep_desc_dev(t->deep), t->queue}, &a, a.n_steps, graph_unroll, st);
   }
   if (t->group) group_invalidate(t->group);
-  const StepTarget x = {t->bf16, t->D, t->ddesc, t->dargs, t->dctr, t->ditems, t->n_items, 1};
-  return run_tuned(t->queue, x, &a, a.n_steps, graph_unroll, counts, st);
+  StepTarget x = {t->bf16, t->D, t->ddesc, t->dargs, t->dctr, t->ditems, t->n_items, 1};
+  x.fused = t->fused_ok && !t->group && !counts;
+  if (x.fused && t->alt_step != t->total_it) {
+    const int rp = (int)((t->total_it + 1) & 1), es = 2, H = t->D.H;
+    for (int n = 0; n < t->D.ntrain; ++n) {
+      HIP_TRY(hipMemcpyAsync(t->w2x[n][rp], t->D.net[n].w2ct, (size_t)H * H * es, hipMemcpyDeviceToDevice, st));
+      HIP_TRY(hipMemcpyAsync(t->w3x[n][rp], t->D.net[n].w3t, (size_t)H * t->D.net[n].out_pad * es, hipMemcpyDeviceToDevice, st));
+    }
+    t->queue.dev_args_valid = false;
+  }
+  if (int rc = run_tuned(t->queue, x, &a, a.n_steps, graph_unroll, counts, st)) {
+    t->alt_step = -1;
+    return rc;
+  }
+  t->alt_step = x.fused ? t->total_it + a.n_steps : -1;
+  return 0;
 }
 
 extern "C" int iqlhip_train_steps(iqlhip_trainer *t, const iqlhip_replay_view *view, int64_t n_steps,
diff --git a/iqlpref_amd/csrc/iql_fused.h b/iqlpref_amd/csrc/iql_fused.h
--- /dev/null
+++ b/iqlpref_amd/csrc/iql_fused.h
@@ -0,0 +1,685 @@
+
+constexpr int FU_T = 512;
+constexpr int FU_B = 256, FU_H = 256;
+constexpr int FU_NK = FU_B / 32;
+constexpr int FU_DLD = FU_B + 8;
+constexpr int FU_DZ3_BYTES = 32 * FU_DLD * 2;
+constexpr int FU_OFF_DZ3 = 32 * 1024;
+constexpr int FU_OFF_FIN = 49 * 1024 + 512;
+constexpr int FU_MAX_SLOTS = 3 + MAX_CRITICS + 2 * 32;
+constexpr int FU_OFF_LS = FU_OFF_FIN + FU_MAX_SLOTS * 1024;
+constexpr int FU_DYN_BYTES = 128 * 1024;
+static_assert(FU_OFF_DZ3 + FU_DZ3_BYTES <= FU_OFF_FIN && FU_OFF_LS + 128 <= FU_DYN_BYTES, "LDS map");
+static_assert(FU_DZ3_BYTES <= UPD_LDS * 4 && UPD_TILE * 4 >= USR * FU_B * 2, "strips: dz3 / dZ1^T inside the tile array");
+static_assert(FU_NK == UKC && USR == 16 && UTO == 64 && UTI == 32, "tile geometry of update_body");
+
+__device__ __forceinline__ float fu_lo(uint32_t w) { return __builtin_bit_cast(float, w << 16); }
+__device__ __forceinline__ float fu_hi(uint32_t w) { return __builtin_bit_cast(float, w & 0xffff0000u); }
+__device__ __forceinline__ void fu_unpack8(const uint4 &g, float (&v)[8]) {
+  v[0] = fu_lo(g.x), v[1] = fu_hi(g.x), v[2] = fu_lo(g.y), v[3] = fu_hi(g.y);
+  v[4] = fu_lo(g.z), v[5] = fu_hi(g.z), v[6] = fu_lo(g.w), v[7] = fu_hi(g.w);
+}
+
+struct FuSlots {
+  int lo, hi, mean, act;
+};
+__device__ __forceinline__ FuSlots fu_slots(const TrainerDesc &D, int net) {
+  FuSlots s;
+  const bool is_q = net < D.E, is_a = net == D.net_a;
+  s.mean = 3 + D.E, s.act = 3 + D.E + D.A;
+  s.lo = is_q ? 0 : 2;
+  s.hi = is_q ? 2 : (is_a ? s.act + D.A : s.mean);
+  return s;
+}
+
+template <int CH>
+struct FuFin {
+  float pv[CH][4];
+};
+template <int CH>
+__device__ __forceinline__ void fu_fin_issue(FuFin<CH> &f, const TrainerDesc &D, const FuSlots &sl, int net, int s0,
+                                             int hh, int row, const float *g_outs, const float *g_act) {
+  const unsigned plane = (unsigned)D.OUTW * FU_B;
+#pragma unroll
+  for (int c = 0; c < CH; ++c) {
+    int s = s0 + 2 * c + hh;
+    s = s < sl.hi ? s : sl.hi - 1;
+    const bool isact = s >= sl.act;
+    const int col = s == 0 ? D.out_nv : (s == 1 ? net : (s < 2 + D.E ? D.out_qt + s - 2 : (s == 2 + D.E ? D.out_v : D.out_mean + (s - sl.mean))));
+    const float *base = isact ? g_act + (s - sl.act) : g_outs + (unsigned)col * FU_B;
+    const unsigned ps = isact ? 0u : plane;
+    const unsigned lo = isact ? (unsigned)row * (unsigned)D.A : (unsigned)row;
+#pragma unroll
+    for (int p = 0; p < 4; ++p) f.pv[c][p] = ldg(base + (p * ps + lo));
+  }
+}
+template <int CH>
+__device__ __forceinline__ void fu_fin_finish(const FuFin<CH> &f, const FuSlots &sl, int s0, int hh, int row, float *fin) {
+#pragma unroll
+  for (int c = 0; c < CH; ++c) {
+    const int s = s0 + 2 * c + hh;
+    if (s < sl.hi) {
+      float v;
+      if (s >= sl.act) {
+        v = f.pv[c][0];
+      } else {
+        float sum = f.pv[c][0];
+#pragma unroll
+        for (int p = 1; p < 4; ++p) sum += f.pv[c][p];
+        v = Prec<true>::round(sum);
+        if (s >= sl.mean) v = Prec<true>::round(tanhf(v));
+      }
+      fin[s * FU_B + row] = v;
+    }
+  }
+}
+
+__device__ __forceinline__ void fu_lossin(LossIn &lin, const TrainerDesc &D, int net, const float *fin, int row, float rew,
+                                          float done) {
+  const bool is_q = net < D.E;
+#pragma unroll
+  for (int e = 0; e < MAX_CRITICS; ++e) lin.qt[e] = is_q ? 0.f : fin[(2 + (e < D.E ? e : 0)) * FU_B + row];
+  lin.vv = is_q ? 0.f : fin[(2 + D.E) * FU_B + row];
+  lin.nv = is_q ? fin[row] : 0.f;
+  lin.qv = is_q ? fin[FU_B + row] : 0.f;
+  lin.rew = rew, lin.done = done;
+  lin.mean = 0.f, lin.act = 0.f, lin.ls = 0.f;
+}
+
+template <int JN>
+__device__ __forceinline__ void fu_tile_panel(char *panel, const uint16_t *dz3b, const uint16_t *w3x, int opad, int o0,
+                                              const uint4 (&h2f)[4], int ks, int lane) {
+  const int r = lane & 15, q = lane >> 4;
+  constexpr int NG = (JN + 7) / 8;
+  uint4 wq[4][NG];
+#pragma unroll
+  for (int ot = 0; ot < 4; ++ot)
+#pragma unroll
+    for (int g = 0; g < NG; ++g) wq[ot][g] = ldg16(w3x + (size_t)(o0 + 16 * ot + r) * opad + 8 * g);
+  float s[4][8];
+#pragma unroll
+  for (int ot = 0; ot < 4; ++ot)
+#pragma unroll
+    for (int e = 0; e < 8; ++e) s[ot][e] = 0.f;
+#pragma unroll
+  for (int j = 0; j < JN; ++j) {
+    float dv[8];
+    fu_unpack8(*reinterpret_cast<const uint4 *>(dz3b + j * FU_DLD + 32 * ks + 8 * q), dv);
+#pragma unroll
+    for (int ot = 0; ot < 4; ++ot) {
+      const uint4 &g = wq[ot][j / 8];
+      const uint32_t wds[4] = {g.x, g.y, g.z, g.w};
+      const uint32_t wd = wds[(j % 8) >> 1];
+      const float w = (j & 1) ? fu_hi(wd) : fu_lo(wd);
+#pragma unroll
+      for (int e = 0; e < 8; ++e) s[ot][e] = __builtin_fmaf(dv[e], w, s[ot][e]);
+    }
+    if ((j & 3) == 3) __builtin_amdgcn_sched_barrier(0);
+  }
+#pragma unroll
+  for (int ot = 0; ot < 4; ++ot) {
+    float hv[8], t[8];
+    fu_unpack8(h2f[ot], hv);
+#pragma unroll
+    for (int e = 0; e < 8; ++e) t[e] = hv[e] > 0.f ? s[ot][e] : 0.f;
+    *reinterpret_cast<uint4 *>(panel + ((ot * FU_NK + ks) * 64 + lane) * 16) =
+        make_uint4(pk_bf16(t[0], t[1]), pk_bf16(t[2], t[3]), pk_bf16(t[4], t[5]), pk_bf16(t[6], t[7]));
+  }
+}
+
+template <int JN, int UN>
+__device__ __forceinline__ void fu_strip_panel(char *panel, const uint16_t *dz3b, const uint16_t *w3x, int opad,
+                                               const uint32_t *m2net, int ks, int lane) {
+  const int r = lane & 15, q = lane >> 4;
+  constexpr int NG = (JN + 7) / 8;
+#pragma unroll 1
+  for (int u0 = 0; u0 < 8; u0 += UN) {
+    float wf[UN][JN];
+#pragma unroll
+    for (int e = 0; e < UN; ++e) {
+#pragma unroll
+      for (int g = 0; g < NG; ++g) {
+        const uint4 w8 = ldg16(w3x + (size_t)(32 * ks + 8 * q + u0 + e) * opad + 8 * g);
+        float wv[8];
+        fu_unpack8(w8, wv);
+#pragma unroll
+        for (int k = 0; k < 8; ++k)
+          if (8 * g + k < JN) wf[e][8 * g + k] = wv[k];
+      }
+    }
+    uint32_t sa = ldg(m2net + (size_t)r * (FU_H / 32) + ks), sb = ldg(m2net + (size_t)(16 + r) * (FU_H / 32) + ks);
+#pragma unroll 1
+    for (int mp = 0; mp < FU_B / 32; ++mp) {
+      const int mn = mp + 1 < FU_B / 32 ? mp + 1 : mp;
+      const uint32_t na = ldg(m2net + (size_t)(32 * mn + r) * (FU_H / 32) + ks);
+      const uint32_t nb = ldg(m2net + (size_t)(32 * mn + 16 + r) * (FU_H / 32) + ks);
+      float s0[UN], s1[UN];
+#pragma unroll
+      for (int e = 0; e < UN; ++e) s0[e] = 0.f, s1[e] = 0.f;
+#pragma unroll
+      for (int j = 0; j < JN; ++j) {
+        const float da = bf2f(dz3b[j * FU_DLD + 32 * mp + r]), db = bf2f(dz3b[j * FU_DLD + 32 * mp + 16 + r]);
+#pragma unroll
+        for (int e = 0; e < UN; ++e) {
+          s0[e] = __builtin_fmaf(da, wf[e][j], s0[e]);
+          s1[e] = __builtin_fmaf(db, wf[e][j], s1[e]);
+        }
+        if ((j & 7) == 7) __builtin_amdgcn_sched_barrier(0);
+      }
+      const uint32_t ba = sa >> (8 * q + u0), bb = sb >> (8 * q + u0);
+      uint32_t pa[UN / 2], pb[UN / 2];
+#pragma unroll
+      for (int e = 0; e < UN; e += 2) {
+        pa[e / 2] = pk_bf16((ba >> e) & 1 ? s0[e] : 0.f, (ba >> (e + 1)) & 1 ? s0[e + 1] : 0.f);
+        pb[e / 2] = pk_bf16((bb >> e) & 1 ? s1[e] : 0.f, (bb >> (e + 1)) & 1 ? s1[e + 1] : 0.f);
+      }
+      char *fa = panel + (((2 * mp) * FU_NK + ks) * 64 + lane) * 16 + 2 * u0;
+      char *fb = panel + (((2 * mp + 1) * FU_NK + ks) * 64 + lane) * 16 + 2 * u0;
+      if constexpr (UN == 8) {
+        *reinterpret_cast<uint4 *>(fa) = make_uint4(pa[0], pa[1], pa[2], pa[3]);
+        *reinterpret_cast<uint4 *>(fb) = make_uint4(pb[0], pb[1], pb[2], pb[3]);
+      } else {
+        static_assert(UN == 4, "8 or 4 units per pass");
+        *reinterpret_cast<uint2 *>(fa) = make_uint2(pa[0], pa[1]);
+        *reinterpret_cast<uint2 *>(fb) = make_uint2(pb[0], pb[1]);
+      }
+      sa = na, sb = nb;
+    }
+  }
+}
+
+#define FU_DISPATCH_JN(out_dim, CALL)      \
+  do {                                     \
+    if ((out_dim) == 1) { CALL(1, 8); }    \
+    else if ((out_dim) <= 8) { CALL(8, 8); }   \
+    else if ((out_dim) <= 16) { CALL(16, 4); } \
+    else { CALL(32, 4); }                  \
+  } while (0)
+
+__global__ __launch_bounds__(FU_T, 1) void k_update_fused(const TrainerDesc *__restrict__ Dp,
+                                                          const DevArgs *__restrict__ Ap, DevCtr *__restrict__ Cp,
+                                                          const UpdItem *__restrict__ items, int n_items) {
+  using P = Prec<true>;
+  using T = uint16_t;
+  constexpr int UT = FU_T, H = FU_H, B = FU_B, BP = FU_B, nk = FU_NK;
+  const TrainerDesc &D = *Dp;
+  const DevArgs &A = *Ap;
+  const int blk = blockIdx.x;
+  const int tid = threadIdx.x, lane = tid & 63;
+  const int wave = __builtin_amdgcn_readfirstlane(tid >> 6);
+  const int r = lane & 15, q = lane >> 4;
+  const int row = tid & (B - 1);
+  const int hh = __builtin_amdgcn_readfirstlane(tid >> 8);
+  const UpdItem it = items[blk < n_items ? blk : n_items - 1];
+  const int64_t t1 = Cp->coef_step;
+  const AdamCoef coef = Cp->coef;
+  float *const g_params = D.params, *const g_m = D.exp_avg, *const g_v = D.exp_avg_sq;
+  float *const g_target = D.target, *const g_grads = D.grads;
+  const float *const g_outs = D.outs;
+  const int par = (int)(t1 & 1);
+  const float *const g_rd = D.rd2 + (size_t)(par ^ 1) * B * 2;
+  const float *const g_act = D.actf2 + (size_t)(par ^ 1) * B * D.A;
+  const float *const g_ls = D.ls_snap;
+  const T *const g_hT = reinterpret_cast<const T *>(D.hT);
+  const uint32_t *const g_m2 = D.m2;
+
+  extern __shared__ __attribute__((aligned(16))) char dyn[];
+  __shared__ __attribute__((aligned(16))) float lds_upd[UPD_LDS];
+  __shared__ float bgrad[UTO];
+  float *const tile = lds_upd, *const tile2 = lds_upd + UPD_TILE;
+  float *const fin = reinterpret_cast<float *>(dyn + FU_OFF_FIN);
+  float *const lsl = reinterpret_cast<float *>(dyn + FU_OFF_LS);
+  STAMP(2, 0);
+
+  if (blk >= n_items) {
+    const int nt = D.ntrain, nA = D.A;
+    constexpr int nslab = B / SLAB;
+    float *const gsl = reinterpret_cast<float *>(dyn);
+    float *const rs = reinterpret_cast<float *>(dyn + 32 * 1024);
+    float *const lossp = rs + B;
+    float *const lsp = lossp + MAX_TRAIN * nslab;
+    float *const tot = lsp + nslab * 32;
+    const uint2 rdv = ldg8(g_rd + (size_t)row * 2);
+    if (tid < 32) lsl[tid] = ldg(g_ls + (tid < nA ? tid : nA - 1));
+    float ls = 0.f, pm = 0.f, pv = 0.f;
+    if (!D.deterministic && tid < nA) {
+      const int64_t o = D.off_log_std + tid;
+      ls = ldg(D.params + o), pm = ldg(D.exp_avg + o), pv = ldg(D.exp_avg_sq + o);
+    }
+    for (int net = 0; net < nt; ++net) {
+      const FuSlots sl = fu_slots(D, net);
+      const int out_dim = D.net[net].out_dim;
+      const bool gauss = net == D.net_a && !D.deterministic;
+#pragma unroll 1
+      for (int s0 = sl.lo; s0 < sl.hi; s0 += 8) {
+        FuFin<4> f;
+        fu_fin_issue(f, D, sl, net, s0, hh, row, g_outs, g_act);
+        fu_fin_finish(f, sl, s0, hh, row, fin);
+      }
+      __syncthreads();
+      if (tid < B) {
+        LossIn lin;
+        fu_lossin(lin, D, net, fin, row, __builtin_bit_cast(float, rdv.x), __builtin_bit_cast(float, rdv.y));
+        float s = 0.f;
+#pragma unroll 1
+        for (int j = 0; j < out_dim; ++j) {
+          if (net == D.net_a) lin.mean = fin[(sl.mean + j) * B + row], lin.act = fin[(sl.act + j) * B + row];
+          lin.ls = lsl[j];
+          float d3, lt, gs;
+          loss_terms<true>(D, net, lin, (float)B, D.two_over_B, d3, lt, gs);
+          s += lt;
+          if (gauss) gsl[j * B + row] = gs;
+        }
+        rs[row] = s;
+      }
+      __syncthreads();
+      if (tid < nslab) {
+        float s = 0.f;
+#pragma unroll
+        for (int rr = 0; rr < SLAB; ++rr) s += rs[tid * SLAB + rr];
+        lossp[net * nslab + tid] = s;
+      }
+      if (gauss) {
+        for (int e = tid; e < nA * nslab; e += UT) {
+          const int j = e / nslab, sb = e - j * nslab;
+          float s = 0.f;
+#pragma unroll
+          for (int rr = 0; rr < SLAB; ++rr) s += gsl[j * B + sb * SLAB + rr];
+          lsp[sb * nA + j] = s;
+        }
+      }
+      __syncthreads();
+    }
+    if (!D.deterministic && tid < nA) {
+      float g = 0.f;
+      for (int s = 0; s < nslab; ++s) g += lsp[s * nA + tid];
+      const int64_t o = D.off_log_std + tid;
+      const float lsc = fminf(fmaxf(ls, -20.f), 2.f);
+      g = g * expf(lsc) * ((ls >= -20.f && ls <= 2.f) ? 1.f : 0.f);
+      float p = ls;
+      adam_apply<true>(p, pm, pv, g, coef, coef.neg_step[2]);
+      stg(D.params + o, p), stg(D.exp_avg + o, pm), stg(D.exp_avg_sq + o, pv);
+      if (D.grads) stg(D.grads + o, g);
+    }
+    if (tid >= 64 && tid < 64 + nt) {
+      const int n = tid - 64;
+      float s = 0.f;
+      for (int k = 0; k < nslab; ++k) s += lossp[n * nslab + k];
+      tot[n] = s / (float)B;
+    }
+    __syncthreads();
+    if (tid == 64) {
+      const float vl = tot[D.net_v];
+      float ql = 0.f;
+      for (int e = 0; e < D.E; ++e) ql += tot[e];
+      ql = ql / (float)D.E;
+      const float al = tot[D.net_a];
+      Cp->last_losses[0] = vl, Cp->last_losses[1] = ql, Cp->last_losses[2] = al;
+      Cp->loss_sum[0] += vl, Cp->loss_sum[1] += ql, Cp->loss_sum[2] += al;
+      if (A.losses_out) {
+        float *lo = A.losses_out + (size_t)(t1 - 1 - A.base_step) * 3;
+        stg(lo, vl), stg(lo + 1, ql), stg(lo + 2, al);
+      }
+      Cp->ctr[1] = t1;
+      Cp->ctr[0] = t1;
+    }
+    STAMP(2, 4);
+    return;
+  }
+
+  if (it.net < 0) {
+    if (D.prefetch && (A.idx_mode == 0 || (A.idx_mode == 1 && t1 - A.base_step < A.n_steps)))
+      stage_rows16<true, true>(D, A, t1, it.o0 * (UT / 16), it.i0 * (UT / 16), tid);
+    return;
+  }
+
+  const int net = it.net, L = it.layer;
+  const int out_dim = it.nout, opad = it.nopad;
+  const int Odim = it.Odim, Idim = it.Idim, Kw = it.Kw, Opad = it.Opad;
+  const int o0 = it.o0, i0 = it.i0;
+  const float neg_step = it.group == 0 ? coef.neg_step[0] : (it.group == 1 ? coef.neg_step[1] : coef.neg_step[2]);
+  const bool has_target = it.has_target != 0;
+  const T *const w3x = reinterpret_cast<const T *>(par ? it.w3x[1] : it.w3x[0]);
+  const T *const w2x = reinterpret_cast<const T *>(par ? it.w2x[1] : it.w2x[0]);
+  T *const w3x_out = reinterpret_cast<T *>(par ? it.w3x[0] : it.w3x[1]);
+  T *const w2x_out = reinterpret_cast<T *>(par ? it.w2x[0] : it.w2x[1]);
+  pin_s(D.tau), pin_s(D.one_m_tau), pin_s(D.polyak_convex), pin_s(D.beta), pin_s(D.iql_tau), pin_s(D.discount);
+  pin_s(D.inv_E), pin_s(D.two_over_B), pin_s(D.net_a), pin_s(D.net_v), pin_s(D.deterministic);
+  pin_s(it.off_w), pin_s(it.toff_w), pin_s(it.off_b), pin_s(it.toff_b), pin_s(it.wc), pin_s(it.tc);
+  pin_s(it.w2ct), pin_s(it.w3t), pin_s(it.Xsrc), pin_s(Kw), pin_s(neg_step);
+  pin_s(coef.one_m_b1), pin_s(coef.b2), pin_s(coef.one_m_b2), pin_s(coef.eps), pin_s(coef.inv_bc2_sqrt);
+
+  const FuSlots sl = fu_slots(D, net);
+  const bool small = net != D.net_a && sl.hi - sl.lo <= 4;
+  FuFin<10> f0;
+  if (small) {
+    FuFin<2> f2;
+    fu_fin_issue(f2, D, sl, net, sl.lo, hh, row, g_outs, g_act);
+#pragma unroll
+    for (int c = 0; c < 2; ++c)
+#pragma unroll
+      for (int p = 0; p < 4; ++p) f0.pv[c][p] = f2.pv[c][p];
+  } else {
+    fu_fin_issue(f0, D, sl, net, sl.lo, hh, row, g_outs, g_act);
+  }
+  const uint2 rdv = ldg8(g_rd + (size_t)row * 2);
+  const float lsv = ldg(g_ls + ((tid & 31) < D.A ? (tid & 31) : D.A - 1));
+  __builtin_amdgcn_sched_barrier(0);
+
+  T *const dz3b = L == 0 ? reinterpret_cast<T *>(lds_upd) : reinterpret_cast<T *>(dyn + FU_OFF_DZ3);
+
+  auto loss_phase = [&]() {
+    if (tid < 32) lsl[tid] = lsv;
+    if (small) {
+#pragma unroll
+      for (int c = 0; c < 2; ++c) {
+        const int s = sl.lo + 2 * c + hh;
+        if (s < sl.hi) {
+          float sum = f0.pv[c][0];
+#pragma unroll
+          for (int p = 1; p < 4; ++p) sum += f0.pv[c][p];
+          fin[s * B + row] = P::round(sum);
+        }
+      }
+    } else {
+      fu_fin_finish(f0, sl, sl.lo, hh, row, fin);
+#pragma unroll 1
+      for (int s0 = sl.lo + 20; s0 < sl.hi; s0 += 20) {
+        FuFin<10> f;
+        fu_fin_issue(f, D, sl, net, s0, hh, row, g_outs, g_act);
+        fu_fin_finish(f, sl, s0, hh, row, fin);
+      }
+    }
+    for (int e = tid; e < (opad - out_dim) * B; e += UT) dz3b[(out_dim + e / B) * FU_DLD + (e & (B - 1))] = 0;
+    __syncthreads();
+    LossIn lin;
+    fu_lossin(lin, D, net, fin, row, __builtin_bit_cast(float, rdv.x), __builtin_bit_cast(float, rdv.y));
+#pragma unroll 1
+    for (int j = hh; j < out_dim; j += 2) {
+      if (net == D.net_a) lin.mean = fin[(sl.mean + j) * B + row], lin.act = fin[(sl.act + j) * B + row];
+      lin.ls = lsl[j];
+      float d3, lt, gs;
+      loss_terms<true>(D, net, lin, (float)B, D.two_over_B, d3, lt, gs);
+      dz3b[j * FU_DLD + row] = f2bf(d3);
+    }
+    __syncthreads();
+    STAMP(2, 2);
+  };
+
+  if (L == 0) {
+    const int Ipad = round_up(Idim, 16);
+    const int TLD = Ipad + 4;
+    const int64_t fbase = it.off_w + (int64_t)o0 * Idim, tbase = it.toff_w + (int64_t)o0 * Idim;
+    constexpr int UNE = (USR * UMAXI + UT - 1) / UT;
+    const int n_el = USR * Idim;
+    float pf[UNE], mf[UNE], vf[UNE], tf[UNE];
+    float pb, mb, vb, tb;
+#pragma unroll
+    for (int k = 0; k < UNE; ++k) {
+      const int e = tid + UT * k;
+      const int ec = e < n_el ? e : n_el - 1;
+      pf[k] = ldg(g_params + fbase + ec);
+      mf[k] = ldg(g_m + fbase + ec);
+      vf[k] = ldg(g_v + fbase + ec);
+      tf[k] = ldg((has_target ? g_target + tbase : g_params + fbase) + ec);
+    }
+    {
+      const int ob_ = o0 + (tid & (USR - 1));
+      const int64_t eb = it.off_b + ob_;
+      pb = ldg(g_params + eb), mb = ldg(g_m + eb), vb = ldg(g_v + eb);
+      tb = ldg((has_target ? g_target + it.toff_b : g_params + it.off_b) + ob_);
+    }
+    STAMP(2, 1);
+    __builtin_amdgcn_sched_barrier(0);
+    loss_phase();
+    const uint32_t *m2net = g_m2 + (size_t)net * B * (H / 32);
+#define CALL(JN_, UN_) fu_strip_panel<JN_, UN_>(dyn, dz3b, w3x, opad, m2net, wave, lane)
+    FU_DISPATCH_JN(out_dim, CALL);
+#undef CALL
+    const T *Xsrc = reinterpret_cast<const T *>(it.Xsrc) + (size_t)((t1 - 1) & 1) * D.xrows * BP;
+    const int nit = Ipad >> 4;
+    const int th = wave;
+    constexpr int NT = UNIT / (UT / 64 / UOT);
+    static_assert(NT == 1, "512 threads: one in-feature tile per wave");
+    uint4 w2t[nk];
+#pragma unroll
+    for (int ks = 0; ks < nk; ++ks) w2t[ks] = ldg16(w2x + frag_off<P>(o0 >> 4, ks, H / P::KM, lane));
+    float h1v[2][4];
+#pragma unroll
+    for (int mm = 0; mm < 2; ++mm)
+      load4T<true>(g_hT + (size_t)(net * 2 + 0) * H * BP + fidx<P>(o0 + r, 16 * (2 * wave + mm) + 4 * q, nk), h1v[mm]);
+    uint4 xf[nk];
+    {
+      const int tt = th < nit ? th : nit - 1;
+#pragma unroll
+      for (int ks = 0; ks < nk; ++ks) xf[ks] = ldg16(Xsrc + frag_off<P>(tt, ks, nk, lane));
+    }
+    __syncthreads();
+    STAMP(2, 7);
+    char *const dz1 = reinterpret_cast<char *>(tile2);
+#pragma unroll
+    for (int mm = 0; mm < 2; ++mm) {
+      const int m = 2 * wave + mm;
+      f32x4 acc = f32x4{0.f, 0.f, 0.f, 0.f};
+#pragma unroll
+      for (int ks = 0; ks < nk; ++ks) {
+        const uint4 a = *reinterpret_cast<const uint4 *>(dyn + ((m * nk + ks) * 64 + lane) * 16);
+        P::mma(a, w2t[ks], acc);
+      }
+      float tv[4];
+#pragma unroll
+      for (int i = 0; i < 4; ++i) tv[i] = h1v[mm][i] > 0.f ? acc[i] : 0.f;
+      *reinterpret_cast<uint2 *>(dz1 + (((m >> 1) * 64 + (2 * (m & 1) + (q >> 1)) * 16 + r) * 16 + (q & 1) * 8)) =
+          make_uint2(pk_bf16(tv[0], tv[1]), pk_bf16(tv[2], tv[3]));
+    }
+    __syncthreads();
+    f32x4 acc = f32x4{0.f, 0.f, 0.f, 0.f};
+    float bsum = 0.f;
+    if (th < nit) {
+      uint4 zf[nk];
+#pragma unroll
+      for (int ks = 0; ks < nk; ++ks) zf[ks] = *reinterpret_cast<const uint4 *>(dz1 + (ks * 64 + lane) * 16);
+      if (th == 0) {
+#pragma unroll
+        for (int ks = 0; ks < nk; ++ks) {
+          const uint32_t w[4] = {zf[ks].x, zf[ks].y, zf[ks].z, zf[ks].w};
+#pragma unroll
+          for (int i = 0; i < 4; ++i) bsum += bf2f((uint16_t)(w[i] & 0xffff)) + bf2f((uint16_t)(w[i] >> 16));
+        }
+      }
+#pragma unroll
+      for (int ks = 0; ks < nk; ++ks) P::mma(xf[ks], zf[ks], acc);
+      *reinterpret_cast<f32x4 *>(&tile[r * TLD + 16 * th + 4 * q]) = acc;
+    }
+    if (th == 0) {
+      bsum = xor32_sum(xor16_sum(bsum));
+      if (q == 0) bgrad[r] = bsum;
+    }
+    __syncthreads();
+    STAMP(2, 3);
+    T *wc = reinterpret_cast<T *>(it.wc);
+    T *tc = reinterpret_cast<T *>(it.tc);
+    const int nkw = Kw / P::KM;
+#pragma unroll
+    for (int k = 0; k < UNE; ++k) {
+      const int e = tid + UT * k;
+      if (e < n_el) {
+        const int ol = e / Idim, i = e - ol * Idim;
+        const float g = P::round(tile[ol * TLD + i]);
+        float p_ = pf[k], m_ = mf[k], v_ = vf[k];
+        adam_apply<true>(p_, m_, v_, g, coef, neg_step);
+        tile[ol * TLD + i] = p_;
+        stg(g_params + fbase + e, p_), stg(g_m + fbase + e, m_), stg(g_v + fbase + e, v_);
+        if (g_grads) stg(g_grads + fbase + e, g);
+        if (has_target) {
+          const float t_ = polyak(D, tf[k], p_);
+          tile2[ol * TLD + i] = t_;
+          stg(g_target + tbase + e, t_);
+        }
+      }
+    }
+    if (tid < USR) {
+      const int64_t e = it.off_b + o0 + tid;
+      const float g = P::round(bgrad[tid]);
+      adam_apply<true>(pb, mb, vb, g, coef, neg_step);
+      stg(g_params + e, pb), stg(g_m + e, mb), stg(g_v + e, vb);
+      if (g_grads) stg(g_grads + e, g);
+      if (has_target) stg(g_target + it.toff_b + o0 + tid, polyak(D, tb, pb));
+    }
+    __syncthreads();
+    const int cpr = Ipad >> 2;
+    for (int e = tid; e < USR * cpr; e += UT) {
+      const int ol = e / cpr, i = (e - ol * cpr) * 4;
+      const float4 p4 = *reinterpret_cast<const float4 *>(&tile[ol * TLD + i]);
+      float pv4[4] = {p4.x, p4.y, p4.z, p4.w};
+      store4T<true>(wc + fidx<P>(o0 + ol, i, nkw), pv4);
+      if (has_target) {
+        const float4 t4 = *reinterpret_cast<const float4 *>(&tile2[ol * TLD + i]);
+        float tv4[4] = {i < Idim ? t4.x : 0.f, i + 1 < Idim ? t4.y : 0.f, i + 2 < Idim ? t4.z : 0.f,
+                        i + 3 < Idim ? t4.w : 0.f};
+        store4T<true>(tc + fidx<P>(o0 + ol, i, nkw), tv4);
+      }
+    }
+    STAMP(2, 4);
+    return;
+  }
+
+  const T *Xsrc = reinterpret_cast<const T *>(it.Xsrc);
+  const bool do_bias = i0 == 0;
+  const int ntile_o = Opad >> 4;
+  const uint32_t lane16 = (uint32_t)lane * 16u;
+  constexpr int UTPR_ = UTPR, URPP = UT / UTPR_;
+  static_assert(URPP == UTO, "512 threads: one pass over the tile rows");
+  const int tr = tid / UTPR_, tc4 = (tid % UTPR_) * 4;
+  const int wo = wave >> 1, wi = wave & 1;
+  const int ib = i0 + 16 * wi, ob = o0 + 16 * wo;
+  const bool wave_bias = do_bias && wi == 0;
+  const int otl = (ob >> 4) < ntile_o ? (ob >> 4) : ntile_o - 1;
+  uint4 h2f[4];
+  if (L == 1) {
+#pragma unroll
+    for (int ot = 0; ot < 4; ++ot)
+      h2f[ot] = ldg16(g_hT + (size_t)(net * 2 + 1) * H * BP + frag_off<P>((o0 >> 4) + ot, wave, nk, lane));
+  }
+  uint4 xf[nk];
+  {
+    const char *const xb = reinterpret_cast<const char *>(Xsrc) + (size_t)((ib >> 4) * nk) * 1024;
+#pragma unroll
+    for (int ks = 0; ks < nk; ++ks) xf[ks] = ldg16(xb + (size_t)ks * 1024 + lane16);
+  }
+  __builtin_amdgcn_sched_barrier(0);
+  float pw[4], mw[4], vw[4], tw[4];
+  float pb, mb, vb, tb;
+  {
+    const int o = o0 + tr, i = i0 + tc4;
+    const int oc = o < Odim ? o : Odim - 1;
+    const int64_t e = it.off_w + (int64_t)oc * Idim + i;
+    const int64_t te = (has_target ? it.toff_w : it.off_w) + (int64_t)oc * Idim + i;
+    const float4 a4 = __builtin_bit_cast(float4, ldg16(g_params + e));
+    const float4 b4 = __builtin_bit_cast(float4, ldg16(g_m + e));
+    const float4 c4 = __builtin_bit_cast(float4, ldg16(g_v + e));
+    const float4 d4 = __builtin_bit_cast(float4, ldg16((has_target ? g_target : g_params) + te));
+    pw[0] = a4.x, pw[1] = a4.y, pw[2] = a4.z, pw[3] = a4.w;
+    mw[0] = b4.x, mw[1] = b4.y, mw[2] = b4.z, mw[3] = b4.w;
+    vw[0] = c4.x, vw[1] = c4.y, vw[2] = c4.z, vw[3] = c4.w;
+    tw[0] = d4.x, tw[1] = d4.y, tw[2] = d4.z, tw[3] = d4.w;
+    const int ob_ = o0 + (tid & (UTO - 1)) < Odim ? o0 + (tid & (UTO - 1)) : Odim - 1;
+    const int64_t eb = it.off_b + ob_;
+    pb = ldg(g_params + eb), mb = ldg(g_m + eb), vb = ldg(g_v + eb);
+    tb = ldg((has_target ? g_target + it.toff_b : g_params + it.off_b) + ob_);
+  }
+  STAMP(2, 1);
+  __builtin_amdgcn_sched_barrier(0);
+  loss_phase();
+  uint4 zf[nk];
+  if (L == 1) {
+#define CALL(JN_, UN_) fu_tile_panel<JN_>(dyn, dz3b, w3x, opad, o0, h2f, wave, lane)
+    FU_DISPATCH_JN(out_dim, CALL);
+#undef CALL
+    __syncthreads();
+    STAMP(2, 7);
+#pragma unroll
+    for (int ks = 0; ks < nk; ++ks) zf[ks] = *reinterpret_cast<const uint4 *>(dyn + ((wo * nk + ks) * 64 + lane) * 16);
+  } else {
+#pragma unroll
+    for (int ks = 0; ks < nk; ++ks)
+      zf[ks] = *reinterpret_cast<const uint4 *>(dz3b + (16 * otl + r) * FU_DLD + 32 * ks + 8 * q);
+  }
+  {
+    f32x4 acc = f32x4{0.f, 0.f, 0.f, 0.f};
+    float bsum = 0.f;
+#pragma unroll
+    for (int ks = 0; ks < nk; ++ks) {
+      if (wave_bias) frag_acc<true>(bsum, zf[ks]);
+      P::mma(xf[ks], zf[ks], acc);
+    }
+    *reinterpret_cast<f32x4 *>(&tile[(16 * wo + r) * ULD + 16 * wi + 4 * q]) = acc;
+    if (wave_bias) {
+      const float bs = xor32_sum(xor16_sum(bsum));
+      if (q == 0) bgrad[16 * wo + r] = bs;
+    }
+  }
+  __syncthreads();
+  STAMP(2, 3);
+  T *wc = reinterpret_cast<T *>(it.wc);
+  T *tc = reinterpret_cast<T *>(it.tc);
+  const int nkw = Kw / P::KM;
+  {
+    const int ol = tr, o = o0 + ol, i = i0 + tc4;
+    const float4 g4 = *reinterpret_cast<const float4 *>(&tile[ol * ULD + tc4]);
+    float g[4] = {g4.x, g4.y, g4.z, g4.w};
+    float p[4] = {pw[0], pw[1], pw[2], pw[3]};
+    float m[4] = {mw[0], mw[1], mw[2], mw[3]};
+    float v[4] = {vw[0], vw[1], vw[2], vw[3]};
+    float tv[4] = {tw[0], tw[1], tw[2], tw[3]};
+#pragma unroll
+    for (int k = 0; k < 4; ++k) {
+      g[k] = P::round(g[k]);
+      adam_apply<true>(p[k], m[k], v[k], g[k], coef, neg_step);
+      if (has_target) tv[k] = polyak(D, tv[k], p[k]);
+    }
+    if (L == 1) *reinterpret_cast<float4 *>(&tile[ol * ULD + tc4]) = make_float4(p[0], p[1], p[2], p[3]);
+    if (o < Odim && i < Idim) {
+      const int64_t e = it.off_w + (int64_t)o * Idim + i;
+      const int64_t te = it.toff_w + (int64_t)o * Idim + i;
+      state_store(g_params, e, make_float4(p[0], p[1], p[2], p[3]));
+      state_store(g_m, e, make_float4(m[0], m[1], m[2], m[3]));
+      state_store(g_v, e, make_float4(v[0], v[1], v[2], v[3]));
+      if (g_grads) stg16(g_grads + e, make_float4(g[0], g[1], g[2], g[3]));
+      if (has_target) state_store(g_target, te, make_float4(tv[0], tv[1], tv[2], tv[3]));
+      store4T<true>(wc + fidx<P>(o, i, nkw), p);
+      if (has_target) store4T<true>(tc + fidx<P>(o, i, nkw), tv);
+      if (L == 2) {
+        T *w3t = reinterpret_cast<T *>(it.w3t);
+#pragma unroll
+        for (int k = 0; k < 4; ++k) {
+          stg(w3t + (size_t)(i + k) * Opad + o, P::from_f32(p[k]));
+          stg(w3x_out + (size_t)(i + k) * Opad + o, P::from_f32(p[k]));
+        }
+      }
+    }
+  }
+  STAMP(2, 5);
+  if (do_bias && tid < UTO && o0 + tid < Odim) {
+    const int64_t e = it.off_b + o0 + tid;
+    const float g = P::round(bgrad[tid]);
+    adam_apply<true>(pb, mb, vb, g, coef, neg_step);
+    stg(g_params + e, pb), stg(g_m + e, mb), stg(g_v + e, vb);
+    if (g_grads) stg(g_grads + e, g);
+    if (has_target) stg(g_target + it.toff_b + o0 + tid, polyak(D, tb, pb));
+  }
+  STAMP(2, 6);
+  if (L == 1) {
+    __syncthreads();
+#pragma unroll
+    for (int ps = 0; ps < (UTO / 4) / (UT / UTI); ++ps) {
+      const int il = tid & (UTI - 1), o4 = ((tid >> 5) + (UT / UTI) * ps) * 4;
+      float pv4[4];
+#pragma unroll
+      for (int k = 0; k < 4; ++k) pv4[k] = tile[(o4 + k) * ULD + il];
+      store4T<true>(reinterpret_cast<T *>(it.w2ct) + fidx<P>(i0 + il, o0 + o4, H / P::KM), pv4);
+      store4T<true>(w2x_out + fidx<P>(i0 + il, o0 + o4, H / P::KM), pv4);
+    }
+  }
+  STAMP(2, 4);
+}
diff --git a/iqlpref_amd/csrc/iql_step.h b/iqlpref_amd/csrc/iql_step.h
--- a/iqlpref_amd/csrc/iql_step.h
+++ b/iqlpref_amd/csrc/iql_step.h
@@ -64,6 +64,9 @@
   unsigned long long *dbg;
   double beta1, beta2, eps;
   int64_t t_max;
+  uint32_t *m2;
+  float *rd2;
+  float *actf2;
   FwdNet fwd[MAX_FWD];
   TrainNet net[MAX_TRAIN];
 };
@@ -106,6 +109,8 @@
   void *wc, *tc, *w2ct;
   void *w3t;
   const void *Xsrc, *Zsrc;
+  int32_t nout, nopad;
+  void *w2x[2], *w3x[2];
 };
 
 }
diff --git a/iqlpref_amd/csrc/iql_step.hip b/iqlpref_amd/csrc/iql_step.hip
--- a/iqlpref_amd/csrc/iql_step.hip
+++ b/iqlpref_amd/csrc/iql_step.hip
@@ -305,7 +305,7 @@
   STAMP(0, 5);
 }
 
-template <bool BF16>
+template <bool BF16, bool PAR = false>
 __device__ __forceinline__ void stage_rows16(const TrainerDesc &D, const DevArgs &A, int64_t step, int row0,
                                              int row_step, int tid) {
   using P = Prec<BF16>;
@@ -334,17 +334,21 @@
         if (col < SA) stg(xT + fidx<P>(col, row, nkb), P::from_f32(v[e]));
         if (col >= S && col < SA) stg(D.actf + (size_t)row * D.A + (col - S), v[e]);
         if (col >= SA && col < SA + 2) stg(D.rd + (size_t)row * 2 + (col - SA), v[e]);
-      }
-    }
-  }
-}
-
-template <bool BF16>
+        if constexpr (PAR) {
+          if (col >= S && col < SA) stg(D.actf2 + ((size_t)(step & 1) * B + row) * D.A + (col - S), v[e]);
+          if (col >= SA && col < SA + 2) stg(D.rd2 + ((size_t)(step & 1) * B + row) * 2 + (col - SA), v[e]);
+        }
+      }
+    }
+  }
+}
+
+template <bool BF16, bool PAR = false>
 __global__ __launch_bounds__(256) void k_stage(const TrainerDesc *__restrict__ Dp,
                                                const DevArgs *__restrict__ Ap,
                                                const DevCtr *__restrict__ Cp) {
   Dp += blockIdx.y, Ap += blockIdx.y, Cp += blockIdx.y;
-  stage_rows16<BF16>(*Dp, *Ap, Cp->ctr[0], blockIdx.x * 16, gridDim.x * 16, threadIdx.x);
+  stage_rows16<BF16, PAR>(*Dp, *Ap, Cp->ctr[0], blockIdx.x * 16, gridDim.x * 16, threadIdx.x);
 }
 
 __device__ __forceinline__ void write_adam_coef(const TrainerDesc &D, const DevArgs &A, int64_t t1,
@@ -364,7 +368,7 @@
   static_assert(HQ == 64, "one 16-column tile per wave and part");
 };
 
-template <bool BF16, int H, int MT, int PW>
+template <bool BF16, int H, int MT, int PW, bool M2 = false>
 __global__ __launch_bounds__(256, 3) void k_forward(const TrainerDesc *__restrict__ Dp,
                                                  const DevArgs *__restrict__ Ap,
                                                  const DevCtr *__restrict__ Cp, const int nsl_,
@@ -401,6 +405,7 @@
   const unsigned sstride = (unsigned)D.stage_stride;
   float *const g_outs = D.outs;
   void *const g_hT = D.hT;
+  uint32_t *const g_m2 = M2 ? D.m2 : nullptr;
   const int64_t step = Cp->ctr[0];
   extern __shared__ __attribute__((aligned(16))) char smem[];
   const int tid = threadIdx.x, lane = tid & 63;
@@ -618,6 +623,22 @@
             for (int m = 0; m < MT; ++m)
               if (N.train_slot >= 0 && slab * ROWS + 16 * m < B)
                 act_store8_fwd(plane, fidx<P>(col, slab * ROWS + 16 * m + 4 * q, BP / P::KM), u[m]);
+          }
+          if constexpr (M2) {
+            if (N.train_slot >= 0) {
+#pragma unroll
+              for (int m = 0; m < MT; ++m) {
+#pragma unroll
+                for (int i = 0; i < 4; ++i) {
+                  const uint32_t hb = (i < 2 ? u[m].x : u[m].y) >> (16 * (i & 1));
+                  const uint64_t bal = __ballot(bf2f((uint16_t)(hb & 0xffff)) > 0.f);
+                  const int mrow = slab * ROWS + 16 * m + 4 * lane + i;
+                  if (lane < 4 && mrow < B)
+                    stg(reinterpret_cast<uint16_t *>(g_m2) + ((size_t)N.train_slot * B + mrow) * (H / 16) + (tile2 + 4 * j),
+                        (uint16_t)(bal >> (16 * (lane & 3))));
+                }
+              }
+            }
           }
         }
         continue;
@@ -2164,6 +2185,8 @@
   STAMP(2, 4);
 }
 
+#include "iql_fused.h"
+
 template <bool BF16, int H, bool PRE, int PW, bool NV = false>
 __global__ __launch_bounds__(256, PRE ? 1 : (PW > 1 ? (BF16 ? 4 : 2) : (BF16 ? 6 : 3)))
 void k_backward(const TrainerDesc *__restrict__ Dp, const DevArgs *__restrict__ Ap, DevCtr *__restrict__ Cp,
@@ -2255,6 +2278,9 @@
   hipError_t e = hipFuncSetAttribute(reinterpret_cast<const void *>(k_forward_tp<256, false>),
                                      hipFuncAttributeMaxDynamicSharedMemorySize, 160 * 1024);
   if (e != hipSuccess) return e;
+  e = hipFuncSetAttribute(reinterpret_cast<const void *>(k_update_fused), hipFuncAttributeMaxDynamicSharedMemorySize,
+                          FU_DYN_BYTES);
+  if (e != hipSuccess) return e;
   return hipFuncSetAttribute(reinterpret_cast<const void *>(k_forward_tp<256, true>),
                              hipFuncAttributeMaxDynamicSharedMemorySize, 160 * 1024);
 }
@@ -2262,7 +2288,14 @@
 size_t bwd_smem_bytes(bool bf16, int H);
 
 hipError_t launch_forward(bool bf16, const TrainerDesc &D, const TrainerDesc *dD, const DevArgs *a,
-                          const DevCtr *c, int n_seeds, hipStream_t st) {
+                          const DevCtr *c, int n_seeds, hipStream_t st, bool fused) {
+  if (fused) {
+    const int nsl = D.B / 16;
+    const int grid = 8 * ((D.nfwd + 1 + 7) / 8) * nsl * layer2_parts(D.H);
+    hipLaunchKernelGGL((k_forward<true, 256, 1, 1, true>), dim3(grid, 1), dim3(256), fwd_smem_bytes(true, 256, D.k1max, 1, 1),
+                       st, dD, a, c, nsl, D.nfwd);
+    return hipGetLastError();
+  }
   if (use_tp(bf16, D, n_seeds, false)) {
     const int nsl64 = D.B / 64;
     const int grid = 8 * ((D.nfwd + 1 + 7) / 8) * nsl64;
@@ -2350,11 +2383,18 @@
   return hipGetLastError();
 }
 hipError_t launch_stage(bool bf16, const TrainerDesc &D, const TrainerDesc *dD, const DevArgs *a,
-                        const DevCtr *c, int n_seeds, hipStream_t st) {
-  if (bf16)
+                        const DevCtr *c, int n_seeds, hipStream_t st, bool fused) {
+  if (fused)
+    hipLaunchKernelGGL((k_stage<true, true>), dim3((D.B + 15) / 16, 1), dim3(256), 0, st, dD, a, c);
+  else if (bf16)
     hipLaunchKernelGGL(k_stage<true>, dim3((D.B + 15) / 16, n_seeds), dim3(256), 0, st, dD, a, c);
   else
     hipLaunchKernelGGL(k_stage<false>, dim3((D.B + 15) / 16, n_seeds), dim3(256), 0, st, dD, a, c);
+  return hipGetLastError();
+}
+hipError_t launch_update_fused(const TrainerDesc *dD, const DevArgs *a, DevCtr *c, const UpdItem *items, int n_items,
+                               hipStream_t st) {
+  hipLaunchKernelGGL(k_update_fused, dim3(n_items + 1), dim3(FU_T), FU_DYN_BYTES, st, dD, a, c, items, n_items);
   return hipGetLastError();
 }
 int strip_rows() { return USR; }
diff --git a/iqlpref_amd/iql.py b/iqlpref_amd/iql.py
--- a/iqlpref_amd/iql.py
+++ b/iqlpref_amd/iql.py
@@ -614,6 +614,13 @@
         check(self._lib.iqlhip_trainer_step_kind(self._handle, C.byref(kind)))
         return "general" if kind.value else "tuned"
 
+    def step_launches(self, batch_size: int) -> int:
+        self._ensure_handle(batch_size)
+        n = int(self._lib.iqlhip_trainer_step_launches(self._handle, batch_size))
+        if n < 0:
+            check(n)
+        return n
+
     def sync_weights(self):
         if self._handle is not None:
             with torch.cuda.device(self._dev):
```

Measured after the change: 35680 steps/s. -46.8%, worse.
